# Dostenlinus/Aiyagari-HARK

Hardware: AMD Instinct MI355X
Metric: GE solves/sec (Table II sweep); agent-periods/sec; % HBM roofline (higher is better)
Workload: dtype f64

## Files before the change

aiyagari_hark_amd/_lib.py:

```python
from __future__ import annotations

import atexit
import ctypes
import os
import threading

import torch

HERE = os.path.dirname(os.path.abspath(__file__))
LIB_PATH = os.environ.get("AIYAGARI_LIB") or os.path.join(HERE, "lib", "libaiyagari.so")

AIY_OK = 0
ERRORS = {-1: "AIY_ERR_ARG", -2: "AIY_ERR_HIP", -3: "AIY_ERR_STATE", -4: "AIY_ERR_UNSUPPORTED",
          -5: "AIY_ERR_COMM"}
AIY_MAX_STATES = 64
AIY_SOW_DOUBLES = 8
AIY_OPT_USE_GRAPHS = 1
AIY_OPT_RESIDENT = 2
AIY_OPT_RESIDENT_SHAPE = 3
AIY_OPT_HIST_FUSED = 4
AIY_OPT_RESIDENT_STREAM = 5
AIY_OPT_HIST_RESIDENT = 6
AIY_OPT_HIST_CLUSTER = 7
AIY_OPT_HIST_ACCEL = 8
AIY_OPT_HIST_KRYLOV = 9
AIY_OPT_GE_RESIDENT = 10
AIY_OPT_CU_LIMIT = 11
AIY_OPT_GE_REBALANCE = 12
AIY_OPT_GE_EXTRAP_PERIOD = 13
AIY_OPT_GE_LOGSEC = 14
AIY_OPT_HIST_PULL = 15
AIY_OPT_GE_LOOSE_HIST = 17
AIY_OPT_RESIDENT_SHAPE_STREAM = 18
AIY_OPT_GE_ANDERSON = 23

c_double_p = ctypes.POINTER(ctypes.c_double)
c_int32_p = ctypes.POINTER(ctypes.c_int32)
c_uint8_p = ctypes.POINTER(ctypes.c_uint8)
vp = ctypes.c_void_p


class EgmDims(ctypes.Structure):
    _fields_ = [("n_cal", ctypes.c_int32), ("S", ctypes.c_int32), ("n_M", ctypes.c_int32), ("n_a", ctypes.c_int32)]


class EgmInputs(ctypes.Structure):
    _fields_ = [(n, vp) for n in ("a_grid", "M_grid", "P", "R_next", "W_next", "M_next", "lab", "beta", "crra")]


class Market(ctypes.Structure):
    _fields_ = [("cap_share", ctypes.c_double), ("depr_fac", ctypes.c_double),
                ("prod", ctypes.c_double * 2), ("agg_L", ctypes.c_double * 2)]


class PanelModel(ctypes.Structure):
    _fields_ = [("S", ctypes.c_int32), ("n_M", ctypes.c_int32), ("n_a", ctypes.c_int32), ("n_lab", ctypes.c_int32),
                ("tables", vp), ("M_grid", vp), ("lab_level", vp), ("lab_cdf", vp), ("mrkv_hist", vp),
                ("act_T", ctypes.c_int32), ("unemployed", ctypes.c_int32)]


class PanelBatch(ctypes.Structure):
    _fields_ = [("n_cal", ctypes.c_int32), ("S", ctypes.c_int32), ("n_M", ctypes.c_int32), ("n_a", ctypes.c_int32),
                ("n_lab", ctypes.c_int32), ("tables", vp), ("M_grid", vp), ("lab_level", vp), ("lab_cdf", vp),
                ("mrkv_hist", vp), ("unemployed", ctypes.c_int32)]


class StationaryModel(ctypes.Structure):
    _fields_ = [("n_cal", ctypes.c_int32), ("S", ctypes.c_int32), ("n_a", ctypes.c_int32)] + \
               [(n, vp) for n in ("a_grid", "P", "lab", "beta", "crra", "alpha", "delta", "disc")]


class TransitionModel(ctypes.Structure):
    _fields_ = [("n_cal", ctypes.c_int32), ("S", ctypes.c_int32), ("n_a", ctypes.c_int32), ("T", ctypes.c_int32)] + \
               [(n, vp) for n in ("a_grid", "P", "lab", "beta", "crra", "R", "w", "m_term", "c_term")]


class GeOptions(ctypes.Structure):
    _fields_ = [("method", ctypes.c_int32), ("r_tol", ctypes.c_double), ("egm_tol", ctypes.c_double),
                ("hist_tol", ctypes.c_double), ("max_steps", ctypes.c_int32), ("max_egm_cycles", ctypes.c_int32),
                ("max_hist_iter", ctypes.c_int32), ("warm_hist", ctypes.c_int32), ("warm_egm", ctypes.c_int32),
                ("accel", ctypes.c_int32), ("r_lo", vp), ("r_hi", vp), ("secant_start", ctypes.c_int32),
                ("loose_bracket", ctypes.c_int32), ("egm_extrapolate", ctypes.c_int32), ("status_out", vp)]


SIGNATURES = {
    "aiy_version": (ctypes.c_int32, []),
    "aiy_create": (ctypes.c_int32, [ctypes.c_int32, ctypes.POINTER(vp)]),
    "aiy_destroy": (ctypes.c_int32, [vp]),
    "aiy_last_error": (ctypes.c_char_p, [vp]),
    "aiy_egm_step": (ctypes.c_int32, [vp, ctypes.POINTER(EgmDims), ctypes.POINTER(EgmInputs), vp, vp, vp, vp, vp]),
    "aiy_egm_solve": (ctypes.c_int32, [vp, ctypes.POINTER(EgmDims), ctypes.POINTER(EgmInputs), ctypes.c_double,
                                       ctypes.c_int32, ctypes.c_int32, vp, vp, vp, vp, c_int32_p, c_double_p, vp]),
    "aiy_egm_solve_from": (ctypes.c_int32, [vp, ctypes.POINTER(EgmDims), ctypes.POINTER(EgmInputs), ctypes.c_double,
                                            ctypes.c_int32, ctypes.c_int32, vp, vp, vp, vp, vp, vp, c_int32_p,
                                            c_double_p, vp]),
    "aiy_egm_kernel_time": (ctypes.c_int32, [vp, ctypes.POINTER(EgmDims), ctypes.POINTER(EgmInputs), vp, vp, vp, vp,
                                             ctypes.c_int32, ctypes.POINTER(ctypes.c_float), vp]),
    "aiy_policy_eval": (ctypes.c_int32, [vp, ctypes.c_int32, ctypes.c_int32, ctypes.c_int32, vp, vp, vp, vp, vp, vp,
                                         ctypes.c_int64, vp, vp]),
    "aiy_sim_periods": (ctypes.c_int32, [vp, ctypes.POINTER(PanelModel), ctypes.POINTER(Market), ctypes.c_int64,
                                         ctypes.c_int64, ctypes.c_int64, vp, vp, vp, ctypes.c_int64, vp,
                                         ctypes.c_int64, ctypes.c_uint64, ctypes.c_uint32, ctypes.c_int32,
                                         ctypes.c_int32, vp, vp, vp, vp]),
    "aiy_sim_period_local": (ctypes.c_int32, [vp, ctypes.POINTER(PanelModel), ctypes.c_int64, ctypes.c_int64, vp, vp,
                                              vp, vp, ctypes.c_uint64, ctypes.c_uint32, ctypes.c_int32, vp, vp]),
    "aiy_sim_period_prices": (ctypes.c_int32, [vp, ctypes.POINTER(PanelModel), ctypes.POINTER(Market),
                                               ctypes.c_int64, ctypes.c_int32, vp, vp, vp, vp]),
    "aiy_get_shocks": (ctypes.c_int32, [vp, ctypes.c_int32, vp, ctypes.c_int64, ctypes.c_int64, vp, vp,
                                        ctypes.c_uint64, ctypes.c_uint32, ctypes.c_int32, vp]),
    "aiy_get_states": (ctypes.c_int32, [vp, vp, ctypes.c_int64, ctypes.c_double, ctypes.c_double, vp, vp, vp, vp,
                                        vp]),
    "aiy_get_controls": (ctypes.c_int32, [vp, ctypes.c_int32, ctypes.c_int32, ctypes.c_int32, vp, vp, c_double_p,
                                          ctypes.c_int32, ctypes.c_double, ctypes.c_int64, vp, vp, vp, vp, vp]),
    "aiy_get_poststates": (ctypes.c_int32, [vp, ctypes.c_int64, vp, vp, vp, vp]),
    "aiy_sum": (ctypes.c_int32, [vp, vp, ctypes.c_int64, vp, vp]),
    "aiy_sim_kernel_time": (ctypes.c_int32, [vp, ctypes.POINTER(PanelModel), ctypes.POINTER(Market), ctypes.c_int64,
                                             vp, vp, ctypes.c_uint64, ctypes.c_uint32, vp, ctypes.c_int32,
                                             ctypes.POINTER(ctypes.c_float), vp]),
    "aiy_panel_launch_stats": (ctypes.c_int32, [vp, c_double_p, ctypes.POINTER(ctypes.c_int64),
                                                ctypes.POINTER(ctypes.c_int64), ctypes.c_int32]),
    "aiy_sim_block_max_agents": (ctypes.c_int32, []),
    "aiy_sim_block_periods": (ctypes.c_int32, [vp, ctypes.POINTER(PanelBatch), vp, ctypes.c_int64, vp, vp, vp,
                                               vp, vp, ctypes.c_uint32, ctypes.c_int32, ctypes.c_int32, ctypes.c_int32,
                                               vp, vp, vp, vp]),
    "aiy_set_option": (ctypes.c_int32, [vp, ctypes.c_int32, ctypes.c_int64]),
    "aiy_get_option": (ctypes.c_int32, [vp, ctypes.c_int32, ctypes.POINTER(ctypes.c_int64)]),
    "aiy_index_ints_per_row": (ctypes.c_int32, []),
    "aiy_panel_table_bytes": (ctypes.c_int64, [ctypes.c_int32, ctypes.c_int32, ctypes.c_int32, ctypes.c_int32]),
    "aiy_panel_build": (ctypes.c_int32, [vp, ctypes.c_int32, ctypes.c_int32, ctypes.c_int32, ctypes.c_int32,
                                         ctypes.c_int32, ctypes.c_int32, vp, vp, vp, vp]),
    "aiy_build_index": (ctypes.c_int32, [vp, ctypes.c_int64, ctypes.c_int32, vp, vp, vp]),
    "aiy_comm_unique_id": (ctypes.c_int32, [vp]),
    "aiy_comm_init": (ctypes.c_int32, [vp, vp, ctypes.c_int32, ctypes.c_int32]),
    "aiy_comm_bind": (ctypes.c_int32, [vp, vp]),
    "aiy_comm_destroy": (ctypes.c_int32, [vp]),
    "aiy_allreduce_sum": (ctypes.c_int32, [vp, vp, ctypes.c_int64, vp]),
    "aiy_hist_lottery": (ctypes.c_int32, [vp, ctypes.c_int32, ctypes.c_int32, ctypes.c_int32, vp, vp, vp, vp, vp, vp,
                                          vp, vp, vp]),
    "aiy_hist_solve": (ctypes.c_int32, [vp, ctypes.c_int32, ctypes.c_int32, ctypes.c_int32, vp, vp, vp, vp,
                                        ctypes.c_double, ctypes.c_int32, ctypes.c_int32, vp, vp, c_double_p,
                                        c_int32_p, vp]),
    "aiy_hist_launch_stats": (ctypes.c_int32, [vp, c_double_p, ctypes.POINTER(ctypes.c_int64), ctypes.c_int32]),
    "aiy_ge_resident_plan": (ctypes.c_int32, [vp, ctypes.c_int32, ctypes.c_int32, ctypes.c_int32, c_int32_p]),
    "aiy_ge_last_profile": (ctypes.c_int32, [vp, c_double_p, ctypes.c_int32]),
    "aiy_ge_last_eval_log": (ctypes.c_int32, [vp, c_double_p, ctypes.c_int32]),
    "aiy_ge_last_rounds": (ctypes.c_int32, [vp, ctypes.POINTER(ctypes.c_int32), ctypes.POINTER(ctypes.c_int32)]),
    "aiy_ge_launch_stats": (ctypes.c_int32, [vp, c_double_p, ctypes.POINTER(ctypes.c_int64), c_double_p, c_double_p,
                                             ctypes.c_int32]),
    "aiy_ge_stationary_work_bytes": (ctypes.c_int64, [ctypes.c_int32, ctypes.c_int32, ctypes.c_int32]),
    "aiy_ge_stationary": (ctypes.c_int32, [vp, ctypes.POINTER(StationaryModel), ctypes.POINTER(GeOptions), vp,
                                           c_double_p, c_double_p, c_double_p, c_int32_p, c_int32_p, c_int32_p, vp]),
    "aiy_transition_work_bytes": (ctypes.c_int64, [ctypes.c_int32, ctypes.c_int32, ctypes.c_int32, ctypes.c_int32]),
    "aiy_transition_backward": (ctypes.c_int32, [vp, ctypes.POINTER(TransitionModel), vp, vp, vp, vp, vp, vp]),
    "aiy_transition_forward": (ctypes.c_int32, [vp, ctypes.c_int32, ctypes.c_int32, ctypes.c_int32, ctypes.c_int32,
                                                vp, vp, vp, vp, vp, vp, vp, vp, vp, c_double_p, c_double_p, vp]),
    "aiy_transition_forward_marginals": (ctypes.c_int32, [vp, ctypes.c_int32, ctypes.c_int32, ctypes.c_int32,
                                                          ctypes.c_int32, vp, vp, vp, vp, vp, vp, vp, vp, vp,
                                                          c_double_p, c_double_p, vp, vp]),
    "aiy_jacobian_work_bytes": (ctypes.c_int64, [ctypes.c_int32, ctypes.c_int32, ctypes.c_int32, ctypes.c_int32]),
    "aiy_jacobian_fanout": (ctypes.c_int32, [vp, ctypes.c_int32, ctypes.c_int32, ctypes.c_int32, ctypes.c_int32,
                                             ctypes.c_int32, vp, vp, vp, vp, vp, vp, vp]),
    "aiy_jacobian_diff": (ctypes.c_int32, [vp, ctypes.c_int64, vp, vp, ctypes.c_double, vp]),
    "aiy_jacobian_expectation": (ctypes.c_int32, [vp, ctypes.c_int32, ctypes.c_int32, ctypes.c_int32, ctypes.c_int32,
                                                  vp, vp, vp, vp, vp, vp, vp]),
    "aiy_jacobian_contract": (ctypes.c_int32, [vp, ctypes.c_int32, ctypes.c_int32, ctypes.c_int32, ctypes.c_int32,
                                               vp, vp, vp, vp, vp, vp]),
    "aiy_lottery_mean": (ctypes.c_int32, [vp, ctypes.c_int32, ctypes.c_int32, ctypes.c_int32, ctypes.c_int32, vp, vp, vp,
                                          vp, vp]),
    "aiy_aggregate_lotteries": (ctypes.c_int32, [vp, ctypes.c_int32, ctypes.c_int32, ctypes.c_int32, ctypes.c_int32,
                                                 ctypes.c_int32, vp, vp, vp, vp, vp, vp, vp, vp]),
    "aiy_wealth_stats": (ctypes.c_int32, [vp, vp, vp, ctypes.c_int64, c_double_p, ctypes.c_int32, c_double_p,
                                          c_double_p, vp]),
    "aiy_dist_stats_work_bytes": (ctypes.c_int64, [ctypes.c_int32, ctypes.c_int32]),
    "aiy_dist_marginal": (ctypes.c_int32, [vp, ctypes.c_int32, ctypes.c_int32, ctypes.c_int32, vp, vp, vp]),
    "aiy_dist_stats": (ctypes.c_int32, [vp, ctypes.c_int32, ctypes.c_int32, ctypes.c_int32, vp, vp, c_double_p,
                                        ctypes.c_int32, vp, c_double_p, c_double_p, c_double_p, vp]),
    "aiy_value_work_bytes": (ctypes.c_int64, [ctypes.c_int32, ctypes.c_int32, ctypes.c_int32]),
    "aiy_value_backward": (ctypes.c_int32, [vp, ctypes.c_int32, ctypes.c_int32, ctypes.c_int32, ctypes.c_int32,
                                            vp, vp, vp, vp, vp, vp, vp, vp, vp, vp, vp, vp, vp, vp]),
    "aiy_value_stationary": (ctypes.c_int32, [vp, ctypes.c_int32, ctypes.c_int32, ctypes.c_int32, vp, vp, vp, vp, vp,
                                              vp, vp, vp, vp, c_double_p, ctypes.c_double, ctypes.c_int32,
                                              ctypes.c_int32, vp, vp, c_int32_p, c_double_p, vp]),
    "aiy_value_reduce": (ctypes.c_int32, [vp, ctypes.c_int32, ctypes.c_int32, ctypes.c_int32, vp, vp, c_double_p, vp]),
    "aiy_consumption_equivalent": (ctypes.c_int32, [vp, ctypes.c_int32, ctypes.c_int64, vp, vp, vp, vp, vp, vp]),
}

_lib = None
_lock = threading.Lock()


class AiyagariLibError(RuntimeError):
    pass


def load(path: str | None = None):
    global _lib
    with _lock:
        if _lib is not None:
            return _lib
        p = path or LIB_PATH
        if not os.path.exists(p):
            raise AiyagariLibError(
                f"{p} is missing: build it with `python -m aiyagari_hark_amd.build` "
                "(there is no CPU fallback)")
        lib = ctypes.CDLL(p)
        for name, (res, args) in SIGNATURES.items():
            fn = getattr(lib, name)
            fn.restype = res
            fn.argtypes = args
        _lib = lib
        return lib


def exported_symbols():
    return sorted(SIGNATURES)


class Handle:

    def __init__(self, device: int | None = 0):
        self.lib = load()
        if device is None:
            device = torch.cuda.current_device()
        self.device = device
        h = vp()
        rc = self.lib.aiy_create(int(device), ctypes.byref(h))
        if rc != AIY_OK:
            raise AiyagariLibError(f"aiy_create(device={device}) failed: {ERRORS.get(rc, rc)}")
        self.h = h

    def check(self, rc: int, what: str):
        if rc != AIY_OK:
            msg = self.lib.aiy_last_error(self.h)
            raise AiyagariLibError(f"{what} failed: {ERRORS.get(rc, rc)}: {msg.decode() if msg else ''}")

    def get_option(self, option: int) -> int:
        v = ctypes.c_int64()
        self.check(self.lib.aiy_get_option(self.h, int(option), ctypes.byref(v)), "aiy_get_option")
        return int(v.value)

    def set_options(self, values: dict) -> dict:
        prev = {k: self.get_option(k) for k in values}
        for k, v in values.items():
            self.check(self.lib.aiy_set_option(self.h, int(k), int(v)), "aiy_set_option")
        return prev

    def close(self):
        if getattr(self, "h", None):
            self.lib.aiy_destroy(self.h)
            self.h = None

    def __del__(self):
        try:
            self.close()
        except Exception:
            pass


_handles: dict[int, Handle] = {}


def close_all():
    while _handles:
        _, h = _handles.popitem()
        h.close()


atexit.register(close_all)


def handle(device: int | None = None) -> Handle:
    if device is None:
        device = torch.cuda.current_device()
    h = _handles.get(device)
    if h is None:
        h = Handle(device)
        _handles[device] = h
    return h


def ptr(t) -> int | None:
    if t is None:
        return None
    if not t.is_cuda:
        raise AiyagariLibError("libaiyagari takes device tensors only")
    if not t.is_contiguous():
        raise AiyagariLibError("tensor must be contiguous")
    return t.data_ptr()


def work_space(device, what: str, label: str, **sizes):
    nbytes = int(getattr(handle(device.index).lib, f"aiy_{what}_work_bytes")(*(int(v) for v in sizes.values())))
    if nbytes < 0:
        raise ValueError(f"{label} sizes not supported: ".lstrip() + " ".join(f"{k}={v}" for k, v in sizes.items()))
    return torch.empty(nbytes, dtype=torch.uint8, device=device)


def stream_ptr(stream=None) -> int:
    s = stream if stream is not None else torch.cuda.current_stream()
    return s.cuda_stream
```

aiyagari_hark_amd/csrc/ge_resident.hip:

```cpp
#include "common.h"
#include "egm_common.h"
#include "ge_search.h"
#include "hist_bicg.h"
#include "hist_cluster.h"
#include "internal.h"

#include <algorithm>
#include <cmath>

namespace aiy {

constexpr int kGeTHMax = 1024;
constexpr int kGeWavesMax = kGeTHMax / kWave;
constexpr int kGeMaxTiles = 16;
constexpr int kGeBufs = 5;
constexpr int kGeAaM = 3;
constexpr int kGeAaHist = kGeAaM + 2;
#ifdef AIY_DIAG_NO_FUSEA
constexpr bool kGeFuseA = false;
#else
constexpr bool kGeFuseA = true;
#endif
#ifndef AIY_FUSEA_KC2
#define AIY_FUSEA_KC2 0
#endif
constexpr bool kGeFuseAKc2 = AIY_FUSEA_KC2 != 0;
template <int NW>
constexpr size_t ge_egm_lds() { return (size_t)NW * (8 * kTile + 4 * kWin) * sizeof(double); }

struct GeCalDev {
  double alpha, delta, disc, r_lo, r_hi;
};

struct GeState;
struct GeRun {
  int n_cal, S, n_a, G, nj, cap, n_work;
  const double* a_grid;
  const double* P;
  const double* lab;
  const double* beta;
  const double* crra;
  const GeCalDev* cal;
  int method;
  double r_tol, egm_tol, hist_tol;
  int max_steps, max_cyc, max_hist;
  int warm_hist, warm_egm, secant, loose, extrap;
  int extrap_period;
  int aa_period;
  double* aah;
  int logsec;
  double loose_hist;
  double* qb;
  int* ainv;
  double* tab;
  double* mass;
  double* pmass;
  double* pg;
  int* lo;
  double* wlo;
  double* slab;
  int* span;
  unsigned* ctr;
  unsigned long long* gran;
  const int* cal_ids;
  GeState* saved;
  const int* resume;
  unsigned* done_ctr;
  int stop_at;
  int* out_done;
  unsigned* err;
  double* out_r;
  double* out_K;
  double* out_Ks;
  int* out_steps;
  int* out_cyc;
  int* out_its;
  int* out_status;
  double* out_prof;
  double* out_evlog;
};
constexpr int kGeProf = 8;
constexpr int kGeEvLog = 32;
constexpr int kGeEvRec = 6;

struct GeState {
  GeEval ev;
  GeEvalOpts opt;
  double Ks, dist, lam_prev, fext;
  int status, n, stop, nan_stop, moved, extrap;
  int in_hist;
  int buf[kGeBufs];
  long long cyc_sum, its_sum;
  unsigned long long t_egm, t_lot, t_hist, t_k, t0, t_ev0;
  unsigned nc_prev[2];
  unsigned nbc;
};

template <int TH>
__device__ __forceinline__ bool ge_reduce(unsigned long long* gran, int G, int w, unsigned& ne, const double* vals,
                                          int nv, unsigned kmax, double (*s_part)[kGeWavesMax], double* s_res,
                                          int* s_flag, unsigned* err) {
  asm volatile("s_waitcnt vmcnt(0)" ::: "memory");
  return hc_reduce<TH>(gran, G, w, ne, vals, nv, kmax, s_part, s_res, s_flag, err, [] {});
}

template <int SMAX, int NW, typename Sink, typename Begin, typename End>
__device__ __forceinline__ void ge_rows_pass(int S, int n_a, int j0, int j1, const double* __restrict__ a_grid,
                                             const double* __restrict__ src_m, const double* __restrict__ src_c,
                                             double R, const double* s_Wl, int* s_hint, double* lds_win,
                                             Sink&& sink, Begin&& begin, End&& end) {
  const int tid = threadIdx.x, lane = tid & (kWave - 1);
  const int wv = __builtin_amdgcn_readfirstlane(tid / kWave);
  const int n = n_a, n1 = n_a + 1;
  const int ntile = (j1 - j0 + kTile - 1) / kTile;
  double* X = lds_win + (size_t)wv * 4 * kWin;
  double* Y = X + kWin;
  double* XB = X + 2 * kWin;
  double* YB = X + 3 * kWin;
#pragma unroll 1
  for (int tile = wv; tile < ntile; tile += NW) {
    const int jr = j0 + tile * kTile + lane;
    const int j = jr < j1 ? jr : j1 - 1;
    const double a = a_grid[j];
    int* hint = s_hint + tile * SMAX;
    auto fetch = [&](int r, RowWin& wn) {
      const int rr = r < S ? r : S - 1;
      load_win<true>(src_m + (size_t)rr * n1, src_c + (size_t)rr * n1, n, win_base(hint[rr], n1), lane, wn);
    };
    unsigned redo = 0u;
    auto step_unit = [&](int u, const RowWin& wa, const RowWin& wb) {
      const int ra = 2 * u, rb = 2 * u + 1;
      if (ra >= S) return;
      const bool has_b = rb < S;
      const int rbb = has_b ? rb : ra;
      const bool na = __any(stage_win(wa, n, X, Y, lane));
      const bool nb = __any(stage_win(wb, n, XB, YB, lane));
      __builtin_amdgcn_fence(__ATOMIC_RELEASE, "wavefront");
      __builtin_amdgcn_wave_barrier();
      __builtin_amdgcn_fence(__ATOMIC_ACQUIRE, "wavefront");
      const double qa = R * a + s_Wl[ra];
      const double qb = R * a + s_Wl[rbb];
      int lba, lbb;
      bool oka, okb;
      const double fa = search_win(wa.base, na, n, qa, X, Y, lba, oka);
      const double fb = search_win(wb.base, nb, n, qb, XB, YB, lbb, okb);
      hint[ra] = __builtin_amdgcn_readfirstlane(lba);
      if (has_b) hint[rb] = __builtin_amdgcn_readfirstlane(lbb);
      if (__any(!oka)) redo |= 1u << ra;
      else sink(tile, jr, j, ra, qa, fa);
      if (has_b) {
        if (__any(!okb)) redo |= 1u << rb;
        else sink(tile, jr, j, rb, qb, fb);
      }
    };
    RowWin a0, b0, a1, b1;
    fetch(0, a0);
    fetch(1, b0);
    begin(tile, j);
#pragma unroll 1
    for (int u = 0; 2 * u < S; u += 2) {
      fetch(2 * u + 2, a1);
      fetch(2 * u + 3, b1);
      step_unit(u, a0, b0);
      fetch(2 * u + 4, a0);
      fetch(2 * u + 5, b0);
      step_unit(u + 1, a1, b1);
    }
#pragma unroll 1
    while (redo != 0u) {
      const int s = __builtin_ctz(redo);
      redo &= redo - 1u;
      const double q = R * a + s_Wl[s];
      int lb;
      const double f = interp_row_global_agent(src_m + (size_t)s * n1, src_c + (size_t)s * n1, n, q, lb);
      hint[s] = __builtin_amdgcn_readfirstlane(lb);
      sink(tile, jr, j, s, q, f);
    }
    end(tile, j, a);
  }
}

template <int SMAX, int SC, int PK, int NW>
__device__ __forceinline__ double ge_egm_cycle(int S, int n_a, int j0, int j1, const double* __restrict__ a_grid,
                                               const double* src_m, const double* src_c, double* dst_m,
                                               double* dst_c, bool track, double R, double beta, double gam,
                                               const double* s_Wl, const double* s_Pe, int* s_hint,
                                               double* lds_v, double* lds_win, double* ring) {
  const int tid = threadIdx.x, lane = tid & (kWave - 1);
  const int wv = __builtin_amdgcn_readfirstlane(tid / kWave);
  const int n1 = n_a + 1;
  double* Vw = lds_v + (size_t)wv * SMAX * kTile;
  const int ntile = (j1 - j0 + kTile - 1) / kTile;
  double dmax = 0.0;
  if (src_m == nullptr) {
#pragma unroll 1
    for (int tile = wv; tile < ntile; tile += NW) {
      const int jr = j0 + tile * kTile + lane;
      const int j = jr < j1 ? jr : j1 - 1;
      const double a = a_grid[j];
      for (int sp = 0; sp < S; ++sp) {
        const double c = (R * a + s_Wl[sp]) * 1.0;
        Vw[sp * kTile + lane] = R * marg_u<PK>(c, gam);
      }
      for (int s = 0; s < S; ++s) {
        double sum;
        if constexpr (SC > 0) sum = pairwise_dot<SC>(Vw + lane, s_Pe + s * SC);
        else sum = np_pairwise_sum<SMAX>(S, [&](int t) { return Vw[t * kTile + lane] * uniform_f64(s_Pe[s * S + t]); });
        const double c = inv_marg<PK>(beta * sum, gam);
        store_f64_agent(&dst_m[(size_t)s * n1 + j + 1], a + c);
        store_f64_agent(&dst_c[(size_t)s * n1 + j + 1], c);
        if (ring) store_f64_agent(&ring[(size_t)s * n_a + j], c);
        if (j == 0) {
          store_f64_agent(&dst_m[(size_t)s * n1], kBorrowNode);
          store_f64_agent(&dst_c[(size_t)s * n1], kBorrowNode);
        }
      }
    }
    return 0.0;
  }
  constexpr int NP = SC > 0 ? SC : SMAX;
  double pmv[NP], pcv[NP];
  auto begin = [&](int, int j) {
#pragma unroll
    for (int s = 0; s < NP; ++s) {
      const int rr = s < S ? s : S - 1;
      pmv[s] = load_f64_agent(&src_m[(size_t)rr * n1 + j + 1]);
      pcv[s] = load_f64_agent(&src_c[(size_t)rr * n1 + j + 1]);
    }
  };
  auto end = [&](int, int j, double a) {
#pragma unroll
    for (int s = 0; s < NP; ++s) {
      if (s < S) {
        __builtin_amdgcn_sched_barrier(0);
        double sum;
        if constexpr (SC > 0) sum = pairwise_dot<SC>(Vw + lane, s_Pe + s * SC);
        else sum = np_pairwise_sum<SMAX>(S, [&](int t) { return Vw[t * kTile + lane] * uniform_f64(s_Pe[s * S + t]); });
        const double E = beta * sum;
        const double c = inv_marg<PK>(E, gam);
        const double m = a + c;
        store_f64_agent(&dst_m[(size_t)s * n1 + j + 1], m);
        store_f64_agent(&dst_c[(size_t)s * n1 + j + 1], c);
        if (ring) store_f64_agent(&ring[(size_t)s * n_a + j], c);
        if (track) dmax = nan_max(dmax, nan_max(fabs(m - pmv[s]), fabs(c - pcv[s])));
        if (j == 0) {
          store_f64_agent(&dst_m[(size_t)s * n1], kBorrowNode);
          store_f64_agent(&dst_c[(size_t)s * n1], kBorrowNode);
        }
      }
    }
  };
  ge_rows_pass<SMAX, NW>(S, n_a, j0, j1, a_grid, src_m, src_c, R, s_Wl, s_hint, lds_win,
                     [&](int, int, int, int sp, double, double f) {
                       Vw[sp * kTile + lane] = R * marg_u<PK>(f, gam);
                     },
                     begin, end);
  return dmax;
}

constexpr int kGeSmax = 8;
extern __shared__ double ge_dyn[];
__shared__ double ge_s_part[kHcRed][kGeWavesMax];
__shared__ double ge_s_res[kHcRed];
__shared__ int ge_s_flag;
__shared__ double ge_s_Pe[kGeSmax * kGeSmax];
__shared__ double ge_s_Wl[kGeSmax];
__shared__ int ge_s_hint[kGeMaxTiles * kGeSmax];
__shared__ unsigned ge_s_nc;
__shared__ GeState ge_st;

template <int SMAX, int SC, int PK, int NW>
__device__ __forceinline__ double ge_egm_cycle_fn(int S, int n_a, int j0, int j1, const double* a_grid,
                                               const double* src_m, const double* src_c, double* dst_m,
                                               double* dst_c, bool track, double R, double beta, double gam,
                                               double* dyn, double* ring) {
  return ge_egm_cycle<SMAX, SC, PK, NW>(S, n_a, j0, j1, a_grid, src_m, src_c, dst_m, dst_c, track, R, beta, gam,
                                        ge_s_Wl, ge_s_Pe, ge_s_hint, dyn, dyn + (size_t)NW * SMAX * kTile, ring);
}

template <int SMAX, int NW>
__device__ __forceinline__ void ge_lottery_fn(int S, int n_a, int j0, int j1, const double* a_grid, const double* fm,
                                           const double* fc, double R, bool have_prev, int* LO, double* WL,
                                           bool write_through) {
  ge_rows_pass<SMAX, NW>(S, n_a, j0, j1, a_grid, fm, fc, R, ge_s_Wl, ge_s_hint, ge_dyn + (size_t)NW * SMAX * kTile,
                     [&](int, int jr, int, int s, double q, double c) {
                       if (jr >= j1) return;
                       const double ap = q - c;
                       const size_t o = (size_t)s * n_a + jr;
                       int d = -1;
                       if (have_prev) {
                         const int h = LO[o];
                         if (h >= 0 && h < n_a - 1 && a_grid[h] <= ap && ap < a_grid[h + 1]) d = h;
                       }
                       if (d < 0) {
                         int lo = 0, hi = n_a;
                         while (lo < hi) {
                           const int mid = lo + ((hi - lo) >> 1);
                           if (a_grid[mid] <= ap) lo = mid + 1; else hi = mid;
                         }
                         d = lo - 1;
                       }
                       d = d < 0 ? 0 : (d > n_a - 2 ? n_a - 2 : d);
                       double wl = (a_grid[d + 1] - ap) / (a_grid[d + 1] - a_grid[d]);
                       wl = wl < 0.0 ? 0.0 : (wl > 1.0 ? 1.0 : wl);
                       if (write_through) {
                         __hip_atomic_store(to_global(&LO[o]), d, __ATOMIC_RELAXED, __HIP_MEMORY_SCOPE_AGENT);
                         store_f64_agent(&WL[o], wl);
                       } else {
                         LO[o] = d;
                         WL[o] = wl;
                       }
                     },
                     [](int, int) {}, [](int, int, double) {});
}

struct GeCtx {
  double* tab;
  double* X;
  double* PX;
  int* LO;
  double* WL;
  unsigned* ctr;
  unsigned long long* cw;
  unsigned long long* gran;
  const double* a_grid;
  double* aah;
  unsigned* err;
  double beta, gam;
  size_t tab_sz;
  int j0, j1, w, G, S, n_a, cal, lc;
  __device__ __forceinline__ double* tabm(int b) const { return tab + (size_t)b * 2 * tab_sz; }
  __device__ __forceinline__ double* tabc(int b) const { return tab + (size_t)b * 2 * tab_sz + tab_sz; }
};

__device__ __forceinline__ GeEvalOpts ge_eval_opts(const GeRun& g) {
  return {g.method, g.loose, g.logsec, g.warm_egm, g.warm_hist, g.secant, g.r_tol, g.egm_tol, g.hist_tol, g.loose_hist};
}

__device__ __forceinline__ bool ge_barrier(const GeCtx& cx, unsigned& nb, unsigned* err) {
  asm volatile("s_waitcnt vmcnt(0)" ::: "memory");
  ++nb;
  return hc_barrier(err, cx.ctr, (unsigned)cx.G * nb, &ge_s_flag);
}

__device__ __forceinline__ bool ge_vote(const GeCtx& cx, unsigned* err, unsigned flag, unsigned& dlt) {
  GeState& st = ge_st;
  const int tid = threadIdx.x;
  if (tid == 0) ++st.nbc;
  asm volatile("s_waitcnt vmcnt(0)" ::: "memory");
  __syncthreads();
  const unsigned k = st.nbc, par = k & 1u;
  if (!hc_barrier_count(err, &cx.cw[par], (unsigned)cx.G * ((k + par) / 2), flag, &ge_s_nc, &ge_s_flag))
    return false;
  if (tid == 0) {
    dlt = ge_s_nc - st.nc_prev[par];
    st.nc_prev[par] = ge_s_nc;
  }
  return true;
}

template <int TH>
__device__ __forceinline__ void ge_secant_tables(const GeCtx& cx, int b_cur, int b_prev, int b_init, double theta) {
  const int tid = threadIdx.x, n1 = cx.n_a + 1;
  for (int s = 0; s < cx.S; ++s) {
    for (int k = cx.j0 + tid; k < cx.j1; k += TH) {
      const size_t o = (size_t)s * n1 + k + 1;
      const double cm = load_f64_agent(&cx.tabm(b_cur)[o]), pm = load_f64_agent(&cx.tabm(b_prev)[o]);
      const double cc = load_f64_agent(&cx.tabc(b_cur)[o]), pc = load_f64_agent(&cx.tabc(b_prev)[o]);
      store_f64_agent(&cx.tabm(b_init)[o], theta == 0.0 ? cm : cm + theta * (cm - pm));
      store_f64_agent(&cx.tabc(b_init)[o], theta == 0.0 ? cc : cc + theta * (cc - pc));
    }
    if (cx.j0 == 0 && tid == 0) {
      store_f64_agent(&cx.tabm(b_init)[(size_t)s * n1], kBorrowNode);
      store_f64_agent(&cx.tabc(b_init)[(size_t)s * n1], kBorrowNode);
    }
  }
}

template <int TH>
__device__ __forceinline__ bool ge_extrapolate(const GeCtx& cx, unsigned& nb, unsigned* err, int b_dst, int b_src,
                                               double dclu, int n) {
  GeState& st = ge_st;
  const int tid = threadIdx.x, n1 = cx.n_a + 1;
  if (tid == 0) {
    st.fext = egm_extrap_factor(dclu, st.dist, st.ev.etol, n, st.lam_prev);
    if (st.fext != 0.0) st.moved = 1;
  }
  __syncthreads();
  const double f = st.fext;
  if (f != 0.0) {
    double* cm = cx.tabm(b_dst);
    double* cc = cx.tabc(b_dst);
    const double* pm = cx.tabm(b_src);
    const double* pc = cx.tabc(b_src);
    for (int s = 0; s < cx.S; ++s)
      for (int k = cx.j0 + tid; k < cx.j1; k += TH) {
        const size_t o = (size_t)s * n1 + k + 1;
        const double x = load_f64_agent(&cm[o]), y = load_f64_agent(&cc[o]);
        store_f64_agent(&cm[o], x + f * (x - load_f64_agent(&pm[o])));
        store_f64_agent(&cc[o], y + f * (y - load_f64_agent(&pc[o])));
      }
    if (!ge_barrier(cx, nb, err)) return false;
  }
  return true;
}

__device__ __forceinline__ double* ge_ring(const GeCtx& cx, int c) {
  return cx.aah + (size_t)(c % kGeAaHist) * cx.S * cx.n_a;
}

template <int TH>
__device__ __forceinline__ bool ge_anderson(const GeCtx& cx, unsigned& nb, unsigned& ne, int n, int b_dst) {
  static_assert(kGeAaM == 3 && kGeAaHist == 5, "the mixing is written for m = 3");
  const int tid = threadIdx.x, n1 = cx.n_a + 1;
  const double* W0 = ge_ring(cx, n - 4);
  const double* W1 = ge_ring(cx, n - 3);
  const double* W2 = ge_ring(cx, n - 2);
  const double* W3 = ge_ring(cx, n - 1);
  const double* W4 = ge_ring(cx, n);
  double gp[9];
  for (int q = 0; q < 9; ++q) gp[q] = 0.0;
  for (int s = 0; s < cx.S; ++s)
    for (int k = cx.j0 + tid; k < cx.j1; k += TH) {
      const size_t o = (size_t)s * cx.n_a + k;
      const double w0 = load_f64_agent(W0 + o), w1 = load_f64_agent(W1 + o), w2 = load_f64_agent(W2 + o);
      const double w3 = load_f64_agent(W3 + o), w4 = load_f64_agent(W4 + o);
      aa_gram_add(w0, w1, w2, w3, w4, gp);
    }
  double gs[9], gam[3];
  if (!ge_reduce<TH>(cx.gran, cx.G, cx.w, ne, gp, 6, 0u, ge_s_part, ge_s_res, &ge_s_flag, cx.err)) return false;
  for (int q = 0; q < 6; ++q) gs[q] = ge_s_res[q];
  if (!ge_reduce<TH>(cx.gran, cx.G, cx.w, ne, gp + 6, 3, 0u, ge_s_part, ge_s_res, &ge_s_flag, cx.err)) return false;
  for (int q = 0; q < 3; ++q) gs[6 + q] = ge_s_res[q];
  if (aa_solve(gs, gam)) {
    double* dm = cx.tabm(b_dst);
    double* dc = cx.tabc(b_dst);
    for (int s = 0; s < cx.S; ++s)
      for (int k = cx.j0 + tid; k < cx.j1; k += TH) {
        const size_t o = (size_t)s * cx.n_a + k;
        const double w1 = load_f64_agent(W1 + o), w2 = load_f64_agent(W2 + o);
        const double w3 = load_f64_agent(W3 + o), w4 = load_f64_agent(W4 + o);
        const double cn = aa_mix(gam, w1, w2, w3, w4);
        store_f64_agent(&dm[(size_t)s * n1 + k + 1], cx.a_grid[k] + cn);
        store_f64_agent(&dc[(size_t)s * n1 + k + 1], cn);
      }
    if (tid == 0) ge_st.moved = 1;
    if (!ge_barrier(cx, nb, cx.err)) return false;
  }
  return true;
}

struct GeHhOpt {
  int max_cyc, aa_period, extrap_period;
};

__device__ __forceinline__ bool ge_ring_wanted(int n, int p) {
  const int ph = n % p;
  const int mix = ph == 0 ? n : n + (p - ph);
  return (ph == 0 || ph > p - kGeAaHist) && mix >= kGeAaHist + 1;
}

template <int SMAX, int SC, int PK, int TH>
__device__ __forceinline__ int ge_household_solve(const GeCtx& cx, unsigned& nb, unsigned& ne, const GeHhOpt& g,
                                                  double R, const double* init_m, const double* init_c, double* dyn) {
  constexpr int NW = TH / kWave;
  GeState& st = ge_st;
  const int tid = threadIdx.x;
  int final_buf = -1;
  for (int attempt = 0; attempt < 2; ++attempt) {
    if (!ge_barrier(cx, nb, cx.err)) return -1;
    const bool aa = g.aa_period > 0 && attempt == 0;
    const bool ext = st.extrap != 0 && attempt == 0 && !aa;
    if (tid == 0) {
      st.lam_prev = -1.0;
      st.moved = 0;
      st.nan_stop = 0;
    }
    int n = 1;
    const int last_allowed = g.max_cyc + 1;
    bool converged = false;
    while (true) {
      const int b_dst = st.buf[n & 1], b_src = st.buf[(n - 1) & 1];
      const double* sm = n == 1 ? init_m : cx.tabm(b_src);
      const double* sc = n == 1 ? init_c : cx.tabc(b_src);
      const bool track = n >= 2;
      double* ring = aa && ge_ring_wanted(n, g.aa_period) ? ge_ring(cx, n) : nullptr;
      const double dl = ge_egm_cycle_fn<SMAX, SC, PK, NW>(cx.S, cx.n_a, cx.j0, cx.j1, cx.a_grid, sm, sc, cx.tabm(b_dst),
                                                          cx.tabc(b_dst), track, R, cx.beta, cx.gam, dyn, ring);
      const int xp = g.extrap_period;
      const bool want_value = ext && n >= xp - 1 && ((n % xp) == xp - 1 || (n % xp) == 0);
      double dclu = 0.0;
      bool go;
      if (want_value) {
        double v[1] = {dl};
        if (!ge_reduce<TH>(cx.gran, cx.G, cx.w, ne, v, 1, 1u, ge_s_part, ge_s_res, &ge_s_flag, cx.err)) return -1;
        dclu = ge_s_res[0];
        go = dclu > st.ev.etol;
        if (tid == 0) st.nan_stop = dclu != dclu;
      } else {
        const double dw = wave_nan_max(dl);
        if ((tid & (kWave - 1)) == 0) ge_s_part[0][tid / kWave] = dw;
        __syncthreads();
        unsigned flag = 0u, dlt = 0u;
        if (tid == 0) {
          double d = ge_s_part[0][0];
          for (int q = 1; q < TH / kWave; ++q) d = nan_max(d, ge_s_part[0][q]);
          flag = (d > st.ev.etol ? 1u : 0u) | (d != d ? (1u << 16) : 0u);
        }
        if (!ge_vote(cx, cx.err, flag, dlt)) return -1;
        if (tid == 0) {
          st.stop = (dlt & 0xffffu) == 0u || (dlt >> 16) != 0u;
          st.nan_stop = (dlt >> 16) != 0u;
        }
        __syncthreads();
        go = !st.stop;
      }
      if (track && !go) {
        converged = true;
        break;
      }
      if (n >= last_allowed) break;
      if (want_value && (n % xp) == 0) {
        if (!ge_extrapolate<TH>(cx, nb, cx.err, b_dst, b_src, dclu, n)) return -1;
      } else if (want_value) {
        if (tid == 0) st.dist = dclu;
      }
      if (aa && n >= g.aa_period && n >= kGeAaHist + 1 && (n % g.aa_period) == 0) {
        if (!ge_anderson<TH>(cx, nb, ne, n, b_dst)) return -1;
      }
      ++n;
    }
    if (tid == 0) {
      st.n = n;
      if (!converged) st.status |= 1;
    }
    __syncthreads();
    final_buf = st.buf[n & 1];
    if (!(st.moved && st.nan_stop)) break;
    if (tid == 0) {
      st.extrap = 0;
      st.status &= ~1;
    }
    __syncthreads();
  }
  return final_buf;
}

struct GeHhArgs {
  gptr<double> tab, aah;
  gptr<unsigned> ctr, err;
  gptr<unsigned long long> gran;
  gptr<const double> a_grid, init_m, init_c;
  double beta, gam, R;
  int j0, j1, w, G, S, n_a;
  GeHhOpt opt;
  unsigned dyn_lds;
};
template <int SMAX, int SC, int PK, int TH>
__device__ __noinline__ int ge_household_isolated(GeHhArgs a, unsigned* nb_io, unsigned* ne_io) {
  double* dyn = (double*)(lptr<double>)(size_t)(unsigned)hk_uni((int)a.dyn_lds);
  GeCtx cx;
  cx.tab = (double*)hk_uni(a.tab);
  cx.aah = (double*)hk_uni(a.aah);
  cx.ctr = (unsigned*)hk_uni(a.ctr);
  cx.cw = reinterpret_cast<unsigned long long*>(cx.ctr + 2);
  cx.err = (unsigned*)hk_uni(a.err);
  cx.gran = (unsigned long long*)hk_uni(a.gran);
  cx.a_grid = (const double*)hk_uni(a.a_grid);
  cx.X = cx.PX = cx.WL = nullptr;
  cx.LO = nullptr;
  cx.beta = hk_uni(a.beta); cx.gam = hk_uni(a.gam);
  cx.j0 = hk_uni(a.j0); cx.j1 = hk_uni(a.j1); cx.w = hk_uni(a.w); cx.G = hk_uni(a.G);
  cx.S = SC > 0 ? SC : hk_uni(a.S);
  cx.n_a = hk_uni(a.n_a);
  cx.cal = cx.lc = 0;
  cx.tab_sz = (size_t)cx.S * (cx.n_a + 1);
  const GeHhOpt opt = {hk_uni(a.opt.max_cyc), hk_uni(a.opt.aa_period), hk_uni(a.opt.extrap_period)};
  unsigned nb = *nb_io, ne = *ne_io;
  const int fb = ge_household_solve<SMAX, SC, PK, TH>(cx, nb, ne, opt, hk_uni(a.R), (const double*)hk_uni(a.init_m),
                                                     (const double*)hk_uni(a.init_c), dyn);
  *nb_io = nb;
  *ne_io = ne;
  return fb;
}

template <int TH>
__device__ __forceinline__ void ge_mass_start(const GeCtx& cx, bool fresh, bool warm, bool secant, double theta) {
  const int tid = threadIdx.x;
  if (fresh) {
    const double u0 = 1.0 / ((double)cx.S * cx.n_a);
    for (int s = 0; s < cx.S; ++s)
      for (int k = cx.j0 + tid; k < cx.j1; k += TH) cx.X[(size_t)s * cx.n_a + k] = u0;
  } else if (warm) {
    for (int s = 0; s < cx.S; ++s)
      for (int k = cx.j0 + tid; k < cx.j1; k += TH) {
        const size_t o = (size_t)s * cx.n_a + k;
        const double x = cx.X[o];
        if (secant) cx.X[o] = theta == 0.0 ? x : x + theta * (x - cx.PX[o]);
        cx.PX[o] = x;
      }
  }
}

template <int TH>
__device__ __forceinline__ bool ge_capital(const GeCtx& cx, unsigned& ne, unsigned* err) {
  double part = 0.0;
  for (int k = cx.j0 + (int)threadIdx.x; k < cx.j1; k += TH) {
    double ms = 0.0;
    for (int s = 0; s < cx.S; ++s) ms += cx.X[(size_t)s * cx.n_a + k];
    part += ms * cx.a_grid[k];
  }
  double v[1] = {part};
  return ge_reduce<TH>(cx.gran, cx.G, cx.w, ne, v, 1, 0u, ge_s_part, ge_s_res, &ge_s_flag, err);
}

__device__ __forceinline__ void ge_write_out(const GeCtx& cx, const GeRun& g, const GeCalDev& cd) {
  const GeState& st = ge_st;
  const int cal = cx.cal;
  __hip_atomic_fetch_add(to_global(g.done_ctr), 1u, __ATOMIC_RELAXED, __HIP_MEMORY_SCOPE_AGENT);
  g.out_done[cal] = 1;
  g.out_r[cal] = st.ev.rs.x;
  g.out_K[cal] = ge_prices(st.ev.rs.x, cd.alpha, cd.delta).Kd;
  g.out_Ks[cal] = st.Ks;
  g.out_steps[cal] = st.ev.steps;
  g.out_cyc[cal] = (int)min(st.cyc_sum, 0x7fffffffll);
  g.out_its[cal] = (int)min(st.its_sum, 0x7fffffffll);
  g.out_status[cal] = st.status | (st.ev.rs.done ? 0 : 4);
  double* pf = g.out_prof + (size_t)cal * kGeProf;
  pf[0] = st.t_egm * 0.01;
  pf[1] = st.t_lot * 0.01;
  pf[2] = st.t_hist * 0.01;
  pf[3] = st.t_k * 0.01;
  pf[4] = (__builtin_amdgcn_s_memrealtime() - st.t0) * 0.01;
  pf[5] = (double)st.cyc_sum;
  pf[6] = (double)st.its_sum;
  pf[7] = (double)st.ev.steps;
}

template <int SMAX, int SC, int KC, int TH, bool PULL>
__global__ __launch_bounds__(TH) void ge_cluster_kernel(GeRun g) {
  constexpr int NW = TH / kWave;
  static_assert(SMAX <= kGeSmax, "file-scope LDS sized for kGeSmax states");
  GeState& st = ge_st;

  const int per = gridDim.x >> 3;
  const int u = (blockIdx.x & 7) * per + (blockIdx.x >> 3);
  if (u >= g.n_work) return;
  const int G = g.G, S = g.S, n_a = g.n_a;
  const int tid = threadIdx.x;
  GeCtx cx;
  cx.G = G; cx.S = S; cx.n_a = n_a;
  cx.lc = u / G; cx.w = u - cx.lc * G;
  const int lc = cx.lc, w = cx.w, cal = g.cal_ids[lc];
  cx.cal = cal;
  cx.j0 = w * g.nj; cx.j1 = min(cx.j0 + g.nj, n_a);
  const int j0 = cx.j0, j1 = cx.j1;
  cx.a_grid = g.a_grid + (size_t)cal * n_a;
  cx.beta = g.beta[cal]; cx.gam = g.crra[cal];
  const GeCalDev cd = g.cal[cal];
  cx.tab_sz = (size_t)S * (n_a + 1);
  cx.tab = g.tab + (size_t)cal * kGeBufs * 2 * cx.tab_sz;
  const size_t row0 = (size_t)cal * S * n_a;
  cx.X = g.mass + row0;
  cx.PX = g.pmass + row0;
  cx.LO = g.lo + row0;
  cx.WL = g.wlo + row0;
  cx.ctr = g.ctr + (size_t)lc * kHcCtrStride;
  cx.cw = reinterpret_cast<unsigned long long*>(cx.ctr + 2);
  cx.gran = g.gran + (size_t)lc * 2 * G * kHcRedRec;
  cx.aah = g.aah + (size_t)cal * kGeAaHist * S * n_a;
  cx.err = g.err;
  unsigned nb = 0, ne = 0;
  const int pk = crra_kind(cx.gam);

  for (int q = tid; q < S * S; q += TH) ge_s_Pe[q] = g.P[(size_t)cal * S * S + q];
  for (int q = tid; q < kGeMaxTiles * SMAX; q += TH) ge_s_hint[q] = -1;
  if (tid == 0) {
    if (g.resume[cal]) {
      st = g.saved[cal];
      st.t0 = __builtin_amdgcn_s_memrealtime() - st.t0;
    } else {
      st.ev.init(ge_eval_opts(g), cd.r_lo, cd.r_hi);
      st.Ks = 0.0;
      st.in_hist = 0;
      st.status = 0;
      st.cyc_sum = st.its_sum = 0;
      for (int b = 0; b < kGeBufs; ++b) st.buf[b] = b;
      st.t_egm = st.t_lot = st.t_hist = st.t_k = 0ull;
      st.t0 = __builtin_amdgcn_s_memrealtime();
    }
    st.opt = ge_eval_opts(g);
    st.nc_prev[0] = st.nc_prev[1] = 0u;
    st.nbc = 0u;
  }
  __syncthreads();

  bool stopped = false;
  while ((!st.ev.rs.done && st.ev.steps < g.max_steps) || st.ev.final_ks) {
    if (g.stop_at > 0 && st.ev.steps > 0 && !st.in_hist) {
      unsigned flag = 0u, dlt = 0u;
      if (tid == 0)
        flag = __hip_atomic_load(to_global(g.done_ctr), __ATOMIC_RELAXED, __HIP_MEMORY_SCOPE_AGENT) >=
                       (unsigned)g.stop_at ? 1u : 0u;
      if (!ge_vote(cx, g.err, flag, dlt)) return;
      if (tid == 0) st.stop = dlt != 0u;
      __syncthreads();
      if (st.stop) {
        stopped = true;
        break;
      }
    }
    unsigned long long tp = __builtin_amdgcn_s_memrealtime();
    if (tid == 0 && !st.in_hist) st.t_ev0 = tp;
    if (!st.in_hist) {
      if (tid == 0) {
        st.ev.plan(st.opt, cd.alpha, cd.delta);
        st.extrap = g.extrap;
        st.moved = 0;
      }
      __syncthreads();
      if (tid < S) ge_s_Wl[tid] = st.ev.wage * g.lab[(size_t)cal * S + tid];
      const double R = st.ev.R, theta = st.ev.theta;
      const bool secant = st.ev.secant != 0, warm = st.ev.warm_egm != 0;
      const int b_cur = st.buf[2], b_prev = st.buf[3], b_init = st.buf[4];
      if (secant) ge_secant_tables<TH>(cx, b_cur, b_prev, b_init, theta);
      tp = __builtin_amdgcn_s_memrealtime();
      GeHhArgs ha;
      ha.tab = to_global(cx.tab); ha.aah = to_global(cx.aah); ha.ctr = to_global(cx.ctr); ha.err = to_global(g.err);
      ha.gran = to_global(cx.gran); ha.a_grid = to_global(cx.a_grid);
      ha.init_m = to_global((const double*)(secant ? cx.tabm(b_init) : (warm ? cx.tabm(b_cur) : nullptr)));
      ha.init_c = to_global((const double*)(secant ? cx.tabc(b_init) : (warm ? cx.tabc(b_cur) : nullptr)));
      ha.beta = cx.beta; ha.gam = cx.gam; ha.R = R;
      ha.j0 = j0; ha.j1 = j1; ha.w = w; ha.G = G; ha.S = S; ha.n_a = n_a;
      ha.opt = {g.max_cyc, g.aa_period, g.extrap_period};
      ha.dyn_lds = hk_lds_addr(ge_dyn);
      const int final_buf = pk == 1   ? ge_household_isolated<SMAX, SC, 1, TH>(ha, &nb, &ne)
                            : pk == 3 ? ge_household_isolated<SMAX, SC, 3, TH>(ha, &nb, &ne)
                            : pk == 5 ? ge_household_isolated<SMAX, SC, 5, TH>(ha, &nb, &ne)
                                      : ge_household_isolated<SMAX, SC, 0, TH>(ha, &nb, &ne);
      if (final_buf < 0) return;
      if (tid == 0) {
        const unsigned long long tn = __builtin_amdgcn_s_memrealtime();
        st.t_egm += tn - tp;
        st.cyc_sum += st.n;
        const int fb = final_buf;
        const int other = st.buf[0] == fb ? st.buf[1] : st.buf[0];
        const int old_prev = st.buf[3];
        st.buf[3] = st.buf[2];
        st.buf[2] = fb;
        st.buf[0] = other;
        st.buf[1] = old_prev;
      }
      __syncthreads();
      tp = __builtin_amdgcn_s_memrealtime();
      ge_lottery_fn<SMAX, NW>(S, n_a, j0, j1, cx.a_grid, cx.tabm(st.buf[2]), cx.tabc(st.buf[2]), R, st.ev.steps > 0,
                              cx.LO, cx.WL, PULL);
      ge_mass_start<TH>(cx, st.ev.fresh_mass != 0, warm, secant, theta);
      __syncthreads();
      if (tid == 0) {
        const unsigned long long tn = __builtin_amdgcn_s_memrealtime();
        st.t_lot += tn - tp;
        tp = tn;
      }
    }
    int mv;
    {
      HkArgs hk;
      hk.G = G; hk.S = S; hk.n_a = n_a; hk.cap = g.cap; hk.w = w; hk.j0 = j0; hk.j1 = j1;
      hk.LO = to_global((const int*)cx.LO); hk.WL = to_global((const double*)cx.WL); hk.X = to_global(cx.X);
      hk.Pg = to_global(g.pg + row0); hk.Vg = to_global((double*)nullptr);
      hk.slab_cl = to_global(g.slab + (size_t)lc * G * 2 * g.cap);
      hk.span_cl = to_global(g.span + (size_t)lc * G * SMAX * 4);
      hk.ctr = to_global(cx.ctr); hk.gran = to_global(cx.gran); hk.Pc = to_global(g.P + (size_t)cal * S * S);
      hk.max_iter = g.max_hist; hk.err = to_global(g.err);
      hk.tol = st.ev.htol;
      hk.stop_ctr = to_global((const unsigned*)(g.stop_at > 0 ? g.done_ctr : nullptr));
      hk.stop_at = (unsigned)g.stop_at;
      hk.Qg = to_global(g.qb + row0);
      hk.Ainv = to_global(g.ainv + (size_t)cal * S * (n_a + 1));
      hk.lottery_fresh = true;
      hk.dyn_lds = hk_lds_addr(ge_dyn);
      if constexpr (PULL) mv = hk_solve_inlined<SMAX, KC, TH, true, false, SC>(hk, &nb, &ne);
      else mv = hk_solve_isolated<SMAX, KC, TH, false, (KC == 1 || kGeFuseAKc2) && kGeFuseA, SC>(hk, &nb, &ne);
    }
    if (mv == -1) return;
    if (tid == 0) {
      const unsigned long long tn = __builtin_amdgcn_s_memrealtime();
      st.t_hist += tn - tp;
      tp = tn;
    }
    if (mv <= -2) {
      if (tid == 0) {
        st.its_sum += -mv - 2;
        st.in_hist = 1;
        if (w == 0) __hip_atomic_fetch_add(to_global(g.done_ctr + 1), 1u, __ATOMIC_RELAXED, __HIP_MEMORY_SCOPE_AGENT);
      }
      __syncthreads();
      stopped = true;
      break;
    }
    if (tid == 0) st.in_hist = 0;
    if (!ge_capital<TH>(cx, ne, g.err)) return;
    const bool fin = st.ev.final_ks != 0;
    if (tid == 0) {
      const double Ks = ge_s_res[0];
      if (w == 0 && st.ev.steps < kGeEvLog && !fin) {
        double* ev = g.out_evlog + ((size_t)cal * kGeEvLog + st.ev.steps) * kGeEvRec;
        ev[0] = st.ev.rs.x;
        ev[1] = (Ks - st.ev.Kd) / st.ev.Kd;
        ev[2] = (double)st.n;
        ev[3] = (double)mv;
        ev[4] = (double)st.ev.loose;
        ev[5] = (double)(__builtin_amdgcn_s_memrealtime() - st.t_ev0) * 0.01;
      }
      st.its_sum += mv;
      if (mv >= g.max_hist) st.status |= 2;
    }
    if (fin) {
      if (tid == 0) st.Ks = ge_s_res[0];
      __syncthreads();
      break;
    }
    if (tid == 0) {
      st.ev.accept(ge_s_res[0]);
      st.Ks = ge_s_res[0];
      st.t_k += __builtin_amdgcn_s_memrealtime() - tp;
    }
    __syncthreads();
  }
  if (stopped) {
    if (w == 0 && tid == 0) {
      st.t0 = __builtin_amdgcn_s_memrealtime() - st.t0;
      g.saved[cal] = st;
      g.out_done[cal] = 0;
    }
    return;
  }
  if (w == 0 && tid == 0) ge_write_out(cx, g, cd);
}

struct GePlan {
  int G = 0, nj = 0, kc = 0, smax = 0, sc = 0, cap = 0, blocks = 0, th = 0;
  size_t lds = 0;
  const void* fn = nullptr;
};

template <int SMAX, int SC, int KC, int TH>
static const void* ge_fn(bool pull) {
  return pull ? reinterpret_cast<const void*>(ge_cluster_kernel<SMAX, SC, KC, TH, true>)
              : reinterpret_cast<const void*>(ge_cluster_kernel<SMAX, SC, KC, TH, false>);
}

static bool ge_make_plan(aiy_handle* h, int n_cal, int S, int n_a, GePlan& p) {
  if (S < 1 || S > kGeSmax || n_a < 2 || n_cal < 1) return false;
  int cus = 0;
  if (hipDeviceGetAttribute(&cus, hipDeviceAttributeMultiprocessorCount, h->device) != hipSuccess || cus < 1) return false;
  if (h->cu_limit > 0) cus = std::min(cus, h->cu_limit);
  const int g_cap = h->hist_cluster_cap > 0 ? h->hist_cluster_cap : 32;
  if (!hc_cluster_split(n_a, (n_a + 2 * 512 - 1) / (2 * 512), g_cap, cus, n_cal, &p.G, &p.nj)) return false;
  if (p.G > kHcMaxG) return false;
  if (p.nj > kGeMaxTiles * kTile) return false;
  if ((long long)p.G * n_cal > cus) return false;
  p.th = 512;
  const int th = p.th;
  p.kc = p.nj <= th ? 1 : 2;
  p.smax = S == 7 ? 7 : 8;
  p.sc = S == 7 ? 7 : 0;
  const bool pull = h->hist_pull != 0;
  if (p.sc == 7) p.fn = p.kc == 1 ? ge_fn<7, 7, 1, 512>(pull) : ge_fn<7, 7, 2, 512>(pull);
  else p.fn = p.kc == 1 ? ge_fn<8, 0, 1, 512>(pull) : ge_fn<8, 0, 2, 512>(pull);
  HcLds lds;
  if (!hc_lds_budget(h->device, p.fn, lds)) return false;
  p.lds = lds.dyn;
  const size_t vbytes = (size_t)p.kc * p.smax * th * sizeof(double);
  const size_t egm_lds = ge_egm_lds<8>();
  if (p.lds < egm_lds || p.lds <= vbytes + 4096) return false;
  p.cap = (int)((p.lds - vbytes) / sizeof(double));
  p.blocks = (p.G * n_cal + 7) / 8 * 8;
  return true;
}

struct GeScratch {
  double *tab, *mass, *pmass, *pg, *qb, *wlo, *slab, *outd, *prof, *evlog, *aah;
  int *ainv, *lo, *span, *ids, *resume, *done, *outi;
  unsigned *ctr, *err;
  unsigned long long* gran;
  GeState* saved;
  GeCalDev* cal;
  size_t bytes;
};
static GeScratch ge_scratch(Carve c, int n_cal, int S, int n_a, int cus, int cap_max) {
  GeScratch L;
  const size_t pts = (size_t)n_cal * S * n_a;
  L.tab = c.take<double>((size_t)n_cal * kGeBufs * 2 * S * (n_a + 1));
  L.mass = c.take<double>(pts); L.pmass = c.take<double>(pts); L.pg = c.take<double>(pts); L.qb = c.take<double>(pts);
  L.ainv = c.take<int>((size_t)n_cal * S * (n_a + 1));
  L.lo = c.take<int>(pts); L.wlo = c.take<double>(pts);
  L.slab = c.take<double>((size_t)cus * 2 * cap_max);
  L.span = c.take<int>((size_t)cus * 8 * 4);
  L.ctr = c.take<unsigned>((size_t)n_cal * kHcCtrStride);
  L.gran = c.take<unsigned long long>((size_t)cus * 2 * kHcRedRec);
  L.ids = c.take<int>(n_cal);
  L.saved = c.take<GeState>(n_cal);
  L.resume = c.take<int>(n_cal);
  L.done = c.take<int>(n_cal);
  L.err = c.take<unsigned>(256 / sizeof(unsigned));
  L.cal = c.take<GeCalDev>(n_cal);
  L.outd = c.take<double>((size_t)n_cal * 3);
  L.outi = c.take<int>((size_t)n_cal * 4);
  L.prof = c.take<double>((size_t)n_cal * kGeProf);
  L.evlog = c.take<double>((size_t)n_cal * kGeEvLog * kGeEvRec);
  L.aah = c.take<double>((size_t)n_cal * kGeAaHist * S * n_a);
  L.bytes = c.bytes();
  return L;
}

int32_t ge_stationary_resident(aiy_handle* h, const aiy_stationary_model* M, const aiy_ge_options* o, double* r_out,
                               double* K_out, double* Ks_out, int32_t* steps_out, int32_t* cyc_out,
                               int32_t* its_out, int32_t* status_out, hipStream_t st) {
  if (!h->ge_resident || o->accel >= 0) return 0;
  const int n_cal = M->n_cal, S = M->S, n_a = M->n_a;
  GePlan p0;
  if (!ge_make_plan(h, n_cal, S, n_a, p0)) return 0;
  int cus = 0;
  if (hipDeviceGetAttribute(&cus, hipDeviceAttributeMultiprocessorCount, h->device) != hipSuccess) return 0;
  if (h->cu_limit > 0) cus = std::min(cus, h->cu_limit);
  const int cap_max = (int)(kHcLdsTotal / sizeof(double));
  const int32_t rsv = h->ge.reserve(h, ge_scratch(Carve(), n_cal, S, n_a, cus, cap_max).bytes);
  if (rsv) return rsv;
  const GeScratch L = ge_scratch(Carve(h->ge.get()), n_cal, S, n_a, cus, cap_max);
  std::vector<GeCalDev> cals(n_cal);
  for (int c = 0; c < n_cal; ++c) {
    cals[c].alpha = M->alpha[c];
    cals[c].delta = M->delta[c];
    cals[c].disc = M->disc[c];
    cals[c].r_lo = o->r_lo ? o->r_lo[c] : GeEval::default_lo(M->delta[c]);
    cals[c].r_hi = o->r_hi ? o->r_hi[c] : GeEval::default_hi(M->disc[c]);
  }
  GeRun g;
  g.n_cal = n_cal; g.S = S; g.n_a = n_a;
  g.a_grid = M->a_grid; g.P = M->P; g.lab = M->lab; g.beta = M->beta; g.crra = M->crra;
  g.cal = L.cal;
  g.method = o->method; g.r_tol = o->r_tol; g.egm_tol = o->egm_tol; g.hist_tol = o->hist_tol;
  g.max_steps = o->max_steps;
  g.max_cyc = o->max_egm_cycles > 0 ? o->max_egm_cycles : 5000;
  g.max_hist = o->max_hist_iter > 0 ? o->max_hist_iter : 200000;
  g.warm_hist = o->warm_hist != 0; g.warm_egm = o->warm_egm != 0;
  g.secant = o->secant_start != 0; g.loose = o->loose_bracket != 0; g.extrap = o->egm_extrapolate != 0;
  g.extrap_period = h->ge_extrap_period;
  g.aa_period = o->egm_extrapolate != 0 ? h->ge_anderson : 0;
  g.aah = L.aah;
  g.logsec = h->ge_logsec;
  g.tab = L.tab; g.mass = L.mass; g.pmass = L.pmass; g.pg = L.pg; g.qb = L.qb; g.ainv = L.ainv;
  g.loose_hist = std::pow(10.0, -(double)h->ge_loose_hist);
  g.lo = L.lo; g.wlo = L.wlo; g.slab = L.slab; g.span = L.span; g.ctr = L.ctr; g.gran = L.gran;
  int *d_ids = L.ids, *d_resume = L.resume, *outi = L.outi;
  g.cal_ids = d_ids; g.saved = L.saved; g.resume = d_resume; g.out_done = L.done;
  g.err = L.err;
  g.done_ctr = g.err + 1;
  double* outd = L.outd;
  g.out_r = outd; g.out_K = outd + n_cal; g.out_Ks = outd + 2 * n_cal;
  g.out_steps = outi; g.out_cyc = outi + n_cal; g.out_its = outi + 2 * n_cal; g.out_status = outi + 3 * n_cal;
  g.out_prof = L.prof; g.out_evlog = L.evlog;
  AIY_HIP(h, hipMemsetAsync(g.out_evlog, 0, (size_t)n_cal * kGeEvLog * kGeEvRec * sizeof(double), st));
  AIY_HIP(h, hipMemcpyAsync(L.cal, cals.data(), sizeof(GeCalDev) * n_cal, hipMemcpyHostToDevice, st));
  AIY_HIP(h, hipMemsetAsync(d_resume, 0, (size_t)n_cal * sizeof(int), st));
  AIY_HIP(h, hipMemsetAsync(g.out_done, 0, (size_t)n_cal * sizeof(int), st));
  AIY_HIP(h, h->ge_timer.ensure());
  std::vector<int> active(n_cal), done(n_cal, 0), resume(n_cal, 0);
  for (int c = 0; c < n_cal; ++c) active[c] = c;
  h->ge_rounds = 0;
  h->ge_mid_stops = 0;
  while (!active.empty()) {
    const int n = (int)active.size();
    GePlan p;
    if (!ge_make_plan(h, n, S, n_a, p)) return fail(h, AIY_ERR_STATE, "device-resident GE: no plan for %d calibrations", n);
    const Admit adm = admit_launch(p.fn, p.th, p.lds, true);
    if (adm != Admit::fits) {
      if (h->ge_rounds == 0) return 0;
      return fail(h, AIY_ERR_STATE, adm == Admit::attr_error ? "device-resident GE: dynamic LDS attribute"
                                                             : "device-resident GE: occupancy query");
    }
    g.G = p.G; g.nj = p.nj; g.cap = p.cap; g.n_work = n * p.G;
    g.stop_at = (h->ge_rebalance > 0 && n > 4) ? std::max(1, (n * h->ge_rebalance + 99) / 100) : 0;
    std::vector<int> res_h(n_cal);
    for (int c = 0; c < n_cal; ++c) res_h[c] = resume[c];
    AIY_HIP(h, hipMemcpyAsync(d_ids, active.data(), sizeof(int) * n, hipMemcpyHostToDevice, st));
    AIY_HIP(h, hipMemcpyAsync(d_resume, res_h.data(), sizeof(int) * n_cal, hipMemcpyHostToDevice, st));
    AIY_HIP(h, hipMemsetAsync(g.ctr, 0, (size_t)n * kHcCtrStride * sizeof(unsigned), st));
    AIY_HIP(h, hipMemsetAsync(g.gran, 0, (size_t)n * 2 * p.G * kHcRedRec * sizeof(unsigned long long), st));
    AIY_HIP(h, hipMemsetAsync(g.err, 0, 256, st));
    void* args[] = {&g};
    AIY_HIP(h, h->ge_timer.begin(st));
    AIY_HIP(h, hipLaunchKernel(p.fn, dim3(p.blocks), dim3(p.th), args, p.lds, st));
    AIY_HIP(h, h->ge_timer.end(st));
    unsigned errw[3] = {0, 0, 0};
    AIY_HIP(h, hipMemcpyAsync(errw, g.err, sizeof(errw), hipMemcpyDeviceToHost, st));
    AIY_HIP(h, hipMemcpyAsync(done.data(), g.out_done, sizeof(int) * n_cal, hipMemcpyDeviceToHost, st));
    AIY_HIP(h, hipStreamSynchronize(st));
    h->ge_timer.collect();
    ++h->ge_rounds;
    h->ge_mid_stops += errw[2];
    const unsigned err = errw[0];
    if (err == 1u)
      return fail(h, AIY_ERR_STATE, "device-resident GE: cluster barrier timed out (workgroups not co-resident?)");
    if (err) return fail(h, AIY_ERR_STATE, "device-resident GE: histogram shape does not fit (error %u)", err);
    std::vector<int> next;
    for (int c : active) {
      if (!done[c]) {
        next.push_back(c);
        resume[c] = 1;
      }
    }
    if ((int)next.size() == n && g.stop_at > 0)
      return fail(h, AIY_ERR_STATE, "device-resident GE: a rebalancing launch finished no calibration");
    active.swap(next);
  }
  std::vector<double> hd(3 * (size_t)n_cal);
  std::vector<int> hi(4 * (size_t)n_cal);
  AIY_HIP(h, hipMemcpyAsync(hd.data(), outd, sizeof(double) * 3 * n_cal, hipMemcpyDeviceToHost, st));
  AIY_HIP(h, hipMemcpyAsync(hi.data(), outi, sizeof(int) * 4 * n_cal, hipMemcpyDeviceToHost, st));
  h->ge_prof.assign((size_t)n_cal * kGeProf, 0.0);
  h->ge_evlog.assign((size_t)n_cal * kGeEvLog * kGeEvRec, 0.0);
  AIY_HIP(h, hipMemcpyAsync(h->ge_evlog.data(), g.out_evlog, sizeof(double) * kGeEvLog * kGeEvRec * n_cal,
                            hipMemcpyDeviceToHost, st));
  AIY_HIP(h, hipMemcpyAsync(h->ge_prof.data(), g.out_prof, sizeof(double) * kGeProf * n_cal, hipMemcpyDeviceToHost,
                            st));
  AIY_HIP(h, hipStreamSynchronize(st));
  long long cyc = 0, its = 0;
  int steps = 0;
  for (int c = 0; c < n_cal; ++c) {
    r_out[c] = hd[c];
    K_out[c] = hd[n_cal + c];
    if (Ks_out) Ks_out[c] = hd[2 * n_cal + c];
    steps = std::max(steps, hi[c]);
    cyc += hi[n_cal + c];
    its += hi[2 * n_cal + c];
    if (status_out) status_out[c] = hi[3 * n_cal + c];
    h->ge_points += (double)hi[2 * n_cal + c] * S * n_a;
    h->ge_egm_cycles += hi[n_cal + c];
  }
  if (steps_out) *steps_out = steps;
  if (cyc_out) *cyc_out = (int32_t)std::min<long long>(cyc, 0x7fffffff);
  if (its_out) *its_out = (int32_t)std::min<long long>(its, 0x7fffffff);
  return 1;
}

}

using namespace aiy;

extern "C" int32_t aiy_ge_resident_plan(aiy_handle* h, int32_t n_cal, int32_t S, int32_t n_a, int32_t* out4) {
  if (!h || !out4) return AIY_ERR_ARG;
  GePlan p;
  if (!h->ge_resident || !ge_make_plan(h, n_cal, S, n_a, p)) {
    out4[0] = out4[1] = out4[2] = out4[3] = 0;
    return 0;
  }
  out4[0] = p.G;
  out4[1] = p.nj;
  out4[2] = p.kc;
  out4[3] = p.blocks;
  return 1;
}

extern "C" int32_t aiy_ge_last_rounds(aiy_handle* h, int32_t* launches, int32_t* mid_solve_stops) {
  if (!h) return AIY_ERR_ARG;
  if (launches) *launches = h->ge_rounds;
  if (mid_solve_stops) *mid_solve_stops = h->ge_mid_stops;
  return AIY_OK;
}

extern "C" int32_t aiy_ge_launch_stats(aiy_handle* h, double* ms_sum, int64_t* launches, double* point_matvecs,
                                       double* egm_cycles, int32_t reset) {
  if (!h) return AIY_ERR_ARG;
  h->ge_timer.read(ms_sum, launches, reset != 0);
  if (point_matvecs) *point_matvecs = h->ge_points;
  if (egm_cycles) *egm_cycles = h->ge_egm_cycles;
  if (reset) {
    h->ge_points = 0.0;
    h->ge_egm_cycles = 0.0;
  }
  return AIY_OK;
}

extern "C" int32_t aiy_ge_last_eval_log(aiy_handle* h, double* out, int32_t n_cal) {
  if (!h || !out || n_cal < 0) return AIY_ERR_ARG;
  const int have = (int)(h->ge_evlog.size() / (kGeEvLog * kGeEvRec));
  const int n = std::min(have, (int)n_cal);
  std::copy(h->ge_evlog.begin(), h->ge_evlog.begin() + (size_t)n * kGeEvLog * kGeEvRec, out);
  return n;
}

extern "C" int32_t aiy_ge_last_profile(aiy_handle* h, double* out, int32_t n_cal) {
  if (!h || !out || n_cal < 0) return AIY_ERR_ARG;
  const int have = (int)(h->ge_prof.size() / kGeProf);
  const int n = std::min(have, (int)n_cal);
  std::copy(h->ge_prof.begin(), h->ge_prof.begin() + (size_t)n * kGeProf, out);
  return n;
}
```

aiyagari_hark_amd/csrc/hist_bicg.h:

```cpp
#pragma once

#include "common.h"
#include "hist_cluster.h"

namespace aiy {

constexpr int kHkStall = 256;
constexpr double kHkStopSentinel = 1e300;
constexpr int kHkHeavy = 31;
#ifndef AIY_HK_WAVE_CN
#define AIY_HK_WAVE_CN 6
#endif
constexpr int kHkWaveCn = AIY_HK_WAVE_CN;
static_assert(kHcCand <= 32, "covering-span index and count packed in 5 + 6 bits");
__device__ __forceinline__ unsigned short hk_cinfo(int cf, int cn, int hi) {
  return (unsigned short)(cf | (cn << 5) | (hi << 11));
}
__device__ __forceinline__ int hk_cf(int ci) { return ci & 31; }
__device__ __forceinline__ int hk_cn(int ci) { return (ci >> 5) & 63; }
__device__ __forceinline__ int hk_hi(int ci) { return ci >> 11; }

__device__ __forceinline__ double hk_uni(double x) {
  const unsigned long long u = (unsigned long long)__double_as_longlong(x);
  const unsigned lo = (unsigned)__builtin_amdgcn_readfirstlane((int)(unsigned)u);
  const unsigned hi = (unsigned)__builtin_amdgcn_readfirstlane((int)(unsigned)(u >> 32));
  return __longlong_as_double((long long)(((unsigned long long)hi << 32) | lo));
}

__device__ __forceinline__ double hk_rhat(unsigned q) {
  unsigned h = q * 0x9E3779B1u + 0x7F4A7C15u;
  h ^= h >> 16;
  h *= 0x85EBCA6Bu;
  h ^= h >> 13;
  h *= 0xC2B2AE35u;
  h ^= h >> 16;
  return (double)(int)h * (1.0 / 2147483648.0);
}

#ifdef AIY_DIAG_PHASES
#define HK_PH(k)                                                        \
  do {                                                                  \
    if (tid == 0 && blockIdx.x >= AIY_DIAG_PHASES && blockIdx.x < AIY_DIAG_PHASES + 10) { \
      const unsigned long long tn = __builtin_amdgcn_s_memrealtime();   \
      if ((k) >= 0) ph[(k)] += tn - tq;                                 \
      tq = tn;                                                          \
    }                                                                   \
  } while (0)
#else
#define HK_PH(k) \
  do {           \
  } while (0)
#endif

template <int SMAX, int KC, int TH>
struct HkShared {
  double* Tacc;
  int* s_base;
  int (*s_pub)[2];
  int* s_tot;
  HcCand (*s_cand)[kHcCand];
  int* s_ncand;
  unsigned short* s_cinfo;
  double* s_P;
  double (*s_part)[TH / kWave];
  double* s_res;
  int* s_flag;
  int* s_stop;
  int* s_ex;
  int* s_nheavy;
  int* s_wcnt;
  int (*s_heavy)[4];
  double* s_hval;
  int* s_rok;
};

struct HkArgs {
  int G, S, n_a, cap, w, j0, j1;
  gptr<const int> LO;
  gptr<const double> WL;
  gptr<double> X;
  gptr<double> Pg;
  gptr<double> Vg;
  gptr<double> slab_cl;
  gptr<int> span_cl;
  gptr<unsigned> ctr;
  gptr<unsigned long long> gran;
  gptr<const double> Pc;
  double tol;
  int max_iter;
  gptr<unsigned> err;
  gptr<const unsigned> stop_ctr;
  unsigned stop_at;
  gptr<double> Qg;
  gptr<int> Ainv;
  bool lottery_fresh;
  unsigned dyn_lds;
};

template <class T>
using lptr = __attribute__((address_space(3))) T*;
__device__ __forceinline__ unsigned hk_lds_addr(double* p) {
  unsigned a = (unsigned)(size_t)(lptr<double>)p;
  asm volatile("" : "+s"(a));
  return a;
}

template <int SMAX, int KC, int TH, bool PULL = false, bool FUSEA = false, int SC = 0>
__device__ __forceinline__ int hk_solve(const HkArgs& r, const HkShared<SMAX, KC, TH>& L, unsigned& nb,
                                        unsigned& ne) {
  constexpr bool kVlds = SMAX <= 8;
#ifdef AIY_DIAG_PHASES
  unsigned long long ph[6] = {0, 0, 0, 0, 0, 0}, tq = 0;
#endif
  double* Tacc = L.Tacc;
  int* s_base = L.s_base;
  int (*s_pub)[2] = L.s_pub;
  HcCand (*s_cand)[kHcCand] = L.s_cand;
  int* s_ncand = L.s_ncand;
  unsigned short* s_cinfo = L.s_cinfo;
  double* s_P = L.s_P;
  double (*s_part)[TH / kWave] = L.s_part;
  double* s_res = L.s_res;
  int& s_flag = *L.s_flag;
  int& s_stop = *L.s_stop;
  int& s_tot = *L.s_tot;

  const int tid = threadIdx.x;
  const int lane = tid & (kWave - 1), wid = tid / kWave;
  static_assert(SC >= 0 && SC <= SMAX, "compile-time state count within SMAX");
  const int G = r.G, S = SC > 0 ? SC : r.S, n_a = r.n_a, cap = r.cap;
  const int w = r.w;
  const int j0 = r.j0;
  const int j1 = r.j1;
  unsigned* ctr = (unsigned*)r.ctr;
  unsigned long long* gran = (unsigned long long*)r.gran;
  const int* LO = (const int*)r.LO;
  const double* WL = (const double*)r.WL;
  double* X = (double*)r.X;
  double* slab_cl = (double*)r.slab_cl;
  const double* __restrict__ Pc = (const double*)r.Pc;
  int* span_cl = (int*)r.span_cl;
  unsigned* err = (unsigned*)r.err;

  for (int q = tid; q < SMAX * SMAX; q += TH) {
    const int s = q / SMAX, sp = q - s * SMAX;
    s_P[q] = (s < S && sp < S) ? Pc[s * S + sp] : 0.0;
  }
  auto barrier = [&]() -> bool {
    ++nb;
    return hc_barrier(err, ctr, (unsigned)G * nb, &s_flag);
  };
  const int n_own = j1 - j0, aspan = n_own + 2;
  int* s_A = reinterpret_cast<int*>(Tacc);
  int* s_ex = L.s_ex;
  int* Ainv = (int*)r.Ainv;
  double* Qg = (double*)r.Qg;
  if constexpr (PULL) {
    const int n1 = n_a + 1;
    unsigned bad = 0u;
    if (r.lottery_fresh) {
      asm volatile("s_waitcnt vmcnt(0)" ::: "memory");
      if (!barrier()) return -1;
    }
    for (int q = tid; q < S * n_own; q += TH) {
      const int s = q / n_own, j = j0 + (q - s * n_own);
      const int l = hc_lo_at(LO, n_a, r.lottery_fresh, s, j);
      const int lp = j > 0 ? hc_lo_at(LO, n_a, r.lottery_fresh, s, j - 1) : -1;
      const bool ok = l >= 0 && l <= n_a - 2 && lp >= -1 && lp <= l;
      if (!ok) {
        bad = 2u;
        continue;
      }
      for (int d = lp + 1; d <= l; ++d)
        __hip_atomic_store(to_global(&Ainv[(size_t)s * n1 + d]), j, __ATOMIC_RELAXED, __HIP_MEMORY_SCOPE_AGENT);
      if (j == n_a - 1)
        for (int d = l + 1; d <= n_a; ++d)
          __hip_atomic_store(to_global(&Ainv[(size_t)s * n1 + d]), n_a, __ATOMIC_RELAXED, __HIP_MEMORY_SCOPE_AGENT);
    }
    if (S * aspan * (int)sizeof(int) > cap * (int)sizeof(double)) bad = 2u;
    if (bad) __hip_atomic_store(to_global(err), bad, __ATOMIC_RELAXED, __HIP_MEMORY_SCOPE_AGENT);
    hc_exported(LO, n_a, r.lottery_fresh, S, j0, j1, s_ex);
    asm volatile("s_waitcnt vmcnt(0)" ::: "memory");
    if (!barrier()) return -1;
    if (hc_failed(err, &s_stop)) return -1;
    for (int q = tid; q < S * aspan; q += TH) {
      const int s = q / aspan, d = j0 - 1 + (q - s * aspan);
      s_A[q] = d < 0 ? 0 : __hip_atomic_load(to_global(&Ainv[(size_t)s * n1 + d]), __ATOMIC_RELAXED,
                                              __HIP_MEMORY_SCOPE_AGENT);
    }
    __syncthreads();
  }
  if (!PULL && tid == 0) {
    int tot = 0;
    unsigned bad = 0;
    for (int s = 0; s < S; ++s) {
      const int f = LO[(size_t)s * n_a + j0];
      const int l = LO[(size_t)s * n_a + j1 - 1] - f + 2;
      if (l < 2 || f < 0 || f + l > n_a) bad = 2u;
      const int ll = l > 0 ? l : 0;
      s_base[s] = tot - f;
      s_pub[2 * s][0] = tot;
      s_pub[2 * s][1] = tot + max(0, min(ll, j0 - f));
      s_pub[2 * s + 1][0] = tot + min(ll, max(0, j1 - f));
      s_pub[2 * s + 1][1] = tot + ll;
      int* sp = &span_cl[((size_t)w * SMAX + s) * 4];
      __hip_atomic_store(to_global(&sp[0]), f, __ATOMIC_RELAXED, __HIP_MEMORY_SCOPE_AGENT);
      __hip_atomic_store(to_global(&sp[1]), ll, __ATOMIC_RELAXED, __HIP_MEMORY_SCOPE_AGENT);
      __hip_atomic_store(to_global(&sp[2]), tot - f, __ATOMIC_RELAXED, __HIP_MEMORY_SCOPE_AGENT);
      tot += ll;
    }
    s_tot = tot;
    *L.s_nheavy = 0;
    if (tot > cap) bad = 2u;
    if (bad) __hip_atomic_store(to_global(err), bad, __ATOMIC_RELAXED, __HIP_MEMORY_SCOPE_AGENT);
    asm volatile("s_waitcnt vmcnt(0)" ::: "memory");
  }
  if (!PULL) {
  if (!barrier()) return -1;
  if (hc_failed(err, &s_stop)) return -1;
  if (tid < S) {
    const int s = tid;
    int n = 0, bad = 0;
    for (int w2 = 0; w2 < G; ++w2) {
      const int* sp = &span_cl[((size_t)w2 * SMAX + s) * 4];
      const int f = __hip_atomic_load(to_global(&sp[0]), __ATOMIC_RELAXED, __HIP_MEMORY_SCOPE_AGENT);
      const int l = __hip_atomic_load(to_global(&sp[1]), __ATOMIC_RELAXED, __HIP_MEMORY_SCOPE_AGENT);
      if (f < j1 && f + l > j0) {
        const int base = __hip_atomic_load(to_global(&sp[2]), __ATOMIC_RELAXED, __HIP_MEMORY_SCOPE_AGENT);
        if (n < kHcCand) s_cand[s][n] = HcCand{w2, f, l, base};
        else bad = 1;
        ++n;
      }
    }
    s_ncand[s] = n < kHcCand ? n : kHcCand;
    if (bad) {
      __hip_atomic_store(to_global(err), 3u, __ATOMIC_RELAXED, __HIP_MEMORY_SCOPE_AGENT);
      asm volatile("s_waitcnt vmcnt(0)" ::: "memory");
    }
  }
  const int total = s_tot;
  for (int q = tid; q < total; q += TH) Tacc[q] = 0.0;
  if (!barrier()) return -1;
  if (hc_failed(err, &s_stop)) return -1;
  }
#pragma unroll
  for (int k = 0; k < KC; ++k) {
    if (PULL) break;
    const int d = j0 + tid + k * TH;
#pragma unroll
    for (int s = 0; s < SMAX; ++s) {
      int cf = 0, cn = 0;
      if (s < S && d < j1) {
        const int nc = s_ncand[s];
        for (int c = 0; c < nc; ++c) {
          const HcCand cd = s_cand[s][c];
          if (d >= cd.first && d < cd.first + cd.len) {
            if (cn == 0) cf = c;
            ++cn;
          }
        }
      }
      const bool heavy = cn > kHkWaveCn;
      const unsigned long long bm = __ballot(heavy);
      if (lane == 0) L.s_wcnt[wid] = __popcll(bm);
      __syncthreads();
      int base = *L.s_nheavy;
      for (int q = 0; q < wid; ++q) base += L.s_wcnt[q];
      int tot = 0;
      for (int q = 0; q < TH / kWave; ++q) tot += L.s_wcnt[q];
      const int e = base + __popcll(bm & ((1ull << lane) - 1ull));
      int hi = kHkHeavy;
      if (heavy && e < kHkHeavy) {
        hi = e;
        L.s_heavy[e][0] = k;
        L.s_heavy[e][1] = s;
        L.s_heavy[e][2] = tid;
        L.s_heavy[e][3] = cf | (cn << 8);
      }
      __syncthreads();
      if (tid == 0) *L.s_nheavy = base + tot;
      s_cinfo[(k * SMAX + s) * TH + tid] = hk_cinfo(cf, cn, hi);
    }
  }
  constexpr bool kLoReg = SMAX <= 8 && KC == 1 && TH <= 512;
  int dreg[KC][kLoReg ? SMAX : 1];
  double wreg[KC][kLoReg ? SMAX : 1];
  if constexpr (kLoReg) {
#pragma unroll
    for (int k = 0; k < KC; ++k) {
      const int j = j0 + tid + k * TH;
#pragma unroll
      for (int s = 0; s < SMAX; ++s) {
        const bool ok = s < S && j < j1;
        dreg[k][s] = ok ? LO[(size_t)s * n_a + j] : -1;
        wreg[k][s] = ok ? WL[(size_t)s * n_a + j] : 0.0;
      }
    }
  }
  const int v_base = lane < S ? s_base[lane] : 0;
  const int v_plo = lane < 2 * S ? s_pub[lane][0] : 0;
  const int v_phi = lane < 2 * S ? s_pub[lane][1] : 0;
  const int jbase = j0 + tid;
  auto col = [&]() {
    int c = jbase;
    asm volatile("" : "+v"(c));
    return c;
  };

  auto push = [&](const double (&q)[KC][SMAX]) {
    constexpr int PR = SMAX <= 8 ? SMAX : 4;
    const int jc = col();
#pragma unroll
    for (int s0 = 0; s0 < SMAX; s0 += PR) {
      if (s0 < S) {
        int dd[KC][PR];
        double ww[KC][PR];
#pragma unroll
        for (int k = 0; k < KC; ++k) {
          const int j = jc + k * TH;
#pragma unroll
          for (int u = 0; u < PR; ++u) {
            const int s = s0 + u;
            if constexpr (kLoReg) {
              dd[k][u] = s < SMAX ? dreg[k][s < SMAX ? s : 0] : -1;
              ww[k][u] = s < SMAX ? wreg[k][s < SMAX ? s : 0] : 0.0;
            } else {
              const bool ok = s < S && j < j1;
              const int q = min(s, S - 1) * n_a + min(j, n_a - 1);
              const int dv = LO[q];
              const double wv = WL[q];
              dd[k][u] = ok ? dv : -1;
              ww[k][u] = ok ? wv : 0.0;
            }
          }
        }
#pragma unroll
        for (int k = 0; k < KC; ++k) {
          const bool act = j0 + tid + k * TH < j1;
#pragma unroll
          for (int u = 0; u < PR; ++u) {
            const int s = s0 + u;
            if (s < S) {
              const int d = dd[k][u];
              const double vlo = ww[k][u] * q[k][s];
              const double vhi = (1.0 - ww[k][u]) * q[k][s];
              const int ilo = __builtin_amdgcn_readlane(v_base, s) + d, ihi = ilo + 1;
              const int d0 = __builtin_amdgcn_readfirstlane(d);
              if (__all(act && d == d0)) {
                const double tl = wave_sum_lane63(vlo), th = wave_sum_lane63(vhi);
                if (lane == kWave - 1) {
                  atomicAdd(&Tacc[ilo], tl);
                  if (th != 0.0) atomicAdd(&Tacc[ihi], th);
                }
              } else if (act) {
                if (vlo != 0.0) atomicAdd(&Tacc[ilo], vlo);
                if (vhi != 0.0) atomicAdd(&Tacc[ihi], vhi);
              }
            }
          }
        }
      }
    }
    __syncthreads();
  };
  auto publish = [&](int par) {
    double* slab = slab_cl + ((size_t)w * 2 + par) * cap;
    for (int rr = 0; rr < 2 * S; ++rr) {
      const int lo = __builtin_amdgcn_readlane(v_plo, rr), hi = __builtin_amdgcn_readlane(v_phi, rr);
      for (int q = lo + tid; q < hi; q += TH) {
        store_f64_agent(&slab[q], Tacc[q]);
        Tacc[q] = 0.0;
      }
    }
    asm volatile("s_waitcnt vmcnt(0)" ::: "memory");
  };
  auto gather_mix = [&](int par, double (&out)[KC][SMAX]) {
    constexpr int GR = 4;
    double T[KC][SMAX];
#pragma unroll
    for (int k = 0; k < KC; ++k)
#pragma unroll
      for (int s = 0; s < SMAX; ++s) T[k][s] = 0.0;
    bool more = false;
#pragma unroll
    for (int s0 = 0; s0 < SMAX; s0 += GR) {
      if (s0 < S) {
        double v0[KC][GR], v1[KC][GR];
        int oq[KC][GR];
#pragma unroll
        for (int k = 0; k < KC; ++k) {
          const int d = j0 + tid + k * TH;
#pragma unroll
          for (int q = 0; q < GR; ++q) {
            const int s = s0 + q;
            v0[k][q] = 0.0;
            v1[k][q] = 0.0;
            oq[k][q] = -1;
            if (s < S) {
              const int ci = s_cinfo[(k * SMAX + s) * TH + tid], cf = hk_cf(ci), cn = hk_cn(ci);
              if (cn >= 1) {
                const HcCand c = s_cand[s][cf];
                if (c.w != w) v0[k][q] = load_f64_agent(&slab_cl[((size_t)c.w * 2 + par) * cap + c.base + d]);
                else oq[k][q] = c.base + d;
              }
              if (cn >= 2) {
                const HcCand c = s_cand[s][cf + 1];
                if (c.w != w) v1[k][q] = load_f64_agent(&slab_cl[((size_t)c.w * 2 + par) * cap + c.base + d]);
                else oq[k][q] = c.base + d;
              }
              more = more || (cn > 2 && hk_hi(ci) == kHkHeavy);
            }
          }
        }
#pragma unroll
        for (int k = 0; k < KC; ++k)
#pragma unroll
          for (int q = 0; q < GR; ++q)
            if (oq[k][q] >= 0) {
              T[k][s0 + q] = Tacc[oq[k][q]];
              Tacc[oq[k][q]] = 0.0;
            }
#pragma unroll
        for (int k = 0; k < KC; ++k)
#pragma unroll
          for (int q = 0; q < GR; ++q) T[k][s0 + q] = (v0[k][q] + v1[k][q]) + T[k][s0 + q];
      }
    }
    const int nh = min(*L.s_nheavy, kHkHeavy);
    if (nh > 0) {
      constexpr int NW = TH / kWave, EPW = (kHkHeavy + NW - 1) / NW;
      double hx[EPW];
#pragma unroll
      for (int i = 0; i < EPW; ++i) {
        const int e = wid + i * NW;
        hx[i] = 0.0;
        if (e < nh) {
          const int ek = L.s_heavy[e][0], es = L.s_heavy[e][1], et = L.s_heavy[e][2], ec = L.s_heavy[e][3];
          const int c = 2 + lane;
          if (c < (ec >> 8)) hx[i] = hc_take(s_cand[es][(ec & 255) + c], w, j0 + et + ek * TH, par, cap, slab_cl, Tacc);
        }
      }
#pragma unroll
      for (int i = 0; i < EPW; ++i) {
        const int e = wid + i * NW;
        if (e < nh) {
          const double sum = wave_sum_lane63(hx[i]);
          if (lane == kWave - 1) L.s_hval[e] = sum;
        }
      }
      __syncthreads();
#pragma unroll
      for (int k = 0; k < KC; ++k)
#pragma unroll
        for (int s = 0; s < SMAX; ++s)
          if (s < S) {
            const int ci = s_cinfo[(k * SMAX + s) * TH + tid];
            if (hk_hi(ci) < kHkHeavy) T[k][s] += L.s_hval[hk_hi(ci)];
          }
    }
    if (__any(more)) {
#pragma unroll
      for (int k = 0; k < KC; ++k) {
        const int d = j0 + tid + k * TH;
        double e2[SMAX], e3[SMAX];
#pragma unroll
        for (int s = 0; s < SMAX; ++s) {
          e2[s] = 0.0;
          e3[s] = 0.0;
          if (s < S) {
            const int ci = s_cinfo[(k * SMAX + s) * TH + tid], cf = hk_cf(ci), cn = hk_cn(ci);
            if (cn > 2 && hk_hi(ci) == kHkHeavy) {
              e2[s] = hc_take(s_cand[s][cf + 2], w, d, par, cap, slab_cl, Tacc);
              if (cn > 3) e3[s] = hc_take(s_cand[s][cf + 3], w, d, par, cap, slab_cl, Tacc);
            }
          }
        }
#pragma unroll
        for (int s = 0; s < SMAX; ++s) T[k][s] += e2[s] + e3[s];
#pragma unroll
        for (int s = 0; s < SMAX; ++s) {
          if (s < S) {
            const int ci = s_cinfo[(k * SMAX + s) * TH + tid], cf = hk_cf(ci), cn = hk_cn(ci);
            if (hk_hi(ci) < kHkHeavy) continue;
            for (int c0 = 4; c0 < cn; c0 += 4) {
              double x[4];
#pragma unroll
              for (int u = 0; u < 4; ++u) {
                const int c = c0 + u;
                x[u] = 0.0;
                if (c < cn) x[u] = hc_take(s_cand[s][cf + c], w, d, par, cap, slab_cl, Tacc);
              }
              T[k][s] += ((x[0] + x[1]) + x[2]) + x[3];
            }
          }
        }
      }
    }
#pragma unroll
    for (int sp = 0; sp < SMAX; ++sp) {
      double pc[SMAX];
      asm volatile("" ::: "memory");
#pragma unroll
      for (int s = 0; s < SMAX; ++s) pc[s] = s_P[s * SMAX + sp];
#pragma unroll
      for (int k = 0; k < KC; ++k) {
        double acc = 0.0;
#pragma unroll
        for (int s = 0; s < SMAX; ++s) acc += pc[s] * T[k][s];
        out[k][sp] = acc;
      }
    }
  };
  auto stage_q = [&](const double (&q)[KC][SMAX]) {
    const int jc = col();
#pragma unroll
    for (int k = 0; k < KC; ++k) {
      const int j = jc + k * TH;
#pragma unroll
      for (int s = 0; s < SMAX; ++s) {
        if (s < S && j < j1) {
          double* p = Qg + (size_t)s * n_a + j;
          if (j < s_ex[2 * s] || j >= s_ex[2 * s + 1]) store_f64_agent(p, q[k][s]);
          else *p = q[k][s];
        }
      }
    }
    asm volatile("s_waitcnt vmcnt(0)" ::: "memory");
  };
  auto w_at = [&](int s, int j) -> double {
    const double* p = WL + (size_t)s * n_a + j;
    return r.lottery_fresh ? load_f64_agent(p) : *p;
  };
  auto q_at = [&](int s, int j) -> double { return load_f64_agent(Qg + (size_t)s * n_a + j); };
  auto pull_mix = [&](double (&out)[KC][SMAX]) {
    const int jc = col();
#pragma unroll
    for (int k = 0; k < KC; ++k) {
      asm volatile("" ::: "memory");
      const int d = jc + k * TH;
      const bool valid = d < j1;
      double T[SMAX];
#pragma unroll
      for (int s = 0; s < SMAX; ++s) T[s] = 0.0;
      constexpr int GRP = SMAX <= 8 ? (KC == 1 ? (SMAX + 1) / 2 : 2) : 4;
#pragma unroll
      for (int s0 = 0; s0 < SMAX; s0 += GRP) {
        if (s0 >= S) break;
        asm volatile("" ::: "memory");
        int a0[GRP], a1[GRP], a2[GRP];
        double wv[GRP][4], qv[GRP][4];
#pragma unroll
        for (int u = 0; u < GRP; ++u) {
          const int sc = min(s0 + u, S - 1);
          const int* As = s_A + sc * aspan - (j0 - 1);
          a0[u] = valid ? min(max(As[d - 1], 0), n_a) : 0;
          a1[u] = valid ? min(max(As[d], a0[u]), n_a) : 0;
          a2[u] = valid ? min(max(As[d + 1], a1[u]), n_a) : 0;
          const int i0 = min(a1[u], n_a - 1), i1 = min(a1[u] + 1, n_a - 1);
          const int i2 = min(a0[u], n_a - 1), i3 = min(a0[u] + 1, n_a - 1);
          wv[u][0] = w_at(sc, i0); qv[u][0] = q_at(sc, i0);
          wv[u][1] = w_at(sc, i1); qv[u][1] = q_at(sc, i1);
          wv[u][2] = w_at(sc, i2); qv[u][2] = q_at(sc, i2);
          wv[u][3] = w_at(sc, i3); qv[u][3] = q_at(sc, i3);
        }
#pragma unroll
        for (int u = 0; u < GRP; ++u) {
          const int sr = s0 + u;
          if (sr < S) {
            const int n1c = a2[u] - a1[u], n0c = a1[u] - a0[u];
            const bool heavy = valid && (n1c + n0c) > kWave;
            double acc = 0.0;
            if (valid && !heavy) {
              if (n1c > 0) acc += wv[u][0] * qv[u][0];
              if (n1c > 1) acc += wv[u][1] * qv[u][1];
              for (int j = a1[u] + 2; j < a2[u]; ++j) acc += w_at(sr, j) * q_at(sr, j);
              if (n0c > 0) acc += (1.0 - wv[u][2]) * qv[u][2];
              if (n0c > 1) acc += (1.0 - wv[u][3]) * qv[u][3];
              for (int j = a0[u] + 2; j < a1[u]; ++j) acc += (1.0 - w_at(sr, j)) * q_at(sr, j);
            }
            unsigned long long hm = __ballot(heavy);
            while (hm) {
              const int h = __builtin_ctzll(hm);
              hm &= hm - 1ull;
              const int b0 = __builtin_amdgcn_readlane(a0[u], h), b1 = __builtin_amdgcn_readlane(a1[u], h),
                        b2 = __builtin_amdgcn_readlane(a2[u], h);
              double pa = 0.0, pb = 0.0;
              for (int j = b1 + lane; j < b2; j += kWave) pa += w_at(sr, j) * q_at(sr, j);
              for (int j = b0 + lane; j < b1; j += kWave) pb += (1.0 - w_at(sr, j)) * q_at(sr, j);
              const double ta = wave_sum_lane63(pa), tb = wave_sum_lane63(pb);
              const double tot = __shfl(ta, kWave - 1, kWave) + __shfl(tb, kWave - 1, kWave);
              if (lane == h) acc = tot;
            }
            T[sr] = acc;
          }
        }
      }
#pragma unroll
      for (int sp = 0; sp < SMAX; ++sp) {
        double pc[SMAX];
        asm volatile("" ::: "memory");
#pragma unroll
        for (int s = 0; s < SMAX; ++s) pc[s] = s_P[s * SMAX + sp];
        double acc = 0.0;
#pragma unroll
        for (int s = 0; s < SMAX; ++s) acc += pc[s] * T[s];
        out[k][sp] = acc;
      }
    }
  };
  auto matvec = [&](const double (&q)[KC][SMAX], double (&out)[KC][SMAX]) -> bool {
    if constexpr (PULL) {
      HK_PH(5);
      stage_q(q);
      HK_PH(1);
      if (!barrier()) return false;
      HK_PH(2);
      pull_mix(out);
      HK_PH(3);
      return true;
    }
    HK_PH(5);
    push(q);
    HK_PH(0);
    const int par = (int)((nb + 1) & 1);
    publish(par);
    HK_PH(1);
    if (!barrier()) return false;
    HK_PH(2);
    gather_mix(par, out);
    HK_PH(3);
    return true;
  };
  auto reduce = [&](double (&vals)[kHcRed], int nv, unsigned kmax, auto&& prefetch) -> bool {
    HK_PH(5);
    hc_wave_parts(vals, nv, kmax, s_part);
    __syncthreads();
    ++ne;
    const unsigned long long tag = hc_red_tag(ne);
    unsigned long long* slot = hc_red_slot(gran, G, ne);
    hc_store_granules<TH>(slot, w, tag, nv, kmax, s_part);
    prefetch();
    if (wid == 0) hc_sweep(slot, G, tag, nv, kmax, s_res, &s_flag, err);
    __syncthreads();
    HK_PH(4);
    return s_flag != 0;
  };
  auto matvec_rp = [&](auto&& do_push, double (&out)[KC][SMAX], const double* vals, int nv, unsigned kmax) -> bool {
    HK_PH(5);
    hc_wave_parts(vals, nv, kmax, s_part);
    do_push();
    HK_PH(0);
    ++ne;
    const unsigned long long tag = hc_red_tag(ne);
    unsigned long long* slot = hc_red_slot(gran, G, ne);
    hc_store_granules<TH>(slot, w, tag, nv, kmax, s_part);
    const int par = (int)((nb + 1) & 1);
    publish(par);
    HK_PH(1);
    if (!barrier()) return false;
    HK_PH(2);
    if (wid == TH / kWave - 1) hc_sweep(slot, G, tag, nv, kmax, s_res, L.s_rok, err);
    gather_mix(par, out);
    __syncthreads();
    HK_PH(3);
    return *L.s_rok != 0;
  };
  auto matvec_r = [&](const double (&q)[KC][SMAX], double (&out)[KC][SMAX], const double* vals, int nv,
                      unsigned kmax) -> bool { return matvec_rp([&] { push(q); }, out, vals, nv, kmax); };
  double rv[KC][SMAX], pv[KC][SMAX], tv[KC][SMAX];
  double* Vl = kVlds ? Tacc + cap : (double*)r.Vg;
  double* Pg = (double*)r.Pg;
  auto vidx = [&](int k, int s) { return (k * SMAX + s) * TH + tid; };
  double part[kHcRed];
  const double tol = r.tol;
  int mv = 0;
  bool restart = true, first = true;
  double rho = 0.0, total0 = 0.0;
  auto own = [&](int jc, int k, int s) { return s < S && jc + k * TH < j1; };
  auto col_act = [&](int jc, bool (&act)[KC]) {
#pragma unroll
    for (int k = 0; k < KC; ++k) act[k] = jc + k * TH < j1;
  };
  bool act[KC];
  unsigned seed = 0;
  auto rh_at = [&](int jc, int k, int s) { return hk_rhat((unsigned)(s * n_a + jc + k * TH) + seed * 0x5BD1E995u); };
  double best = __builtin_inf();
  int mv_best = 0;
  auto gidx = [&](int jc, int k, int s) { return (size_t)s * n_a + jc + k * TH; };
  double* Ug = (double*)r.Qg;
  double pu = 0.0;
  auto make_u = [&]() {
    if constexpr (FUSEA) {
      const int jc = col();
      double acc = 0.0;
#pragma unroll
      for (int k = 0; k < KC; ++k)
#pragma unroll
        for (int s = 0; s < SMAX; ++s) {
          if (own(jc, k, s)) {
            int d;
            double wl;
            if constexpr (kLoReg) {
              d = dreg[k][s];
              wl = wreg[k][s];
            } else {
              d = LO[gidx(jc, k, s)];
              wl = WL[gidx(jc, k, s)];
            }
            double tr = 0.0;
            for (int sp = 0; sp < S; ++sp) {
              const unsigned q = (unsigned)(sp * n_a + d) + seed * 0x5BD1E995u;
              tr += s_P[s * SMAX + sp] * (wl * hk_rhat(q) + (1.0 - wl) * hk_rhat(q + 1u));
            }
            const double u = rh_at(jc, k, s) - tr;
            Ug[gidx(jc, k, s)] = u;
            acc += u * pv[k][s];
          }
        }
      pu = acc;
    }
  };
#ifndef AIY_FUSEA_KC2
#define AIY_FUSEA_KC2 0
#endif
  constexpr bool kUqPre = KC == 1 || AIY_FUSEA_KC2 == 1;
  HK_PH(-1);
  while (true) {
    if (restart) {
      int jc = col();
#pragma unroll
      for (int k = 0; k < KC; ++k)
#pragma unroll
        for (int s = 0; s < SMAX; ++s) {
          const double xv = X[min(s, S - 1) * n_a + min(jc + k * TH, n_a - 1)];
          pv[k][s] = own(jc, k, s) ? xv : 0.0;
        }
      if (!matvec(pv, tv)) return -1;
      ++mv;
      jc = col();
      double rr = 0.0, rm = 0.0, xs = 0.0;
#pragma unroll
      for (int k = 0; k < KC; ++k)
#pragma unroll
        for (int s = 0; s < SMAX; ++s) {
          rv[k][s] = tv[k][s] - pv[k][s];
          if (own(jc, k, s)) {
            rr += rh_at(jc, k, s) * rv[k][s];
            rm = nan_max(rm, fabs(rv[k][s]));
            xs += pv[k][s];
          }
        }
      part[0] = rr;
      part[1] = rm;
      part[2] = xs;
      if (!reduce(part, 3, 2u, [] {})) return -1;
      rho = s_res[0];
      if (mv == 1) total0 = s_res[2];
      if (s_res[1] < tol || mv >= r.max_iter) {
        const double scale = total0 / s_res[2];
#pragma unroll
        for (int k = 0; k < KC; ++k)
#pragma unroll
          for (int s = 0; s < SMAX; ++s)
            if (own(jc, k, s)) X[gidx(jc, k, s)] = mv == 1 ? tv[k][s] : tv[k][s] * scale;
        break;
      }
#pragma unroll
      for (int k = 0; k < KC; ++k)
#pragma unroll
        for (int s = 0; s < SMAX; ++s) pv[k][s] = rv[k][s];
      make_u();
      restart = false;
      first = true;
    }
#pragma unroll
    for (int k = 0; k < KC; ++k)
#pragma unroll
      for (int s = 0; s < SMAX; ++s) Vl[vidx(k, s)] = rv[k][s];
    if (r.stop_ctr != nullptr && tid == 0 && ((mv >> 1) & 7) == 0)
      s_stop = __hip_atomic_load((const unsigned*)r.stop_ctr, __ATOMIC_RELAXED, __HIP_MEMORY_SCOPE_AGENT) >= r.stop_at;
    double xq[KC][SMAX];
    int jc;
    if constexpr (FUSEA) {
      jc = col();
      col_act(jc, act);
      double rm = 0.0;
#pragma unroll
      for (int k = 0; k < KC; ++k) {
        if (act[k]) {
#pragma unroll
          for (int s = 0; s < SMAX; ++s)
            if (s < S) rm = nan_max(rm, fabs(Vl[vidx(k, s)]));
        }
        if constexpr (KC == 1) {
#pragma unroll
          for (int s = 0; s < SMAX; ++s) xq[k][s] = X[min(s, S - 1) * n_a + min(jc + k * TH, n_a - 1)];
        }
      }
      part[0] = pu;
      part[1] = (r.stop_ctr != nullptr && tid == 0 && s_stop) ? kHkStopSentinel : rm;
      if (!matvec_r(pv, tv, part, 2, 2u)) return -1;
      ++mv;
      jc = col();
#pragma unroll
      for (int k = 0; k < KC; ++k)
#pragma unroll
        for (int s = 0; s < SMAX; ++s) {
          const double v = pv[k][s] - tv[k][s];
          rv[k][s] = Vl[vidx(k, s)];
          Vl[vidx(k, s)] = v;
          if constexpr (KC > 1) xq[k][s] = X[min(s, S - 1) * n_a + min(jc + k * TH, n_a - 1)];
        }
    } else {
      if (!matvec(pv, tv)) return -1;
      ++mv;
      jc = col();
      col_act(jc, act);
      double rvv = 0.0, rm = 0.0;
#pragma unroll
      for (int k = 0; k < KC; ++k) {
#pragma unroll
        for (int s = 0; s < SMAX; ++s) {
          tv[k][s] = pv[k][s] - tv[k][s];
          rv[k][s] = Vl[vidx(k, s)];
          Vl[vidx(k, s)] = tv[k][s];
        }
        if (act[k]) {
#pragma unroll
          for (int s = 0; s < SMAX; ++s)
            if (s < S) {
              rvv += rh_at(jc, k, s) * tv[k][s];
              rm = nan_max(rm, fabs(rv[k][s]));
            }
        }
      }
      part[0] = rvv;
      part[1] = (r.stop_ctr != nullptr && tid == 0 && s_stop) ? kHkStopSentinel : rm;
      if (!reduce(part, 2, 2u, [&] {
            const int jq = col();
#pragma unroll
            for (int k = 0; k < KC; ++k)
#pragma unroll
              for (int s = 0; s < SMAX; ++s) xq[k][s] = X[min(s, S - 1) * n_a + min(jq + k * TH, n_a - 1)];
          }))
        return -1;
    }
    if (s_res[1] >= kHkStopSentinel) return -(2 + mv);
    if ((!first && s_res[1] < tol) || mv >= r.max_iter) {
      restart = true;
      continue;
    }
    if (first || s_res[1] < 0.9 * best) {
      best = first ? __builtin_inf() : s_res[1];
      mv_best = mv;
    } else if (mv - mv_best > kHkStall) {
      ++seed;
      best = __builtin_inf();
      restart = true;
      continue;
    }
    first = false;
    const double alpha = rho / s_res[0];
    if (!(fabs(alpha) < 1e300)) {
      restart = true;
      continue;
    }
    jc = col();
    col_act(jc, act);
#pragma unroll
    for (int k = 0; k < KC; ++k) {
      if (act[k]) {
#pragma unroll
        for (int s = 0; s < SMAX; ++s)
          if (s < S) {
            const int g = s * n_a + jc + k * TH;
            X[g] = xq[k][s] + alpha * pv[k][s];
            Pg[g] = pv[k][s];
          }
      }
#pragma unroll
      for (int s = 0; s < SMAX; ++s) rv[k][s] -= alpha * Vl[vidx(k, s)];
    }
    if (!matvec(rv, tv)) return -1;
    ++mv;
    jc = col();
    col_act(jc, act);
    double ts = 0.0, tt = 0.0, rs = 0.0, rt = 0.0, sm = 0.0;
#pragma unroll
    for (int k = 0; k < KC; ++k) {
#pragma unroll
      for (int s = 0; s < SMAX; ++s) tv[k][s] = rv[k][s] - tv[k][s];
      if (act[k]) {
#pragma unroll
        for (int s = 0; s < SMAX; ++s)
          if (s < S) {
            const double h = rh_at(jc, k, s);
            ts += tv[k][s] * rv[k][s];
            tt += tv[k][s] * tv[k][s];
            rs += h * rv[k][s];
            rt += h * tv[k][s];
            sm = nan_max(sm, fabs(rv[k][s]));
          }
      }
    }
    part[0] = ts;
    part[1] = tt;
    part[2] = rs;
    part[3] = rt;
    part[4] = sm;
    double pq[KC][SMAX];
    double uq[FUSEA && kUqPre ? KC : 1][SMAX];
    if (!reduce(part, 5, 16u, [&] {
          const int jq = col();
#pragma unroll
          for (int k = 0; k < KC; ++k)
#pragma unroll
            for (int s = 0; s < SMAX; ++s) {
              const int g = min(s, S - 1) * n_a + min(jq + k * TH, n_a - 1);
              xq[k][s] = X[g];
              pq[k][s] = Pg[g];
              if constexpr (FUSEA && kUqPre) uq[k][s] = Ug[g];
            }
        }))
      return -1;
    double omega = (s_res[4] < tol) ? 0.0 : s_res[0] / s_res[1];
    if (!(fabs(omega) < 1e300)) omega = 0.0;
    if (omega == 0.0) {
      restart = true;
      continue;
    }
    const double rho2 = s_res[2] - omega * s_res[3];
    const double beta = (rho2 / rho) * (alpha / omega);
    rho = rho2;
    jc = col();
    col_act(jc, act);
    double pun = 0.0;
#pragma unroll
    for (int k = 0; k < KC; ++k) {
      if (act[k]) {
#pragma unroll
        for (int s = 0; s < SMAX; ++s)
          if (s < S) X[s * n_a + jc + k * TH] = xq[k][s] + omega * rv[k][s];
      }
#pragma unroll
      for (int s = 0; s < SMAX; ++s) {
        const double pold = (act[k] && s < S) ? pq[k][s] : 0.0;
        rv[k][s] = rv[k][s] - omega * tv[k][s];
        pv[k][s] = rv[k][s] + beta * (pold - omega * Vl[vidx(k, s)]);
      }
      if constexpr (FUSEA && kUqPre) {
        if (act[k]) {
#pragma unroll
          for (int s = 0; s < SMAX; ++s)
            if (s < S) pun += uq[k][s] * pv[k][s];
        }
      }
    }
    if constexpr (FUSEA && !kUqPre) {
      double ul[KC][SMAX];
#pragma unroll
      for (int k = 0; k < KC; ++k)
#pragma unroll
        for (int s = 0; s < SMAX; ++s) ul[k][s] = Ug[min(s, S - 1) * n_a + min(jc + k * TH, n_a - 1)];
#pragma unroll
      for (int k = 0; k < KC; ++k)
#pragma unroll
        for (int s = 0; s < SMAX; ++s)
          if (own(jc, k, s)) pun += ul[k][s] * pv[k][s];
    }
    pu = pun;
    if (!(fabs(beta) < 1e300) || rho == 0.0) restart = true;
  }
#ifdef AIY_DIAG_PHASES
  if (tid == 0 && blockIdx.x >= AIY_DIAG_PHASES && blockIdx.x < AIY_DIAG_PHASES + 10 && mv > 0)
    printf("[bicg phases] block %d G=%d nj=%d matvecs=%d us/matvec: push %.2f publish %.2f barrier %.2f gather+mix "
           "%.2f reduce %.2f vector %.2f\n",
           (int)blockIdx.x, G, j1 - j0, mv, ph[0] * 0.01 / mv, ph[1] * 0.01 / mv, ph[2] * 0.01 / mv, ph[3] * 0.01 / mv,
           ph[4] * 0.01 / mv, ph[5] * 0.01 / mv);
#endif
  return mv;
}

__device__ __forceinline__ int hk_uni(int x) { return __builtin_amdgcn_readfirstlane(x); }
template <class T>
__device__ __forceinline__ gptr<T> hk_uni(gptr<T> p) {
  const unsigned long long u = (unsigned long long)p;
  const unsigned lo = (unsigned)__builtin_amdgcn_readfirstlane((int)(unsigned)u);
  const unsigned hi = (unsigned)__builtin_amdgcn_readfirstlane((int)(unsigned)(u >> 32));
  return (gptr<T>)(((unsigned long long)hi << 32) | lo);
}
__device__ __forceinline__ HkArgs hk_uniform_args(const HkArgs& a) {
  HkArgs u;
  u.G = hk_uni(a.G); u.S = hk_uni(a.S); u.n_a = hk_uni(a.n_a); u.cap = hk_uni(a.cap);
  u.w = hk_uni(a.w); u.j0 = hk_uni(a.j0); u.j1 = hk_uni(a.j1);
  u.LO = hk_uni(a.LO); u.WL = hk_uni(a.WL); u.X = hk_uni(a.X); u.Pg = hk_uni(a.Pg); u.Vg = hk_uni(a.Vg);
  u.slab_cl = hk_uni(a.slab_cl); u.span_cl = hk_uni(a.span_cl); u.ctr = hk_uni(a.ctr); u.gran = hk_uni(a.gran);
  u.Pc = hk_uni(a.Pc);
  u.tol = hk_uni(a.tol);
  u.max_iter = hk_uni(a.max_iter);
  u.err = hk_uni(a.err);
  u.stop_ctr = hk_uni(a.stop_ctr);
  u.stop_at = (unsigned)hk_uni((int)a.stop_at);
  u.Qg = hk_uni(a.Qg); u.Ainv = hk_uni(a.Ainv);
  u.lottery_fresh = hk_uni((int)a.lottery_fresh) != 0;
  u.dyn_lds = (unsigned)hk_uni((int)a.dyn_lds);
  return u;
}

template <int SMAX, int KC, int TH, bool PULL = false, bool FUSEA = false, int SC = 0>
__device__ __noinline__ int hk_solve_isolated(HkArgs a, unsigned* nb_io, unsigned* ne_io);
template <int SMAX, int KC, int TH, bool PULL = false, bool FUSEA = false, int SC = 0>
__device__ __forceinline__ int hk_solve_inlined(HkArgs a, unsigned* nb_io, unsigned* ne_io) {
  extern __shared__ double hk_dyn_in[];
  __shared__ int s_base[SMAX];
  __shared__ int s_pub[2 * SMAX][2];
  __shared__ int s_tot;
  __shared__ HcCand s_cand[SMAX][kHcCand];
  __shared__ int s_ncand[SMAX];
  __shared__ unsigned short s_cinfo[PULL ? 1 : KC * SMAX * TH];
  __shared__ double s_P[SMAX * SMAX];
  __shared__ double s_part[kHcRed][TH / kWave];
  __shared__ double s_res[kHcRed];
  __shared__ int s_flag, s_stop;
  __shared__ int s_ex[2 * SMAX];
  __shared__ int s_nheavy, s_heavy[kHkHeavy][4], s_rok, s_wcnt[TH / kWave];
  __shared__ double s_hval[kHkHeavy];
  HkShared<SMAX, KC, TH> L{hk_dyn_in, s_base, s_pub, &s_tot, s_cand, s_ncand, s_cinfo, s_P, s_part, s_res,
                                 &s_flag, &s_stop, s_ex, &s_nheavy, s_wcnt, s_heavy, s_hval, &s_rok};
  unsigned nb = *nb_io, ne = *ne_io;
  const int mv = hk_solve<SMAX, KC, TH, PULL, FUSEA, SC>(a, L, nb, ne);
  *nb_io = nb;
  *ne_io = ne;
  return mv;
}
template <int SMAX, int KC, int TH, bool PULL, bool FUSEA, int SC>
__device__ __noinline__ int hk_solve_isolated(HkArgs a, unsigned* nb_io, unsigned* ne_io) {
  double* hk_dyn = (double*)(lptr<double>)(size_t)(unsigned)__builtin_amdgcn_readfirstlane((int)a.dyn_lds);
  __shared__ int s_base[SMAX];
  __shared__ int s_pub[2 * SMAX][2];
  __shared__ int s_tot;
  __shared__ HcCand s_cand[SMAX][kHcCand];
  __shared__ int s_ncand[SMAX];
  __shared__ unsigned short s_cinfo[KC * SMAX * TH];
  __shared__ double s_P[SMAX * SMAX];
  __shared__ double s_part[kHcRed][TH / kWave];
  __shared__ double s_res[kHcRed];
  __shared__ int s_flag, s_stop;
  __shared__ int s_ex[2 * SMAX];
  __shared__ int s_nheavy, s_heavy[kHkHeavy][4], s_rok, s_wcnt[TH / kWave];
  __shared__ double s_hval[kHkHeavy];
  HkShared<SMAX, KC, TH> L{hk_dyn, s_base, s_pub, &s_tot, s_cand, s_ncand, s_cinfo, s_P, s_part, s_res,
                                 &s_flag, &s_stop, s_ex, &s_nheavy, s_wcnt, s_heavy, s_hval, &s_rok};
  unsigned nb = *nb_io, ne = *ne_io;
  const int mv = hk_solve<SMAX, KC, TH, PULL, FUSEA, SC>(hk_uniform_args(a), L, nb, ne);
  *nb_io = nb;
  *ne_io = ne;
  return mv;
}

}
```

aiyagari_hark_amd/csrc/internal.h:

```cpp
#pragma once

#include <hip/hip_runtime.h>
#include <rccl/rccl.h>

#include <cstdarg>
#include <cstdio>
#include <cstring>
#include <string>
#include <vector>

#include "../../include/aiyagari.h"
#include "carve.h"
#include "owned.h"

struct aiy_handle {
  int device = 0;
  std::string err;
  aiy::DeviceBuffer egm_dev; aiy::PinnedBuffer egm_pin;
  aiy::DeviceBuffer egm_hint;
  unsigned long long egm_hint_sig = ~0ull;
  aiy::DeviceBuffer egm_aa;
  aiy::DeviceBuffer partials, ticket;
  hipStream_t cap_stream = nullptr;
  bool use_graphs = true;
  aiy::DeviceBuffer hist_dev; aiy::PinnedBuffer hist_pin;
  bool hist_fused = false;
  bool hist_resident = true;
  int hist_cluster_cap = 0;
  int hist_accel = 0;
  int hist_krylov = 0;
  int res_shape_stream = 1;
  int hist_pull = 0;
  int ge_loose_hist = 8;
  const double* egm_tolv = nullptr;
  const double* egm_tolh = nullptr;
  const double* hist_tolv = nullptr;
  int egm_extrap = 0;
  aiy::DeviceBuffer hc, hcd;
  aiy::LaunchTimer hc_timer;
  bool ge_resident = false;
  int cu_limit = 0;
  int ge_rebalance = 55;
  int ge_rounds = 0;
  int ge_mid_stops = 0;
  int ge_extrap_period = 32;
  int ge_anderson = 12;
  int ge_logsec = 2;
  aiy::DeviceBuffer ge;
  aiy::LaunchTimer ge_timer;
  double ge_points = 0.0, ge_egm_cycles = 0.0;
  std::vector<double> ge_prof;
  std::vector<double> ge_evlog;
  aiy::DeviceBuffer stats;
  aiy::DeviceBuffer welf;
  aiy::DeviceBuffer res_sync;
  bool use_resident = true;
  int res_shape = 0;
  aiy::LaunchTimer res_timer;
  long long res_periods = 0;
  unsigned res_epoch = 0;
  const void* res_occ_fn = nullptr;
  size_t res_occ_lds = 0;
  aiy::DeviceBuffer blk_dev; aiy::PinnedBuffer blk_pin;
  bool res_stream = false;
  ncclComm_t comm = nullptr;
  bool comm_owned = false;
  int nranks = 1, rank = 0;
  hipStream_t last_stream = nullptr;
  bool has_last_stream = false;
  aiy::Event hand_ev;
};

int32_t aiy_egm_solve_impl(aiy_handle* h, const aiy_egm_dims* dims, const aiy_egm_inputs* in, double tol,
                           int32_t max_cycles, int32_t chunk, const double* m_init, const double* c_init,
                           double* work_m, double* work_c, double* m_out, double* c_out, int32_t* cycles_out,
                           double* dist_out, aiy_stream stream);

namespace aiy {

int32_t launch_build_index(aiy_handle* h, const double* x, long long n_rows, int n1, int* H, hipStream_t st);
int32_t hist_solve_resident(aiy_handle* h, int n_cal, int S, int n_a, const int* lo, const double* wlo,
                            const double* P, double tol, int max_iter, double* mass, int* d_iters, hipStream_t st);
int32_t hist_resident_plan(aiy_handle* h, int n_cal, int S, int n_a, int* out4);
int32_t ge_stationary_resident(aiy_handle* h, const aiy_stationary_model* M, const aiy_ge_options* o, double* r_out,
                               double* K_out, double* Ks_out, int32_t* steps_out, int32_t* cyc_out,
                               int32_t* its_out, int32_t* status_out, hipStream_t st);

inline int32_t fail(aiy_handle* h, int32_t code, const char* fmt, ...) {
  char buf[512];
  va_list ap;
  va_start(ap, fmt);
  vsnprintf(buf, sizeof(buf), fmt, ap);
  va_end(ap);
  if (h) h->err = buf;
  return code;
}

#define AIY_HIP(h, expr)                                                                 \
  do {                                                                                   \
    hipError_t _e = (expr);                                                              \
    if (_e != hipSuccess)                                                                \
      return aiy::fail((h), AIY_ERR_HIP, "%s failed: %s (%s:%d)", #expr,                \
                       hipGetErrorString(_e), __FILE__, __LINE__);                        \
  } while (0)

#define AIY_CHECK_LAUNCH(h) AIY_HIP(h, hipGetLastError())

inline hipStream_t as_stream(aiy_stream s) { return reinterpret_cast<hipStream_t>(s); }

inline int32_t use_stream(aiy_handle* h, hipStream_t st) {
  if (h->has_last_stream && h->last_stream != st) {
    AIY_HIP(h, h->hand_ev.ensure(hipEventDisableTiming));
    if (hipEventRecord(h->hand_ev.get(), h->last_stream) == hipSuccess) {
      AIY_HIP(h, hipStreamWaitEvent(st, h->hand_ev.get(), 0));
    } else {
      (void)hipGetLastError();
    }
  }
  h->last_stream = st;
  h->has_last_stream = true;
  return AIY_OK;
}
#define AIY_USE_STREAM(h, st)                        \
  do {                                               \
    int32_t _r = aiy::use_stream((h), (st));         \
    if (_r) return _r;                               \
  } while (0)

enum class Admit { fits, not_fits, attr_error, query_error };
inline Admit admit_launch(const void* fn, int threads, size_t lds, bool set_attr, hipError_t* err = nullptr) {
  hipError_t e = hipSuccess;
  Admit a = Admit::fits;
  int per_cu = 0;
  if (set_attr && (e = hipFuncSetAttribute(fn, hipFuncAttributeMaxDynamicSharedMemorySize, (int)lds)) != hipSuccess)
    a = Admit::attr_error;
  else if ((e = hipOccupancyMaxActiveBlocksPerMultiprocessor(&per_cu, fn, threads, lds)) != hipSuccess)
    a = Admit::query_error;
  else if (per_cu < 1)
    a = Admit::not_fits;
  if (e != hipSuccess) (void)hipGetLastError();
  if (err) *err = e;
  return a;
}

template <class Launch>
int32_t time_launches(aiy_handle* h, hipStream_t st, int n, Launch launch, float* ms) {
  std::vector<hipEvent_t> ev(2 * (size_t)n, nullptr);
  int32_t rc = AIY_OK;
  for (auto& e : ev)
    if (hipEventCreate(&e) != hipSuccess) { rc = fail(h, AIY_ERR_HIP, "hipEventCreate failed"); break; }
  for (int k = 0; rc == AIY_OK && k < n; ++k) {
    if (hipEventRecord(ev[2 * k], st) != hipSuccess) rc = fail(h, AIY_ERR_HIP, "hipEventRecord failed");
    launch();
    if (hipGetLastError() != hipSuccess) rc = fail(h, AIY_ERR_HIP, "kernel launch failed");
    if (hipEventRecord(ev[2 * k + 1], st) != hipSuccess) rc = fail(h, AIY_ERR_HIP, "hipEventRecord failed");
  }
  if (rc == AIY_OK && hipStreamSynchronize(st) != hipSuccess) rc = fail(h, AIY_ERR_HIP, "hipStreamSynchronize failed");
  float tot = 0.f;
  for (int k = 0; rc == AIY_OK && k < n; ++k) {
    float t = 0.f;
    if (hipEventElapsedTime(&t, ev[2 * k], ev[2 * k + 1]) != hipSuccess) rc = fail(h, AIY_ERR_HIP, "hipEventElapsedTime failed");
    tot += t;
  }
  for (auto& e : ev)
    if (e) (void)hipEventDestroy(e);
  if (rc == AIY_OK) *ms = tot;
  return rc;
}

}
```

aiyagari_hark_amd/csrc/panel.hip:

```cpp
#include "common.h"
#include "internal.h"
#include "panel_common.h"

#include <algorithm>

namespace aiy {

constexpr int kSimBlock = 256;
constexpr int kSimMaxBlocks = 8192;
constexpr int kTicketGroups = 16;
constexpr int kTicketStride = 32;
constexpr int kGraphPeriods = 64;

struct PanelRun {
  long long n, offset, n_total;
  double* a;
  uint8_t* lab;
  const double* u;
  long long u_ld;
  int u_t0;
  const uint8_t* emp;
  long long emp_ld;
  unsigned long long seed;
  unsigned ge_iter;
// ... 111 lines not shown
  __shared__ int is_last;
#pragma unroll
  for (int o = 32; o > 0; o >>= 1) local += __shfl_down(local, o, kWave);
  if ((threadIdx.x & (kWave - 1)) == 0) red[threadIdx.x / kWave] = local;
  __syncthreads();
  if (threadIdx.x == 0) {
    const double s = (red[0] + red[1]) + (red[2] + red[3]);
    store_f64_agent(&r.partials[blockIdx.x], s);
    asm volatile("s_waitcnt vmcnt(0)" ::: "memory");
    const int nb = (int)gridDim.x;
    const int ng = nb < kTicketGroups ? nb : kTicketGroups;
    const int g = blockIdx.x % kTicketGroups;
    const int gsize = (nb - g + kTicketGroups - 1) / kTicketGroups;
    const unsigned prev = __hip_atomic_fetch_add(to_global(&r.ticket[g * kTicketStride]), 1u, __ATOMIC_RELAXED,
                                                 __HIP_MEMORY_SCOPE_AGENT);
    is_last = 0;
    if (prev == (unsigned)gsize - 1) {
      const unsigned top = __hip_atomic_fetch_add(to_global(&r.ticket[kTicketGroups * kTicketStride]), 1u, __ATOMIC_RELAXED,
                                                  __HIP_MEMORY_SCOPE_AGENT);
      is_last = (top == (unsigned)ng - 1) ? 1 : 0;
    }
  }
  __syncthreads();
  if (!is_last) return;
  double acc = 0.0;
  for (int b = threadIdx.x; b < (int)gridDim.x; b += blockDim.x) acc += load_f64_agent(&r.partials[b]);
#pragma unroll
  for (int o = 32; o > 0; o >>= 1) acc += __shfl_down(acc, o, kWave);
  __syncthreads();
  if ((threadIdx.x & (kWave - 1)) == 0) red[threadIdx.x / kWave] = acc;
  __syncthreads();
  if (threadIdx.x == 0) {
    const double total = (red[0] + red[1]) + (red[2] + red[3]);
    for (int g = 0; g <= kTicketGroups; ++g)
      __hip_atomic_store(to_global(&r.ticket[g * kTicketStride]), 0u, __ATOMIC_RELAXED, __HIP_MEMORY_SCOPE_AGENT);
    if (r.finish) mill(mk, P.mrkv_hist, r.n_total, total, r.sow, r.hist_A, r.hist_M);
    else store_f64_agent(&r.sow[6], total);
  }
}

__global__ void period_price_kernel(aiy_market mk, const int* __restrict__ mrkv_hist, long long n_total, double* sow,
                                    double* hist_A, double* hist_M) {
  if (threadIdx.x != 0) return;
  mill(mk, mrkv_hist, n_total, load_f64_agent(&sow[6]), sow, hist_A, hist_M);
}

__global__ void zero_sum_kernel(double* sow) {
  if (threadIdx.x == 0) store_f64_agent(&sow[6], 0.0);
}

__global__ void set_period_kernel(double* sow, int t) {
  if (threadIdx.x == 0) store_f64_agent(&sow[7], (double)t);
}

static int sim_blocks(long long n) {
  long long nb = (n + (long long)kSimBlock * kAgents - 1) / ((long long)kSimBlock * kAgents);
  return (int)std::max(1LL, std::min<long long>(nb, kSimMaxBlocks));
}

static int32_t ensure_panel_scratch(aiy_handle* h) {
  if (h->cap_stream) return AIY_OK;
  const size_t tk = sizeof(unsigned) * (kTicketGroups + 1) * kTicketStride;
  int32_t rc = h->partials.reserve(h, sizeof(double) * kSimMaxBlocks);
  if (rc == AIY_OK) rc = h->ticket.reserve(h, tk);
  if (rc) return rc;
  AIY_HIP(h, hipMemset(h->ticket.get(), 0, tk));
  AIY_HIP(h, hipStreamCreateWithFlags(&h->cap_stream, hipStreamNonBlocking));
  return AIY_OK;
}

static int32_t enqueue_period(aiy_handle* h, const PanelDev& P, const PanelRun& r, const aiy_market& mk, int nb,
                              hipStream_t st) {
  if (r.n > 0) {
    hipLaunchKernelGGL(sim_period_kernel, dim3(nb), dim3(kSimBlock), 0, st, P, r, mk);
  } else {
    hipLaunchKernelGGL(zero_sum_kernel, dim3(1), dim3(64), 0, st, r.sow);
  }
  if (!r.finish) {
    ncclResult_t e = ncclAllReduce(r.sow + 6, r.sow + 6, 1, ncclDouble, ncclSum, h->comm, st);
    if (e != ncclSuccess) return fail(h, AIY_ERR_COMM, "ncclAllReduce: %s", ncclGetErrorString(e));
    hipLaunchKernelGGL(period_price_kernel, dim3(1), dim3(64), 0, st, mk, P.mrkv_hist, r.n_total, r.sow, r.hist_A,
                       r.hist_M);
  }
  return AIY_OK;
}

}

using namespace aiy;

extern "C" int32_t aiy_sim_periods(aiy_handle* h, const aiy_panel_model* model, const aiy_market* mkt,
                                   int64_t n_local, int64_t agent_offset, int64_t n_total, double* a, uint8_t* lab,
                                   const double* u, int64_t u_ld, const uint8_t* emp, int64_t emp_ld, uint64_t seed,
                                   uint32_t ge_iter, int32_t t0, int32_t n_periods, double* sow, double* hist_A,
                                   double* hist_M, aiy_stream stream) {
  if (!h) return AIY_ERR_ARG;
  if (!model || !mkt || !sow) return fail(h, AIY_ERR_ARG, "null model/market/sow");
  PanelDev P;
  int32_t rc = panel_dev(h, model, P);
  if (rc) return rc;
  if (n_local < 0 || n_total < 1 || agent_offset < 0) return fail(h, AIY_ERR_ARG, "bad agent counts");
  if (n_local > 0 && (!a || !lab)) return fail(h, AIY_ERR_ARG, "null agent arrays");
  if (u && u_ld < n_local) return fail(h, AIY_ERR_ARG, "u_ld < n_local");
  if (emp && emp_ld < n_local) return fail(h, AIY_ERR_ARG, "emp_ld < n_local");
  if (emp && !P.unemployed) return fail(h, AIY_ERR_ARG, "employment states need tables with the unemployed cells");
  if (t0 < 0 || n_periods < 0 || t0 + (int64_t)n_periods > P.act_T)
    return fail(h, AIY_ERR_ARG, "bad period range [%d, %lld) for act_T=%d", t0, (long long)t0 + n_periods, P.act_T);
  if (ge_iter >= (1u << 12)) return fail(h, AIY_ERR_ARG, "ge_iter too large for the Philox counter");
  if (!h->comm && n_local != n_total) return fail(h, AIY_ERR_ARG, "n_local != n_total without a communicator");
  if (n_periods == 0) return AIY_OK;
  AIY_HIP(h, hipSetDevice(h->device));
  rc = ensure_panel_scratch(h);
  if (rc) return rc;
  hipStream_t st = as_stream(stream);
  rc = use_stream(h, st);
  if (rc) return rc;
  const int nb = sim_blocks(n_local);
  PanelRun r;
  r.n = n_local; r.offset = agent_offset; r.n_total = n_total; r.a = a; r.lab = lab; r.u = u; r.u_ld = u_ld;
  r.u_t0 = t0; r.emp = emp; r.emp_ld = emp_ld; r.seed = seed; r.ge_iter = ge_iter; r.sow = sow;
  r.partials = h->partials.as<double>(); r.ticket = h->ticket.as<unsigned>();
  r.hist_A = hist_A; r.hist_M = hist_M; r.finish = h->comm ? 0 : 1;
  const aiy_market mk = *mkt;

  const bool res_ok = h->use_resident && !emp && n_local >= kResMinAgents && resident_supported(P) &&
                      resident_aligned(a, lab);
  if (h->comm && res_ok && (agent_offset & 1) == 0) {
    hipLaunchKernelGGL(set_period_kernel, dim3(1), dim3(64), 0, st, sow, (int)t0);
    for (int p = 0; p < n_periods; ++p) {
      const int fl = kResSharded | (p == 0 ? kResDraw0 : kResPrices | kResKeepTmo) |
                     (p + 1 < n_periods ? kResDrawNext : 0);
      rc = launch_resident(h, P, mk, n_local, a, lab, u ? u + (size_t)p * u_ld : nullptr, u_ld, seed, ge_iter, t0 + p,
                           1, sow, hist_A, hist_M, st, agent_offset, fl, n_total);
      if (rc) return rc;
      const ncclResult_t e = ncclAllReduce(sow + 6, sow + 6, 1, ncclDouble, ncclSum, h->comm, st);
      if (e != ncclSuccess) return fail(h, AIY_ERR_COMM, "ncclAllReduce: %s", ncclGetErrorString(e));
    }
    hipLaunchKernelGGL(period_price_kernel, dim3(1), dim3(64), 0, st, mk, P.mrkv_hist, (long long)n_total, sow,
                       hist_A, hist_M);
    AIY_CHECK_LAUNCH(h);
    return resident_status(h, st, false);
  }
  if (!h->comm && res_ok) {
    hipLaunchKernelGGL(set_period_kernel, dim3(1), dim3(64), 0, st, sow, (int)t0);
    rc = launch_resident(h, P, mk, n_local, a, lab, u, u_ld, seed, ge_iter, t0, n_periods, sow, hist_A, hist_M, st);
    if (rc) return rc;
    AIY_CHECK_LAUNCH(h);
    return resident_status(h, st);
  }
  hipLaunchKernelGGL(set_period_kernel, dim3(1), dim3(64), 0, st, sow, (int)t0);
  int done = 0;
  if (h->use_graphs && !h->comm && n_periods >= 2 * kGraphPeriods) {
    hipGraph_t g = nullptr;
    hipGraphExec_t ge = nullptr;
    AIY_HIP(h, hipStreamBeginCapture(h->cap_stream, hipStreamCaptureModeThreadLocal));
    for (int p = 0; p < kGraphPeriods; ++p) {
      rc = enqueue_period(h, P, r, mk, nb, h->cap_stream);
      if (rc) {
        hipGraph_t junk;
        (void)hipStreamEndCapture(h->cap_stream, &junk);
        return rc;
      }
    }
    AIY_HIP(h, hipStreamEndCapture(h->cap_stream, &g));
    AIY_HIP(h, hipGraphInstantiate(&ge, g, nullptr, nullptr, 0));
    const int reps = n_periods / kGraphPeriods;
    for (int k = 0; k < reps; ++k) AIY_HIP(h, hipGraphLaunch(ge, st));
    done = reps * kGraphPeriods;
    AIY_HIP(h, hipStreamSynchronize(st));
    (void)hipGraphExecDestroy(ge);
    (void)hipGraphDestroy(g);
  }
  for (int p = done; p < n_periods; ++p) {
    rc = enqueue_period(h, P, r, mk, nb, st);
    if (rc) return rc;
  }
  AIY_CHECK_LAUNCH(h);
  return AIY_OK;
}

extern "C" int32_t aiy_sim_period_local(aiy_handle* h, const aiy_panel_model* model, int64_t n_local,
                                        int64_t agent_offset, double* a, uint8_t* lab, const double* u,
                                        const uint8_t* emp, uint64_t seed, uint32_t ge_iter, int32_t t, double* sow,
                                        aiy_stream stream) {
  if (!h) return AIY_ERR_ARG;
  if (!sow) return fail(h, AIY_ERR_ARG, "null sow");
  PanelDev P;
  int32_t rc = panel_dev(h, model, P);
  if (rc) return rc;
  if (n_local < 0 || agent_offset < 0) return fail(h, AIY_ERR_ARG, "bad agent counts");
  if (n_local > 0 && (!a || !lab)) return fail(h, AIY_ERR_ARG, "null agent arrays");
  if (t < 0 || t >= P.act_T) return fail(h, AIY_ERR_ARG, "period t=%d outside [0, act_T=%d)", t, P.act_T);
  if (ge_iter >= (1u << 12)) return fail(h, AIY_ERR_ARG, "ge_iter too large for the Philox counter");
  if (emp && !P.unemployed) return fail(h, AIY_ERR_ARG, "employment states need tables with the unemployed cells");
  AIY_HIP(h, hipSetDevice(h->device));
  rc = ensure_panel_scratch(h);
  if (rc) return rc;
  hipStream_t st = as_stream(stream);
  rc = use_stream(h, st);
  if (rc) return rc;
  PanelRun r;
  r.n = n_local; r.offset = agent_offset; r.n_total = n_local; r.a = a; r.lab = lab; r.u = u; r.u_ld = n_local;
  r.u_t0 = t; r.emp = emp; r.emp_ld = n_local; r.seed = seed; r.ge_iter = ge_iter; r.sow = sow; r.partials = h->partials.as<double>(); r.ticket = h->ticket.as<unsigned>();
  r.hist_A = nullptr; r.hist_M = nullptr; r.finish = 0;
  hipLaunchKernelGGL(set_period_kernel, dim3(1), dim3(64), 0, st, sow, (int)t);
  if (h->use_resident && !emp && n_local >= kResMinAgents && resident_supported(P) && resident_aligned(a, lab) &&
      (agent_offset & 1) == 0) {
    const aiy_market unused{};
    rc = launch_resident(h, P, unused, n_local, a, lab, u, n_local, seed, ge_iter, t, 1, sow, nullptr, nullptr, st,
                         agent_offset, kResSharded | kResDraw0);
    if (rc) return rc;
    AIY_CHECK_LAUNCH(h);
    return resident_status(h, st, false);
  }
  if (n_local > 0) {
    const aiy_market unused{};
    hipLaunchKernelGGL(sim_period_kernel, dim3(sim_blocks(n_local)), dim3(kSimBlock), 0, st, P, r, unused);
  } else {
    hipLaunchKernelGGL(zero_sum_kernel, dim3(1), dim3(64), 0, st, sow);
  }
  AIY_CHECK_LAUNCH(h);
  return AIY_OK;
}

extern "C" int32_t aiy_sim_period_prices(aiy_handle* h, const aiy_panel_model* model, const aiy_market* mkt,
                                         int64_t n_total, int32_t t, double* sow, double* hist_A, double* hist_M,
                                         aiy_stream stream) {
  if (!h) return AIY_ERR_ARG;
  if (!mkt || !sow) return fail(h, AIY_ERR_ARG, "null market/sow");
  PanelDev P;
  int32_t rc = panel_dev(h, model, P);
  if (rc) return rc;
  if (n_total < 1) return fail(h, AIY_ERR_ARG, "n_total < 1");
  if (t < 0 || t >= P.act_T) return fail(h, AIY_ERR_ARG, "period t=%d outside [0, act_T=%d)", t, P.act_T);
  AIY_HIP(h, hipSetDevice(h->device));
  hipStream_t st = as_stream(stream);
  rc = use_stream(h, st);
  if (rc) return rc;
  hipLaunchKernelGGL(period_price_kernel, dim3(1), dim3(64), 0, st, *mkt, P.mrkv_hist, (long long)n_total, sow, hist_A,
                     hist_M);
  AIY_CHECK_LAUNCH(h);
  return AIY_OK;
}

extern "C" int32_t aiy_sim_kernel_time(aiy_handle* h, const aiy_panel_model* model, const aiy_market* mkt,
                                       int64_t n_local, double* a, uint8_t* lab, uint64_t seed, uint32_t ge_iter,
                                       double* sow, int32_t n_launch, float* ms_out, aiy_stream stream) {
  if (!h) return AIY_ERR_ARG;
  if (!model || !mkt || !sow || !a || !lab || !ms_out || n_local < 1 || n_launch < 1)
    return fail(h, AIY_ERR_ARG, "bad arguments");
  PanelDev P;
  int32_t rc = panel_dev(h, model, P);
  if (rc) return rc;
  if (n_launch > P.act_T) return fail(h, AIY_ERR_ARG, "n_launch=%d > act_T=%d", n_launch, P.act_T);
  AIY_HIP(h, hipSetDevice(h->device));
  rc = ensure_panel_scratch(h);
  if (rc) return rc;
  hipStream_t st = as_stream(stream);
  rc = use_stream(h, st);
  if (rc) return rc;
  PanelRun r;
  r.n = n_local; r.offset = 0; r.n_total = n_local; r.a = a; r.lab = lab; r.u = nullptr; r.u_ld = 0; r.u_t0 = 0;
  r.emp = nullptr; r.emp_ld = 0; r.seed = seed; r.ge_iter = ge_iter; r.sow = sow; r.partials = h->partials.as<double>(); r.ticket = h->ticket.as<unsigned>();
  r.hist_A = nullptr; r.hist_M = nullptr; r.finish = 1;
  const int nb = sim_blocks(n_local);
  hipLaunchKernelGGL(set_period_kernel, dim3(1), dim3(64), 0, st, sow, 0);
  AIY_CHECK_LAUNCH(h);
  if (h->use_resident && n_local >= kResMinAgents && resident_supported(P) &&
      resident_aligned(a, lab)) {
    rc = time_launches(h, st, 1,
                       [&] {
                         (void)launch_resident(h, P, *mkt, n_local, a, lab, nullptr, 0, seed, ge_iter, 0, n_launch, sow,
                                               nullptr, nullptr, st);
                       },
                       ms_out);
    if (rc) return rc;
    return resident_status(h, st);
  }
  return time_launches(h, st, n_launch,
                       [&] { hipLaunchKernelGGL(sim_period_kernel, dim3(nb), dim3(kSimBlock), 0, st, P, r, *mkt); },
                       ms_out);
}

extern "C" int32_t aiy_set_option(aiy_handle* h, int32_t option, int64_t value) {
  if (!h) return AIY_ERR_ARG;
  switch (option) {
    case AIY_OPT_USE_GRAPHS: h->use_graphs = value != 0; return AIY_OK;
    case AIY_OPT_RESIDENT:
      h->use_resident = value != 0;
      return AIY_OK;
    case AIY_OPT_RESIDENT_SHAPE:
      if (value < 0 || value > 2) return fail(h, AIY_ERR_ARG, "AIY_OPT_RESIDENT_SHAPE must be 0, 1 or 2");
      h->res_shape = (int)value;
      return AIY_OK;
    case AIY_OPT_HIST_FUSED: h->hist_fused = value != 0; return AIY_OK;
    case AIY_OPT_RESIDENT_STREAM: h->res_stream = value != 0; return AIY_OK;
    case AIY_OPT_HIST_RESIDENT: h->hist_resident = value != 0; return AIY_OK;
    case AIY_OPT_HIST_ACCEL:
      if (value < 0 || value > (1 << 20)) return fail(h, AIY_ERR_ARG, "AIY_OPT_HIST_ACCEL must be >= 0");
      h->hist_accel = (int)value;
      return AIY_OK;
    case AIY_OPT_HIST_KRYLOV: h->hist_krylov = value != 0; return AIY_OK;
    case AIY_OPT_HIST_PULL: h->hist_pull = value != 0; return AIY_OK;
    case AIY_OPT_RESIDENT_SHAPE_STREAM:
      if (value < -1 || value > 2) return fail(h, AIY_ERR_ARG, "AIY_OPT_RESIDENT_SHAPE_STREAM must be -1, 0, 1 or 2");
      h->res_shape_stream = (int)value;
      return AIY_OK;
    case AIY_OPT_GE_LOOSE_HIST:
      if (value < 6 || value > 14) return fail(h, AIY_ERR_ARG, "AIY_OPT_GE_LOOSE_HIST must be in [6, 14]");
      h->ge_loose_hist = (int)value;
      return AIY_OK;
    case AIY_OPT_GE_RESIDENT: h->ge_resident = value != 0; return AIY_OK;
    case AIY_OPT_GE_LOGSEC:
      if (value < 0 || value > 2) return fail(h, AIY_ERR_ARG, "AIY_OPT_GE_LOGSEC must be 0, 1 or 2");
      h->ge_logsec = (int)value;
      return AIY_OK;
    case AIY_OPT_GE_EXTRAP_PERIOD:
      if (value < 4 || value > 1024) return fail(h, AIY_ERR_ARG, "AIY_OPT_GE_EXTRAP_PERIOD must be in [4, 1024]");
      h->ge_extrap_period = (int)value;
      return AIY_OK;
    case AIY_OPT_GE_ANDERSON:
      if (value != 0 && (value < 5 || value > 1024))
        return fail(h, AIY_ERR_ARG, "AIY_OPT_GE_ANDERSON must be 0 or in [5, 1024]");
      h->ge_anderson = (int)value;
      return AIY_OK;
    case AIY_OPT_GE_REBALANCE:
      if (value < 0 || value > 100) return fail(h, AIY_ERR_ARG, "AIY_OPT_GE_REBALANCE must be in [0, 100]");
      h->ge_rebalance = (int)value;
      return AIY_OK;
    case AIY_OPT_CU_LIMIT:
      if (value < 0 || value > 65536) return fail(h, AIY_ERR_ARG, "AIY_OPT_CU_LIMIT must be in [0, 65536]");
      h->cu_limit = (int)value;
      return AIY_OK;
    case AIY_OPT_HIST_CLUSTER:
      if (value < 0 || value > 128) return fail(h, AIY_ERR_ARG, "AIY_OPT_HIST_CLUSTER must be in [0, 128]");
      h->hist_cluster_cap = (int)value;
      return AIY_OK;
    default: return fail(h, AIY_ERR_ARG, "unknown option %d", option);
  }
}

extern "C" int32_t aiy_get_option(aiy_handle* h, int32_t option, int64_t* value) {
  if (!h || !value) return AIY_ERR_ARG;
  switch (option) {
    case AIY_OPT_USE_GRAPHS: *value = h->use_graphs; return AIY_OK;
    case AIY_OPT_RESIDENT: *value = h->use_resident; return AIY_OK;
    case AIY_OPT_RESIDENT_SHAPE: *value = h->res_shape; return AIY_OK;
    case AIY_OPT_HIST_FUSED: *value = h->hist_fused; return AIY_OK;
    case AIY_OPT_RESIDENT_STREAM: *value = h->res_stream; return AIY_OK;
    case AIY_OPT_HIST_RESIDENT: *value = h->hist_resident; return AIY_OK;
    case AIY_OPT_HIST_ACCEL: *value = h->hist_accel; return AIY_OK;
    case AIY_OPT_HIST_KRYLOV: *value = h->hist_krylov; return AIY_OK;
    case AIY_OPT_HIST_PULL: *value = h->hist_pull; return AIY_OK;
    case AIY_OPT_RESIDENT_SHAPE_STREAM: *value = h->res_shape_stream; return AIY_OK;
    case AIY_OPT_GE_LOOSE_HIST: *value = h->ge_loose_hist; return AIY_OK;
    case AIY_OPT_GE_RESIDENT: *value = h->ge_resident; return AIY_OK;
    case AIY_OPT_GE_LOGSEC: *value = h->ge_logsec; return AIY_OK;
    case AIY_OPT_GE_EXTRAP_PERIOD: *value = h->ge_extrap_period; return AIY_OK;
    case AIY_OPT_GE_ANDERSON: *value = h->ge_anderson; return AIY_OK;
    case AIY_OPT_GE_REBALANCE: *value = h->ge_rebalance; return AIY_OK;
    case AIY_OPT_CU_LIMIT: *value = h->cu_limit; return AIY_OK;
    case AIY_OPT_HIST_CLUSTER: *value = h->hist_cluster_cap; return AIY_OK;
    default: return fail(h, AIY_ERR_ARG, "unknown option %d", option);
  }
}
```

aiyagari_hark_amd/stationary.py:

```python
from __future__ import annotations

import atexit
import ctypes
import math
from dataclasses import dataclass, field

import numpy as np
import torch

from . import _lib
from . import setup_math as sm
from .egm import EgmBatch, egm_solve

F64 = torch.float64

TABLE2_RHO = (0.0, 0.3, 0.6, 0.9)
TABLE2_SIGMA = (0.2, 0.4)
TABLE2_CRRA = (1.0, 3.0, 5.0)


@dataclass
class Calibration:
    LaborAR: float = 0.6
    LaborSD: float = 0.2
    CRRA: float = 1.0
    DiscFac: float = 0.96
    CapShare: float = 0.36
    DeprFac: float = 0.08
    LaborStatesNo: int = 7
    income: str = "tauchen"

    def income_process(self):
        if self.income == "tauchen":
            y, P = sm.labor_tauchen(self.LaborStatesNo, self.LaborAR, self.LaborSD)
        elif self.income == "rouwenhorst":
            y, P = sm.rouwenhorst(self.LaborStatesNo, self.LaborAR, self.LaborSD)
        else:
            raise ValueError(self.income)
        return sm.labor_levels(y), P


def table2_calibrations(**kw):
    return [Calibration(LaborAR=r, LaborSD=s, CRRA=c, **kw)
            for s in TABLE2_SIGMA for r in TABLE2_RHO for c in TABLE2_CRRA]


def _resolve_device(device):
    dev = torch.device(device if device is not None else "cuda")
    if dev.type != "cuda":
        raise ValueError(f"stationary solves run on a GPU, not {dev}")
    if dev.index is None:
        dev = torch.device("cuda", torch.cuda.current_device())
    return dev


def firm_prices(r, alpha, delta):
    r, alpha, delta = np.broadcast_arrays(np.asarray(r, dtype=np.float64), np.asarray(alpha, dtype=np.float64),
                                          np.asarray(delta, dtype=np.float64))
    KtoL = np.empty(r.shape)
    w = np.empty(r.shape)
    for i in np.ndindex(r.shape):
        a = float(alpha[i])
        k = math.pow(a / (float(r[i]) + float(delta[i])), 1.0 / (1.0 - a))
        KtoL[i] = k
        w[i] = (1.0 - a) * math.pow(k, a)
    if KtoL.ndim == 0:
        return float(w), float(KtoL)
    return w, KtoL


@dataclass
class StationaryResult:
    r: np.ndarray
    K: np.ndarray
    K_supply: np.ndarray
    KtoY: np.ndarray
    saving_rate: np.ndarray
    bisection_steps: int
    egm_cycles: list = field(default_factory=list)
    hist_iters: list = field(default_factory=list)
    status: np.ndarray | None = None


class StationaryBatch:

    def __init__(self, cals, aGrid, device=None):
        self.cals = list(cals)
        self.device = _resolve_device(device)
        n_cal = len(self.cals)
        levels, Ps = zip(*(c.income_process() for c in self.cals))
        S = len(levels[0])
        if any(len(l) != S for l in levels):
            raise ValueError("all calibrations of a batch need the same number of income states")
        self.S = S
        self.n_a = int(np.asarray(aGrid).shape[-1])
        self.aGrid = np.broadcast_to(np.asarray(aGrid, dtype=np.float64), (n_cal, self.n_a)).copy()
        self.levels = np.stack(levels)
        self.P = np.stack(Ps)
        dev = self.device
        self.d_a = torch.as_tensor(self.aGrid).to(dev)
        self.d_P = torch.as_tensor(self.P).to(dev)
        self.d_lab = torch.as_tensor(self.levels).to(dev)
        self.d_beta = torch.as_tensor([c.DiscFac for c in self.cals], dtype=F64).to(dev)
        self.d_crra = torch.as_tensor([c.CRRA for c in self.cals], dtype=F64).to(dev)
        self.alpha = np.array([c.CapShare for c in self.cals])
        self.delta = np.array([c.DeprFac for c in self.cals])
        shp = (n_cal, S, self.n_a)
        self.lo = torch.empty(shp, dtype=torch.int32, device=dev)
        self.wlo = torch.empty(shp, dtype=F64, device=dev)
        self.mass = torch.empty(shp, dtype=F64, device=dev)
        self.work = torch.empty((2,) + shp, dtype=F64, device=dev)

    def capital_supply(self, r, egm_tol=1e-8, hist_tol=1e-12, max_hist=200000, warm=False, warm_egm=False,
                       accel=0):
        n_cal, S = len(self.cals), self.S
        r = np.asarray(r, dtype=np.float64)
        w, _ = firm_prices(r, self.alpha, self.delta)
        R = 1.0 + r
        dev = self.device
        Rn = torch.as_tensor(np.repeat(R[:, None, None], S, axis=2)).to(dev)
        Wn = torch.as_tensor(np.repeat(w[:, None, None], S, axis=2)).to(dev)
        batch = EgmBatch(self.d_a, torch.zeros((n_cal, 1), dtype=F64, device=dev), self.d_P, Rn, Wn,
                         torch.zeros_like(Rn), self.d_lab, self.d_beta, self.d_crra)
        init = self.last_tables if (warm_egm and getattr(self, "last_tables", None) is not None) else None
        m, c, cycles, _ = egm_solve(batch, tol=egm_tol, init=init)
        h = _lib.handle(dev.index)
        dR = torch.as_tensor(R).to(dev)
        dw = torch.as_tensor(w).to(dev)
        sp = _lib.stream_ptr()
        h.check(h.lib.aiy_hist_lottery(h.h, n_cal, S, self.n_a, _lib.ptr(m), _lib.ptr(c), _lib.ptr(self.d_a),
                                       _lib.ptr(dR), _lib.ptr(dw), _lib.ptr(self.d_lab), _lib.ptr(self.lo),
                                       _lib.ptr(self.wlo), sp), "aiy_hist_lottery")
        if not (warm and getattr(self, "_mass_valid", False)):
            self.mass.fill_(1.0 / (S * self.n_a))
        K = (ctypes.c_double * n_cal)()
        iters = (ctypes.c_int32 * n_cal)()
        h.check(h.lib.aiy_set_option(h.h, _lib.AIY_OPT_HIST_ACCEL, max(int(accel), 0)), "aiy_set_option")
        h.check(h.lib.aiy_set_option(h.h, _lib.AIY_OPT_HIST_KRYLOV, int(accel < 0)), "aiy_set_option")
        try:
            h.check(h.lib.aiy_hist_solve(h.h, n_cal, S, self.n_a, _lib.ptr(self.lo), _lib.ptr(self.wlo),
                                         _lib.ptr(self.d_P), _lib.ptr(self.d_a), float(hist_tol), int(max_hist), 64,
                                         _lib.ptr(self.mass), _lib.ptr(self.work), K, iters, sp), "aiy_hist_solve")
        finally:
            h.check(h.lib.aiy_set_option(h.h, _lib.AIY_OPT_HIST_ACCEL, 0), "aiy_set_option")
            h.check(h.lib.aiy_set_option(h.h, _lib.AIY_OPT_HIST_KRYLOV, 0), "aiy_set_option")
        self.last_tables = (m, c)
        self._mass_valid = True
        return np.array(K[:]), np.array(cycles), np.array(iters[:])


class _Brent:

    def __init__(self, lo, hi, xtol):
        self.lo, self.hi, self.flo, self.fhi, self.xtol = lo, hi, None, None, xtol
        self.brent = False
        self.done = False
        self.x = 0.5 * (lo + hi)

    def propose(self):
        return self.x

    def update(self, f):
        if self.done:
            return
        if not self.brent:
            if f > 0:
                self.hi, self.fhi = self.x, f
            else:
                self.lo, self.flo = self.x, f
            if self.hi - self.lo <= self.xtol:
                self.done, self.x = True, 0.5 * (self.lo + self.hi)
                return
            if self.flo is None or self.fhi is None:
                self.x = 0.5 * (self.lo + self.hi)
                return
            self.brent = True
            self.xpre, self.fpre, self.xcur, self.fcur = self.lo, self.flo, self.hi, self.fhi
            self.xblk = self.fblk = self.spre = self.scur = 0.0
            self._step()
            return
        self.xpre, self.fpre = self.xprev_eval, self.fprev_eval
        self.fcur = f
        self._step()

    def _step(self):
        xpre, fpre, xcur, fcur = self.xpre, self.fpre, self.xcur, self.fcur
        xblk, fblk, spre, scur = self.xblk, self.fblk, self.spre, self.scur
        if fpre * fcur < 0:
            xblk, fblk = xpre, fpre
            spre = scur = xcur - xpre
        if abs(fblk) < abs(fcur):
            xpre, xcur, xblk = xcur, xblk, xcur
            fpre, fcur, fblk = fcur, fblk, fcur
        delta = 0.5 * (self.xtol + 4 * np.finfo(float).eps * abs(xcur))
        sbis = 0.5 * (xblk - xcur)
        if fcur == 0 or abs(sbis) < delta:
            self.done, self.x = True, xcur
            return
        if abs(spre) > delta and abs(fcur) < abs(fpre):
            if xpre == xblk:
                stry = -fcur * (xcur - xpre) / (fcur - fpre)
            else:
                dpre = (fpre - fcur) / (xpre - xcur)
                dblk = (fblk - fcur) / (xblk - xcur)
                stry = -fcur * (fblk * dblk - fpre * dpre) / (dblk * dpre * (fblk - fpre))
            if 2 * abs(stry) < min(abs(spre), 3 * abs(sbis) - delta):
                spre, scur = scur, stry
            else:
                spre = scur = sbis
        else:
            spre = scur = sbis
        self.xprev_eval, self.fprev_eval = xcur, fcur
        xcur = xcur + (scur if abs(scur) > delta else (delta if sbis > 0 else -delta))
        self.xpre, self.fpre, self.xcur, self.fcur = xpre, fpre, xcur, fcur
        self.xblk, self.fblk, self.spre, self.scur = xblk, fblk, spre, scur
        self.x = xcur


def resident_plan(device, n_cal, S, n_a, cu_share=1.0):
    dev = _resolve_device(device)
    h = _lib.handle(dev.index)
    prev = h.set_options({_lib.AIY_OPT_GE_RESIDENT: 1, _lib.AIY_OPT_CU_LIMIT: _cu_limit(dev, cu_share)})
    out = (ctypes.c_int32 * 4)()
    try:
        ok = h.lib.aiy_ge_resident_plan(h.h, int(n_cal), int(S), int(n_a), out)
    finally:
        h.set_options(prev)
    return tuple(out) if ok == 1 else None


def _cu_limit(dev, cu_share):
    return 0 if float(cu_share) >= 1.0 else _device_cus(dev, cu_share)


def ge_stationary_native(b, method, r_tol, egm_tol, hist_tol, max_steps, warm_hist, warm_egm, accel, r_lo=None,
                         r_hi=None, secant=False, loose=False, extrapolate=False, handle=None, stream=None,
                         resident=False, cu_share=1.0):
    n = len(b.cals)
    h = handle if handle is not None else _lib.handle(b.device.index)
    work = torch.empty(int(h.lib.aiy_ge_stationary_work_bytes(n, b.S, b.n_a)), dtype=torch.uint8, device=b.device)
    host = lambda x: (ctypes.c_double * n)(*[float(v) for v in x])
    alpha, delta = host(b.alpha), host(b.delta)
    disc = host([c.DiscFac for c in b.cals])
    model = _lib.StationaryModel(n, b.S, b.n_a, _lib.ptr(b.d_a), _lib.ptr(b.d_P), _lib.ptr(b.d_lab),
                                 _lib.ptr(b.d_beta), _lib.ptr(b.d_crra), ctypes.addressof(alpha),
                                 ctypes.addressof(delta), ctypes.addressof(disc))
    lo = host(np.broadcast_to(np.asarray(r_lo, float), (n,))) if r_lo is not None else None
    hi = host(np.broadcast_to(np.asarray(r_hi, float), (n,))) if r_hi is not None else None
    opt = _lib.GeOptions({"bisect": 0, "brent": 1}[method], float(r_tol), float(egm_tol), float(hist_tol),
                         int(max_steps), 5000, 200000, int(bool(warm_hist)), int(bool(warm_egm)), int(accel),
                         ctypes.addressof(lo) if lo is not None else None,
                         ctypes.addressof(hi) if hi is not None else None, int(bool(secant)), int(bool(loose)),
                         int(bool(extrapolate)), None)
    status = (ctypes.c_int32 * n)()
    opt.status_out = ctypes.addressof(status)
    r, K, Ks = (ctypes.c_double * n)(), (ctypes.c_double * n)(), (ctypes.c_double * n)()
    steps, cyc, its = ctypes.c_int32(), ctypes.c_int32(), ctypes.c_int32()
    prev = h.set_options({_lib.AIY_OPT_GE_RESIDENT: int(bool(resident)),
                          _lib.AIY_OPT_CU_LIMIT: _cu_limit(b.device, cu_share)})
    try:
        h.check(h.lib.aiy_ge_stationary(h.h, ctypes.byref(model), ctypes.byref(opt), _lib.ptr(work), r, K, Ks,
                                        ctypes.byref(steps), ctypes.byref(cyc), ctypes.byref(its),
                                        _lib.stream_ptr(stream)),
                "aiy_ge_stationary")
    finally:
        h.set_options(prev)
    return (np.array(r[:]), np.array(K[:]), np.array(Ks[:]), int(steps.value), int(cyc.value), int(its.value),
            np.array(status[:], dtype=np.int32))


_GROUP_CTX = {}
_GROUP_CARRY_OPTIONS = (_lib.AIY_OPT_GE_LOGSEC, _lib.AIY_OPT_GE_REBALANCE, _lib.AIY_OPT_GE_EXTRAP_PERIOD,
                        _lib.AIY_OPT_HIST_PULL, _lib.AIY_OPT_GE_LOOSE_HIST, _lib.AIY_OPT_GE_ANDERSON)


def _close_groups():
    while _GROUP_CTX:
        _, (h, _) = _GROUP_CTX.popitem()
        h.close()


atexit.register(_close_groups)


def _device_cus(dev, cu_share=1.0):
    cus = torch.cuda.get_device_properties(dev).multi_processor_count
    return max(1, int(cus * float(cu_share)))


def _solve_groups(cals, aGrid, dev, groups, method, r_tol, egm_tol, hist_tol, max_steps, warm_hist, warm_egm, accel,
                  r_lo, r_hi, secant, loose, extrapolate, cu_share=1.0):
    from concurrent.futures import ThreadPoolExecutor
    n = len(cals)
    idx = [list(range(g, n, groups)) for g in range(groups)]
    idx = [i for i in idx if i]
    cus = _device_cus(dev, cu_share)
    cap = max(1, min(32, cus // n))
    cur = torch.cuda.current_stream(dev)
    shared = _lib.handle(dev.index)
    carry = {o: shared.get_option(o) for o in _GROUP_CARRY_OPTIONS}
    jobs = []
    for gi, ii in enumerate(idx):
        key = (dev.index, gi)
        if key not in _GROUP_CTX:
            _GROUP_CTX[key] = (_lib.Handle(dev.index), torch.cuda.Stream(dev))
        h, st = _GROUP_CTX[key]
        h.set_options({**carry, _lib.AIY_OPT_HIST_CLUSTER: cap})
        b = StationaryBatch([cals[i] for i in ii], aGrid, device=dev)
        sub = lambda x: None if x is None else np.broadcast_to(np.asarray(x, float), (n,))[ii]
        st.wait_stream(cur)
        jobs.append((ii, b, h, st, sub(r_lo), sub(r_hi)))

    def run(job):
        ii, b, h, st, lo, hi = job
        with torch.cuda.stream(st):
            return ge_stationary_native(b, method, r_tol, egm_tol, hist_tol, max_steps, warm_hist, warm_egm, accel,
                                        lo, hi, secant=secant, loose=loose, extrapolate=extrapolate, handle=h,
                                        stream=st)
    with ThreadPoolExecutor(max_workers=len(jobs)) as ex:
        outs = list(ex.map(run, jobs))
    for _, _, _, st, _, _ in jobs:
        cur.wait_stream(st)
    r, K, Ks = np.zeros(n), np.zeros(n), np.zeros(n)
    status = np.zeros(n, dtype=np.int32)
    steps = cyc = its = 0
    for (ii, b, *_), (rg, Kg, Ksg, sg, cg, ig, stg) in zip(jobs, outs):
        r[ii], K[ii], Ks[ii], status[ii] = rg, Kg, Ksg, stg
        steps, cyc, its = max(steps, sg), cyc + cg, its + ig
    alpha = np.array([c.CapShare for c in cals])
    delta = np.array([c.DeprFac for c in cals])
    KtoY = K ** (1.0 - alpha)
    return StationaryResult(r=r, K=K, K_supply=Ks, KtoY=KtoY, saving_rate=delta * KtoY, bisection_steps=steps,
                            egm_cycles=[np.array([cyc])], hist_iters=[np.array([its])], status=status)


def solve_table2(cals=None, n_a=10000, aMin=0.001, aMax=50.0, aNestFac=2, r_tol=1e-7, egm_tol=1e-8,
                 hist_tol=1e-12, device=None, r_lo=None, r_hi=None, max_steps=60, log=None, warm_hist=True,
                 method="bisect", warm_egm=None, accel=None, engine="native", secant=None, loose=None,
                 extrapolate=None, groups=None, cu_share=1.0, resident=None):
    cals = table2_calibrations() if cals is None else list(cals)
    device = _resolve_device(device)
    aGrid = sm.make_grid_exp_mult(aMin, aMax, n_a, aNestFac)
    if warm_egm is None:
        warm_egm = method == "brent"
    if accel is None:
        accel = -1 if method == "brent" else 0
    if secant is None:
        secant = method == "brent"
    if loose is None:
        loose = method == "brent"
    if extrapolate is None:
        extrapolate = method == "brent"
    if resident is None:
        resident = (engine == "native" and log is None and accel < 0 and
                    resident_plan(device, len(cals), cals[0].LaborStatesNo, n_a, cu_share) is not None)
    resident = bool(resident) and engine == "native" and log is None
    if resident:
        groups = 1
    if groups is None:
        groups = 3 if (method == "brent" and engine == "native" and log is None and len(cals) >= 3) else 1
    if groups > 1:
        S0 = cals[0].LaborStatesNo
        g_min = -(-n_a // (512 * (2 if S0 <= 8 else 1)))
        if g_min * len(cals) > _device_cus(device, cu_share):
            groups = 1
    if engine == "native" and log is None and groups > 1 and len(cals) > 1:
        return _solve_groups(cals, aGrid, device, int(groups), method, r_tol, egm_tol,
                             hist_tol, max_steps, warm_hist, warm_egm, accel, r_lo, r_hi,
                             secant and warm_hist and warm_egm, loose, extrapolate, cu_share)
    b = StationaryBatch(cals, aGrid, device=device)
    n = len(cals)
    lo = np.full(n, -0.5 * b.delta) if r_lo is None else np.broadcast_to(np.asarray(r_lo, float), (n,)).copy()
    hi = (1.0 / np.array([c.DiscFac for c in cals]) - 1.0 - 1e-9) if r_hi is None else \
        np.broadcast_to(np.asarray(r_hi, float), (n,)).copy()
    steps = 0
    cyc_log, it_log = [], []
    Ks = np.zeros(n)
    if engine == "native" and log is None:
        r, K, Ks, steps, cyc_sum, it_sum, status = ge_stationary_native(b, method, r_tol, egm_tol, hist_tol, max_steps,
                                                                warm_hist, warm_egm, accel, r_lo if r_lo is not None
                                                                else None, r_hi if r_hi is not None else None,
                                                                secant=secant and warm_hist and warm_egm,
                                                                loose=loose, extrapolate=extrapolate,
                                                                resident=resident, cu_share=cu_share)
        KtoY = K ** (1.0 - b.alpha)
        return StationaryResult(r=r, K=K, K_supply=Ks, KtoY=KtoY, saving_rate=b.delta * KtoY, bisection_steps=steps,
                                egm_cycles=[np.array([cyc_sum])], hist_iters=[np.array([it_sum])], status=status)
    if method == "brent":
        search = [_Brent(lo[k], hi[k], r_tol) for k in range(n)]
        while not all(sr.done for sr in search) and steps < max_steps:
            x = np.array([sr.propose() for sr in search])
            Ks, cycles, iters = b.capital_supply(x, egm_tol=egm_tol, hist_tol=hist_tol, warm=warm_hist and steps > 0,
                                                 warm_egm=warm_egm and steps > 0, accel=accel)
            _, Kd = firm_prices(x, b.alpha, b.delta)
            for k, sr in enumerate(search):
                sr.update(float(Ks[k] - Kd[k]))
            steps += 1
            cyc_log.append(cycles)
            it_log.append(iters)
            if log is not None:
                log.append(dict(step=steps, r=x.copy(), Ks=Ks.copy(), Kd=Kd.copy()))
        r = np.array([sr.propose() for sr in search])
    elif method == "bisect":
        while np.any(hi - lo > r_tol) and steps < max_steps:
            mid = 0.5 * (lo + hi)
            Ks, cycles, iters = b.capital_supply(mid, egm_tol=egm_tol, hist_tol=hist_tol,
                                                 warm=warm_hist and steps > 0, warm_egm=warm_egm and steps > 0,
                                                 accel=accel)
            _, Kd = firm_prices(mid, b.alpha, b.delta)
            up = Ks > Kd
            hi = np.where(up, mid, hi)
            lo = np.where(up, lo, mid)
            steps += 1
            cyc_log.append(cycles)
            it_log.append(iters)
            if log is not None:
                log.append(dict(step=steps, r=mid.copy(), Ks=Ks.copy(), Kd=Kd.copy()))
        r = 0.5 * (lo + hi)
    else:
        raise ValueError(f"method {method!r}")
    _, K = firm_prices(r, b.alpha, b.delta)
    KtoY = K ** (1.0 - b.alpha)
    return StationaryResult(r=r, K=K, K_supply=Ks, KtoY=KtoY, saving_rate=b.delta * KtoY, bisection_steps=steps,
                            egm_cycles=cyc_log, hist_iters=it_log)
```

include/aiyagari.h:

```cpp
#ifndef AIYAGARI_H
#define AIYAGARI_H

#include <stdint.h>

#ifdef __cplusplus
extern "C" {
#endif

#define AIY_OK 0
#define AIY_ERR_ARG (-1)
#define AIY_ERR_HIP (-2)
#define AIY_ERR_STATE (-3)
#define AIY_ERR_UNSUPPORTED (-4)
#define AIY_ERR_COMM (-5)

#define AIY_MAX_STATES 64

typedef struct aiy_handle aiy_handle;
typedef void* aiy_stream;

typedef struct {
  int32_t n_cal;
  int32_t S;
  int32_t n_M;
  int32_t n_a;
} aiy_egm_dims;

typedef struct {
  const double* a_grid;
  const double* M_grid;
  const double* P;
  const double* R_next;
  const double* W_next;
  const double* M_next;
  const double* lab;
  const double* beta;
  const double* crra;
} aiy_egm_inputs;

int32_t aiy_version(void);

int32_t aiy_create(int32_t device, aiy_handle** out);
int32_t aiy_destroy(aiy_handle* h);
const char* aiy_last_error(const aiy_handle* h);

int32_t aiy_egm_step(aiy_handle* h, const aiy_egm_dims* dims, const aiy_egm_inputs* in,
                     const double* m_next, const double* c_next, double* m_out, double* c_out,
                     aiy_stream stream);

int32_t aiy_egm_solve(aiy_handle* h, const aiy_egm_dims* dims, const aiy_egm_inputs* in, double tol,
                      int32_t max_cycles, int32_t chunk, double* work_m, double* work_c,
                      double* m_out, double* c_out, int32_t* cycles_out, double* dist_out,
                      aiy_stream stream);

int32_t aiy_egm_solve_from(aiy_handle* h, const aiy_egm_dims* dims, const aiy_egm_inputs* in, double tol,
                           int32_t max_cycles, int32_t chunk, const double* m_init, const double* c_init,
                           double* work_m, double* work_c, double* m_out, double* c_out, int32_t* cycles_out,
                           double* dist_out, aiy_stream stream);

int32_t aiy_egm_kernel_time(aiy_handle* h, const aiy_egm_dims* dims, const aiy_egm_inputs* in,
                            const double* m_next, const double* c_next, double* m_out, double* c_out,
                            int32_t n_launch, float* ms_out, aiy_stream stream);

int32_t aiy_policy_eval(aiy_handle* h, int32_t S, int32_t n_M, int32_t n_a, const double* m_tab,
                        const double* c_tab, const double* M_grid, const int32_t* state,
                        const double* m, const double* M, int64_t n, double* c_out, aiy_stream stream);

int32_t aiy_index_ints_per_row(void);
int32_t aiy_build_index(aiy_handle* h, int64_t n_rows, int32_t n1, const double* x, int32_t* index,
                        aiy_stream stream);


typedef struct {
  double cap_share;
  double depr_fac;
  double prod[2];
  double agg_L[2];
} aiy_market;

typedef struct {
  int32_t S, n_M, n_a, n_lab;
  const void* tables;
  const double* M_grid;
  const double* lab_level;
  const double* lab_cdf;
  const int32_t* mrkv_hist;
  int32_t act_T;
  int32_t unemployed;
} aiy_panel_model;

int64_t aiy_panel_table_bytes(int32_t n_lab, int32_t n_M, int32_t n_a, int32_t unemployed);
int32_t aiy_panel_build(aiy_handle* h, int32_t n_cal, int32_t S, int32_t n_M, int32_t n_a, int32_t n_lab,
                        int32_t unemployed, const double* m_pol, const double* c_pol, void* tables,
                        aiy_stream stream);

#define AIY_SOW_DOUBLES 8

int32_t aiy_sim_periods(aiy_handle* h, const aiy_panel_model* model, const aiy_market* mkt,
                        int64_t n_local, int64_t agent_offset, int64_t n_total, double* a,
                        uint8_t* lab, const double* u, int64_t u_ld, const uint8_t* emp, int64_t emp_ld,
                        uint64_t seed, uint32_t ge_iter, int32_t t0, int32_t n_periods, double* sow,
                        double* hist_A, double* hist_M, aiy_stream stream);

int32_t aiy_sim_period_local(aiy_handle* h, const aiy_panel_model* model, int64_t n_local,
                             int64_t agent_offset, double* a, uint8_t* lab, const double* u,
                             const uint8_t* emp, uint64_t seed, uint32_t ge_iter, int32_t t, double* sow,
                             aiy_stream stream);
int32_t aiy_sim_period_prices(aiy_handle* h, const aiy_panel_model* model, const aiy_market* mkt,
                              int64_t n_total, int32_t t, double* sow, double* hist_A, double* hist_M,
                              aiy_stream stream);

int32_t aiy_get_shocks(aiy_handle* h, int32_t n_lab, const double* lab_cdf, int64_t n, int64_t agent_offset,
                       uint8_t* lab, const double* u, uint64_t seed, uint32_t ge_iter, int32_t t,
                       aiy_stream stream);
int32_t aiy_get_states(aiy_handle* h, const double* lab_level, int64_t n, double Rnow, double Wnow,
                       const double* a_prev, const uint8_t* lab, const uint8_t* emp, double* m_out,
                       aiy_stream stream);
int32_t aiy_get_controls(aiy_handle* h, int32_t S, int32_t n_M, int32_t n_a, const double* m_tab,
                         const double* c_tab, const double* M_grid_host, int32_t Mrkv, double Mnow, int64_t n,
                         const double* m, const uint8_t* lab, const uint8_t* emp, double* c_out,
                         aiy_stream stream);
int32_t aiy_get_poststates(aiy_handle* h, int64_t n, const double* m, const double* c, double* a_out,
                           aiy_stream stream);
int32_t aiy_sum(aiy_handle* h, const double* x, int64_t n, double* out, aiy_stream stream);

int32_t aiy_sim_kernel_time(aiy_handle* h, const aiy_panel_model* model, const aiy_market* mkt,
                            int64_t n_local, double* a, uint8_t* lab, uint64_t seed, uint32_t ge_iter,
                            double* sow, int32_t n_launch, float* ms_out, aiy_stream stream);

int32_t aiy_panel_launch_stats(aiy_handle* h, double* ms_sum, int64_t* launches, int64_t* periods,
                               int32_t reset);

typedef struct {
  int32_t n_cal, S, n_M, n_a, n_lab;
  const void* tables;
  const double* M_grid;
  const double* lab_level;
  const double* lab_cdf;
  const int32_t* mrkv_hist;
  int32_t unemployed;
} aiy_panel_batch;

int32_t aiy_sim_block_max_agents(void);

int32_t aiy_sim_block_periods(aiy_handle* h, const aiy_panel_batch* model, const aiy_market* markets,
                              int64_t n_agents, double* a, uint8_t* lab, const double* u,
                              const uint8_t* emp, const uint64_t* seeds, uint32_t ge_iter, int32_t t0, int32_t n_periods,
                              int32_t act_T, double* sow, double* hist_A, double* hist_M,
                              aiy_stream stream);

#define AIY_OPT_USE_GRAPHS 1
#define AIY_OPT_RESIDENT 2
#define AIY_OPT_HIST_FUSED 4
#define AIY_OPT_RESIDENT_SHAPE 3
#define AIY_OPT_RESIDENT_STREAM 5
#define AIY_OPT_HIST_RESIDENT 6
#define AIY_OPT_HIST_CLUSTER 7
#define AIY_OPT_HIST_ACCEL 8
#define AIY_OPT_HIST_KRYLOV 9
#define AIY_OPT_GE_RESIDENT 10
#define AIY_OPT_CU_LIMIT 11
#define AIY_OPT_GE_REBALANCE 12
#define AIY_OPT_GE_EXTRAP_PERIOD 13
#define AIY_OPT_GE_ANDERSON 23
#define AIY_OPT_GE_LOGSEC 14
#define AIY_OPT_HIST_PULL 15
#define AIY_OPT_GE_LOOSE_HIST 17
#define AIY_OPT_RESIDENT_SHAPE_STREAM 18
int32_t aiy_set_option(aiy_handle* h, int32_t option, int64_t value);
int32_t aiy_get_option(aiy_handle* h, int32_t option, int64_t* value);

int32_t aiy_comm_unique_id(void* out128);
int32_t aiy_comm_init(aiy_handle* h, const void* unique_id128, int32_t nranks, int32_t rank);
int32_t aiy_comm_bind(aiy_handle* h, void* comm);
int32_t aiy_comm_destroy(aiy_handle* h);
int32_t aiy_allreduce_sum(aiy_handle* h, double* buf, int64_t n, aiy_stream stream);


int32_t aiy_hist_lottery(aiy_handle* h, int32_t n_cal, int32_t S, int32_t n_a, const double* m_tab,
                         const double* c_tab, const double* a_grid, const double* R, const double* w,
                         const double* lab, int32_t* lo, double* wlo, aiy_stream stream);

int32_t aiy_hist_solve(aiy_handle* h, int32_t n_cal, int32_t S, int32_t n_a, const int32_t* lo,
                       const double* wlo, const double* P, const double* a_grid, double tol,
                       int32_t max_iter, int32_t chunk, double* mass, double* work, double* K_out,
                       int32_t* iters_out, aiy_stream stream);


typedef struct {
  int32_t n_cal, S, n_a;
  const double* a_grid;
  const double* P;
  const double* lab;
  const double* beta;
  const double* crra;
  const double* alpha;
  const double* delta;
  const double* disc;
} aiy_stationary_model;

typedef struct {
  int32_t method;
  double r_tol;
  double egm_tol;
  double hist_tol;
  int32_t max_steps, max_egm_cycles, max_hist_iter;
  int32_t warm_hist;
  int32_t warm_egm;
  int32_t accel;
  const double* r_lo;
  const double* r_hi;
  int32_t secant_start;
  int32_t loose_bracket;
  int32_t egm_extrapolate;
  int32_t* status_out;
} aiy_ge_options;

int64_t aiy_ge_stationary_work_bytes(int32_t n_cal, int32_t S, int32_t n_a);

int32_t aiy_ge_stationary(aiy_handle* h, const aiy_stationary_model* model, const aiy_ge_options* opt,
                          void* work, double* r_out, double* K_out, double* Ks_out, int32_t* steps_out,
                          int32_t* egm_cycles_out, int32_t* hist_iters_out, aiy_stream stream);

int32_t aiy_ge_resident_plan(aiy_handle* h, int32_t n_cal, int32_t S, int32_t n_a, int32_t* out4);

int32_t aiy_ge_launch_stats(aiy_handle* h, double* ms_sum, int64_t* launches, double* point_matvecs,
                            double* egm_cycles, int32_t reset);

int32_t aiy_ge_last_profile(aiy_handle* h, double* out, int32_t n_cal);
int32_t aiy_ge_last_eval_log(aiy_handle* h, double* out, int32_t n_cal);

int32_t aiy_ge_last_rounds(aiy_handle* h, int32_t* launches, int32_t* mid_solve_stops);

int32_t aiy_hist_launch_stats(aiy_handle* h, double* ms_sum, int64_t* launches, int32_t reset);


typedef struct {
  int32_t n_cal, S, n_a, T;
  const double* a_grid;
  const double* P;
  const double* lab;
  const double* beta;
  const double* crra;
  const double* R;
  const double* w;
  const double* m_term;
  const double* c_term;
} aiy_transition_model;

int64_t aiy_transition_work_bytes(int32_t n_cal, int32_t S, int32_t n_a, int32_t T);

int32_t aiy_transition_backward(aiy_handle* h, const aiy_transition_model* model, void* work, int32_t* lo,
                                double* wlo, double* m0_out, double* c0_out, aiy_stream stream);

int32_t aiy_transition_forward(aiy_handle* h, int32_t n_cal, int32_t S, int32_t n_a, int32_t T,
                               const int32_t* lo, const double* wlo, const double* P, const double* a_grid,
                               const double* R, const double* w, const double* lab, void* work, double* mass,
                               double* Ks_out, double* C_out, aiy_stream stream);

int32_t aiy_transition_forward_marginals(aiy_handle* h, int32_t n_cal, int32_t S, int32_t n_a, int32_t T,
                                         const int32_t* lo, const double* wlo, const double* P,
                                         const double* a_grid, const double* R, const double* w, const double* lab,
                                         void* work, double* mass, double* Ks_out, double* C_out, double* marg_out,
                                         aiy_stream stream);



int64_t aiy_jacobian_work_bytes(int32_t n_cal, int32_t S, int32_t n_a, int32_t T);

int32_t aiy_jacobian_fanout(aiy_handle* h, int32_t n_cal, int32_t S, int32_t n_a, int32_t T, int32_t n_t,
                            const int32_t* lo, const double* wlo, const double* P, const double* mass,
                            void* work, double* out, aiy_stream stream);

int32_t aiy_jacobian_diff(aiy_handle* h, int64_t n, double* shocked, const double* ghost, double step,
                          aiy_stream stream);

int32_t aiy_jacobian_expectation(aiy_handle* h, int32_t n_cal, int32_t S, int32_t n_a, int32_t T,
                                 const int32_t* lo, const double* wlo, const double* P, const double* a_grid,
                                 void* work, double* E_out, aiy_stream stream);

int32_t aiy_jacobian_contract(aiy_handle* h, int32_t n_cal, int32_t S, int32_t n_a, int32_t T, const double* E,
                              const double* dD_R, const double* dD_w, void* work, double* F_out,
                              aiy_stream stream);


int32_t aiy_lottery_mean(aiy_handle* h, int32_t n_cal, int32_t S, int32_t n_a, int32_t n_t, const int32_t* lo,
                         const double* wlo, const double* a_grid, double* out, aiy_stream stream);

int32_t aiy_aggregate_lotteries(aiy_handle* h, int32_t n_cal, int32_t S, int32_t n_a, int32_t T, int32_t n_p,
                                const double* a_star, const double* dA_R, const double* dA_w, const double* X,
                                const double* a_grid, int32_t* lo_out, double* wlo_out, aiy_stream stream);


int32_t aiy_wealth_stats(aiy_handle* h, const double* data, const double* weights, int64_t n,
                         const double* pctiles, int32_t n_p, double* lorenz_out, double* pctl_out,
                         aiy_stream stream);



int64_t aiy_dist_stats_work_bytes(int32_t n_dist, int32_t n_a);

int32_t aiy_dist_marginal(aiy_handle* h, int32_t n_dist, int32_t S, int32_t n_a, const double* mass, double* g,
                          aiy_stream stream);

int32_t aiy_dist_stats(aiy_handle* h, int32_t n_dist, int32_t n_grid, int32_t n_a, const double* g,
                       const double* a_grid, const double* pctiles, int32_t n_p, void* work, double* lorenz_out,
                       double* pctl_out, double* summary_out, aiy_stream stream);



int64_t aiy_value_work_bytes(int32_t n_cal, int32_t S, int32_t n_a);

int32_t aiy_value_backward(aiy_handle* h, int32_t n_cal, int32_t S, int32_t n_a, int32_t T, const int32_t* lo,
                           const double* wlo, const double* P, const double* a_grid, const double* R,
                           const double* w, const double* lab, const double* beta, const double* crra,
                           const double* V_term, void* work, double* V0_out, double* V_path_out,
                           aiy_stream stream);

int32_t aiy_value_stationary(aiy_handle* h, int32_t n_cal, int32_t S, int32_t n_a, const int32_t* lo,
                             const double* wlo, const double* P, const double* a_grid, const double* R,
                             const double* w, const double* lab, const double* beta, const double* crra,
                             const double* beta_host, double tol, int32_t max_iter, int32_t chunk, double* V,
                             void* work, int32_t* iters_out, double* dist_out, aiy_stream stream);

int32_t aiy_value_reduce(aiy_handle* h, int32_t n_cal, int32_t S, int32_t n_a, const double* mass,
                         const double* V, double* W_out, aiy_stream stream);

int32_t aiy_consumption_equivalent(aiy_handle* h, int32_t n_cal, int64_t per, const double* V_new,
                                   const double* V_base, const double* beta, const double* crra, double* g_out,
                                   aiy_stream stream);

#ifdef __cplusplus
}
#endif

#endif
```

Baseline: 633.3.

## Exploit IID income shocks to collapse EGM expectations and histogram solve

At runtime the kernel checks whether every row of the transition matrix P is identical (IID shocks). If so, the EGM backward step computes the expectation and consumption once and reuses it for all income states, and the BiCGStab stationary-distribution solve switches to a reduced form. That form keeps a single asset-marginal vector per column instead of S state vectors and recovers the state split from the stationary probabilities. This cuts the per-matvec mixing work and register and memory footprint, at the cost of a large new specialised solver path, a shared LDS struct refactor, and an extra per-calibration flag copy back to the host.

```diff
diff --git a/aiyagari_hark_amd/_lib.py b/aiyagari_hark_amd/_lib.py
--- a/aiyagari_hark_amd/_lib.py
+++ b/aiyagari_hark_amd/_lib.py
@@ -33,6 +33,7 @@
 AIY_OPT_GE_LOOSE_HIST = 17
 AIY_OPT_RESIDENT_SHAPE_STREAM = 18
 AIY_OPT_GE_ANDERSON = 23
+AIY_OPT_HIST_IID = 24
 
 c_double_p = ctypes.POINTER(ctypes.c_double)
 c_int32_p = ctypes.POINTER(ctypes.c_int32)
@@ -145,6 +146,7 @@
     "aiy_ge_last_profile": (ctypes.c_int32, [vp, c_double_p, ctypes.c_int32]),
     "aiy_ge_last_eval_log": (ctypes.c_int32, [vp, c_double_p, ctypes.c_int32]),
     "aiy_ge_last_rounds": (ctypes.c_int32, [vp, ctypes.POINTER(ctypes.c_int32), ctypes.POINTER(ctypes.c_int32)]),
+    "aiy_ge_last_iid_cells": (ctypes.c_int32, [vp, ctypes.POINTER(ctypes.c_int32)]),
     "aiy_ge_launch_stats": (ctypes.c_int32, [vp, c_double_p, ctypes.POINTER(ctypes.c_int64), c_double_p, c_double_p,
                                              ctypes.c_int32]),
     "aiy_ge_stationary_work_bytes": (ctypes.c_int64, [ctypes.c_int32, ctypes.c_int32, ctypes.c_int32]),
diff --git a/aiyagari_hark_amd/csrc/ge_resident.hip b/aiyagari_hark_amd/csrc/ge_resident.hip
--- a/aiyagari_hark_amd/csrc/ge_resident.hip
+++ b/aiyagari_hark_amd/csrc/ge_resident.hip
@@ -25,6 +25,10 @@
 #define AIY_FUSEA_KC2 0
 #endif
 constexpr bool kGeFuseAKc2 = AIY_FUSEA_KC2 != 0;
+#ifndef AIY_IID_FUSEA_KC2
+#define AIY_IID_FUSEA_KC2 0
+#endif
+constexpr bool kGeIidFuseAKc2 = AIY_IID_FUSEA_KC2 != 0;
 template <int NW>
 constexpr size_t ge_egm_lds() { return (size_t)NW * (8 * kTile + 4 * kWin) * sizeof(double); }
 
@@ -46,6 +50,8 @@
   int max_steps, max_cyc, max_hist;
   int warm_hist, warm_egm, secant, loose, extrap;
   int extrap_period;
+  int iid_on;
+  int* out_iid;
   int aa_period;
   double* aah;
   int logsec;
@@ -185,7 +191,7 @@
                                                const double* src_m, const double* src_c, double* dst_m,
                                                double* dst_c, bool track, double R, double beta, double gam,
                                                const double* s_Wl, const double* s_Pe, int* s_hint,
-                                               double* lds_v, double* lds_win, double* ring) {
+                                               double* lds_v, double* lds_win, double* ring, bool iid) {
   const int tid = threadIdx.x, lane = tid & (kWave - 1);
   const int wv = __builtin_amdgcn_readfirstlane(tid / kWave);
   const int n1 = n_a + 1;
@@ -202,11 +208,14 @@
         const double c = (R * a + s_Wl[sp]) * 1.0;
         Vw[sp * kTile + lane] = R * marg_u<PK>(c, gam);
       }
+      double c = 0.0;
       for (int s = 0; s < S; ++s) {
-        double sum;
-        if constexpr (SC > 0) sum = pairwise_dot<SC>(Vw + lane, s_Pe + s * SC);
-        else sum = np_pairwise_sum<SMAX>(S, [&](int t) { return Vw[t * kTile + lane] * uniform_f64(s_Pe[s * S + t]); });
-        const double c = inv_marg<PK>(beta * sum, gam);
+        if (s == 0 || !iid) {
+          double sum;
+          if constexpr (SC > 0) sum = pairwise_dot<SC>(Vw + lane, s_Pe + s * SC);
+          else sum = np_pairwise_sum<SMAX>(S, [&](int t) { return Vw[t * kTile + lane] * uniform_f64(s_Pe[s * S + t]); });
+          c = inv_marg<PK>(beta * sum, gam);
+        }
         store_f64_agent(&dst_m[(size_t)s * n1 + j + 1], a + c);
         store_f64_agent(&dst_c[(size_t)s * n1 + j + 1], c);
         if (ring) store_f64_agent(&ring[(size_t)s * n_a + j], c);
@@ -229,16 +238,19 @@
     }
   };
   auto end = [&](int, int j, double a) {
+    double c = 0.0, m = 0.0;
 #pragma unroll
     for (int s = 0; s < NP; ++s) {
       if (s < S) {
         __builtin_amdgcn_sched_barrier(0);
-        double sum;
-        if constexpr (SC > 0) sum = pairwise_dot<SC>(Vw + lane, s_Pe + s * SC);
-        else sum = np_pairwise_sum<SMAX>(S, [&](int t) { return Vw[t * kTile + lane] * uniform_f64(s_Pe[s * S + t]); });
-        const double E = beta * sum;
-        const double c = inv_marg<PK>(E, gam);
-        const double m = a + c;
+        if (s == 0 || !iid) {
+          double sum;
+          if constexpr (SC > 0) sum = pairwise_dot<SC>(Vw + lane, s_Pe + s * SC);
+          else sum = np_pairwise_sum<SMAX>(S, [&](int t) { return Vw[t * kTile + lane] * uniform_f64(s_Pe[s * S + t]); });
+          const double E = beta * sum;
+          c = inv_marg<PK>(E, gam);
+          m = a + c;
+        }
         store_f64_agent(&dst_m[(size_t)s * n1 + j + 1], m);
         store_f64_agent(&dst_c[(size_t)s * n1 + j + 1], c);
         if (ring) store_f64_agent(&ring[(size_t)s * n_a + j], c);
@@ -273,9 +285,9 @@
 __device__ __forceinline__ double ge_egm_cycle_fn(int S, int n_a, int j0, int j1, const double* a_grid,
                                                const double* src_m, const double* src_c, double* dst_m,
                                                double* dst_c, bool track, double R, double beta, double gam,
-                                               double* dyn, double* ring) {
+                                               double* dyn, double* ring, bool iid) {
   return ge_egm_cycle<SMAX, SC, PK, NW>(S, n_a, j0, j1, a_grid, src_m, src_c, dst_m, dst_c, track, R, beta, gam,
-                                        ge_s_Wl, ge_s_Pe, ge_s_hint, dyn, dyn + (size_t)NW * SMAX * kTile, ring);
+                                        ge_s_Wl, ge_s_Pe, ge_s_hint, dyn, dyn + (size_t)NW * SMAX * kTile, ring, iid);
 }
 
 template <int SMAX, int NW>
@@ -329,6 +341,7 @@
   double beta, gam;
   size_t tab_sz;
   int j0, j1, w, G, S, n_a, cal, lc;
+  int iid;
   __device__ __forceinline__ double* tabm(int b) const { return tab + (size_t)b * 2 * tab_sz; }
   __device__ __forceinline__ double* tabc(int b) const { return tab + (size_t)b * 2 * tab_sz + tab_sz; }
 };
@@ -486,7 +499,7 @@
       const bool track = n >= 2;
       double* ring = aa && ge_ring_wanted(n, g.aa_period) ? ge_ring(cx, n) : nullptr;
       const double dl = ge_egm_cycle_fn<SMAX, SC, PK, NW>(cx.S, cx.n_a, cx.j0, cx.j1, cx.a_grid, sm, sc, cx.tabm(b_dst),
-                                                          cx.tabc(b_dst), track, R, cx.beta, cx.gam, dyn, ring);
+                                                          cx.tabc(b_dst), track, R, cx.beta, cx.gam, dyn, ring, cx.iid != 0);
       const int xp = g.extrap_period;
       const bool want_value = ext && n >= xp - 1 && ((n % xp) == xp - 1 || (n % xp) == 0);
       double dclu = 0.0;
@@ -552,7 +565,7 @@
   gptr<unsigned long long> gran;
   gptr<const double> a_grid, init_m, init_c;
   double beta, gam, R;
-  int j0, j1, w, G, S, n_a;
+  int j0, j1, w, G, S, n_a, iid;
   GeHhOpt opt;
   unsigned dyn_lds;
 };
@@ -574,6 +587,7 @@
   cx.S = SC > 0 ? SC : hk_uni(a.S);
   cx.n_a = hk_uni(a.n_a);
   cx.cal = cx.lc = 0;
+  cx.iid = hk_uni(a.iid);
   cx.tab_sz = (size_t)cx.S * (cx.n_a + 1);
   const GeHhOpt opt = {hk_uni(a.opt.max_cyc), hk_uni(a.opt.aa_period), hk_uni(a.opt.extrap_period)};
   unsigned nb = *nb_io, ne = *ne_io;
@@ -694,6 +708,13 @@
     st.nbc = 0u;
   }
   __syncthreads();
+  {
+    int iid = g.iid_on != 0 && S >= 2;
+    for (int q = S; q < S * S; ++q)
+      iid &= __double_as_longlong(ge_s_Pe[q]) == __double_as_longlong(ge_s_Pe[q % S]);
+    cx.iid = __builtin_amdgcn_readfirstlane(iid);
+  }
+  if (w == 0 && tid == 0) g.out_iid[cal] = (!PULL && cx.iid) ? 1 : 0;
 
   bool stopped = false;
   while ((!st.ev.rs.done && st.ev.steps < g.max_steps) || st.ev.final_ks) {
@@ -731,7 +752,7 @@
       ha.init_m = to_global((const double*)(secant ? cx.tabm(b_init) : (warm ? cx.tabm(b_cur) : nullptr)));
       ha.init_c = to_global((const double*)(secant ? cx.tabc(b_init) : (warm ? cx.tabc(b_cur) : nullptr)));
       ha.beta = cx.beta; ha.gam = cx.gam; ha.R = R;
-      ha.j0 = j0; ha.j1 = j1; ha.w = w; ha.G = G; ha.S = S; ha.n_a = n_a;
+      ha.j0 = j0; ha.j1 = j1; ha.w = w; ha.G = G; ha.S = S; ha.n_a = n_a; ha.iid = cx.iid;
       ha.opt = {g.max_cyc, g.aa_period, g.extrap_period};
       ha.dyn_lds = hk_lds_addr(ge_dyn);
       const int final_buf = pk == 1   ? ge_household_isolated<SMAX, SC, 1, TH>(ha, &nb, &ne)
@@ -781,6 +802,8 @@
       hk.lottery_fresh = true;
       hk.dyn_lds = hk_lds_addr(ge_dyn);
       if constexpr (PULL) mv = hk_solve_inlined<SMAX, KC, TH, true, false, SC>(hk, &nb, &ne);
+      else if (cx.iid)
+        mv = hk_solve_isolated<SMAX, KC, TH, false, (KC == 1 || kGeIidFuseAKc2) && kGeFuseA, SC, true>(hk, &nb, &ne);
       else mv = hk_solve_isolated<SMAX, KC, TH, false, (KC == 1 || kGeFuseAKc2) && kGeFuseA, SC>(hk, &nb, &ne);
     }
     if (mv == -1) return;
@@ -882,7 +905,7 @@
 
 struct GeScratch {
   double *tab, *mass, *pmass, *pg, *qb, *wlo, *slab, *outd, *prof, *evlog, *aah;
-  int *ainv, *lo, *span, *ids, *resume, *done, *outi;
+  int *ainv, *lo, *span, *ids, *resume, *done, *outi, *iid;
   unsigned *ctr, *err;
   unsigned long long* gran;
   GeState* saved;
@@ -911,6 +934,7 @@
   L.prof = c.take<double>((size_t)n_cal * kGeProf);
   L.evlog = c.take<double>((size_t)n_cal * kGeEvLog * kGeEvRec);
   L.aah = c.take<double>((size_t)n_cal * kGeAaHist * S * n_a);
+  L.iid = c.take<int>(n_cal);
   L.bytes = c.bytes();
   return L;
 }
@@ -918,6 +942,7 @@
 int32_t ge_stationary_resident(aiy_handle* h, const aiy_stationary_model* M, const aiy_ge_options* o, double* r_out,
                                double* K_out, double* Ks_out, int32_t* steps_out, int32_t* cyc_out,
                                int32_t* its_out, int32_t* status_out, hipStream_t st) {
+  h->ge_iid_cells = 0;
   if (!h->ge_resident || o->accel >= 0) return 0;
   const int n_cal = M->n_cal, S = M->S, n_a = M->n_a;
   GePlan p0;
@@ -950,6 +975,7 @@
   g.extrap_period = h->ge_extrap_period;
   g.aa_period = o->egm_extrapolate != 0 ? h->ge_anderson : 0;
   g.aah = L.aah;
+  g.iid_on = h->hist_iid; g.out_iid = L.iid;
   g.logsec = h->ge_logsec;
   g.tab = L.tab; g.mass = L.mass; g.pmass = L.pmass; g.pg = L.pg; g.qb = L.qb; g.ainv = L.ainv;
   g.loose_hist = std::pow(10.0, -(double)h->ge_loose_hist);
@@ -1017,7 +1043,8 @@
     active.swap(next);
   }
   std::vector<double> hd(3 * (size_t)n_cal);
-  std::vector<int> hi(4 * (size_t)n_cal);
+  std::vector<int> hi(4 * (size_t)n_cal), iid_h(n_cal, 0);
+  AIY_HIP(h, hipMemcpyAsync(iid_h.data(), L.iid, sizeof(int) * n_cal, hipMemcpyDeviceToHost, st));
   AIY_HIP(h, hipMemcpyAsync(hd.data(), outd, sizeof(double) * 3 * n_cal, hipMemcpyDeviceToHost, st));
   AIY_HIP(h, hipMemcpyAsync(hi.data(), outi, sizeof(int) * 4 * n_cal, hipMemcpyDeviceToHost, st));
   h->ge_prof.assign((size_t)n_cal * kGeProf, 0.0);
@@ -1030,6 +1057,7 @@
   long long cyc = 0, its = 0;
   int steps = 0;
   for (int c = 0; c < n_cal; ++c) {
+    h->ge_iid_cells += iid_h[c] != 0;
     r_out[c] = hd[c];
     K_out[c] = hd[n_cal + c];
     if (Ks_out) Ks_out[c] = hd[2 * n_cal + c];
@@ -1071,6 +1099,12 @@
   return AIY_OK;
 }
 
+extern "C" int32_t aiy_ge_last_iid_cells(aiy_handle* h, int32_t* cells) {
+  if (!h || !cells) return AIY_ERR_ARG;
+  *cells = h->ge_iid_cells;
+  return AIY_OK;
+}
+
 extern "C" int32_t aiy_ge_launch_stats(aiy_handle* h, double* ms_sum, int64_t* launches, double* point_matvecs,
                                        double* egm_cycles, int32_t reset) {
   if (!h) return AIY_ERR_ARG;
diff --git a/aiyagari_hark_amd/csrc/hist_bicg.h b/aiyagari_hark_amd/csrc/hist_bicg.h
--- a/aiyagari_hark_amd/csrc/hist_bicg.h
+++ b/aiyagari_hark_amd/csrc/hist_bicg.h
@@ -46,9 +46,20 @@
       tq = tn;                                                          \
     }                                                                   \
   } while (0)
+#define HK_PH_REPORT(mv)                                                                                           \
+  do {                                                                                                             \
+    if (tid == 0 && blockIdx.x >= AIY_DIAG_PHASES && blockIdx.x < AIY_DIAG_PHASES + 10 && (mv) > 0)                \
+      printf("[bicg phases] block %d G=%d nj=%d matvecs=%d us/matvec: push %.2f publish %.2f barrier %.2f "        \
+             "gather+mix %.2f reduce %.2f vector %.2f\n",                                                          \
+             (int)blockIdx.x, G, j1 - j0, (mv), ph[0] * 0.01 / (mv), ph[1] * 0.01 / (mv), ph[2] * 0.01 / (mv),     \
+             ph[3] * 0.01 / (mv), ph[4] * 0.01 / (mv), ph[5] * 0.01 / (mv));                                       \
+  } while (0)
 #else
 #define HK_PH(k) \
   do {           \
+  } while (0)
+#define HK_PH_REPORT(mv) \
+  do {                   \
   } while (0)
 #endif
 
@@ -105,10 +116,12 @@
   return a;
 }
 
-template <int SMAX, int KC, int TH, bool PULL = false, bool FUSEA = false, int SC = 0>
+template <int SMAX, int KC, int TH, bool PULL = false, bool FUSEA = false, int SC = 0, bool IID = false>
 __device__ __forceinline__ int hk_solve(const HkArgs& r, const HkShared<SMAX, KC, TH>& L, unsigned& nb,
                                         unsigned& ne) {
   constexpr bool kVlds = SMAX <= 8;
+  static_assert(!IID || (!PULL && SMAX <= 8), "the asset-grid solve: push form, S <= 8");
+  constexpr int NV = IID ? 1 : SMAX;
 #ifdef AIY_DIAG_PHASES
   unsigned long long ph[6] = {0, 0, 0, 0, 0, 0}, tq = 0;
 #endif
@@ -282,7 +295,7 @@
       s_cinfo[(k * SMAX + s) * TH + tid] = hk_cinfo(cf, cn, hi);
     }
   }
-  constexpr bool kLoReg = SMAX <= 8 && KC == 1 && TH <= 512;
+  constexpr bool kLoReg = SMAX <= 8 && (KC == 1 || IID) && TH <= 512;
   int dreg[KC][kLoReg ? SMAX : 1];
   double wreg[KC][kLoReg ? SMAX : 1];
   if constexpr (kLoReg) {
@@ -300,6 +313,11 @@
   const int v_base = lane < S ? s_base[lane] : 0;
   const int v_plo = lane < 2 * S ? s_pub[lane][0] : 0;
   const int v_phi = lane < 2 * S ? s_pub[lane][1] : 0;
+  double pi[IID ? SMAX : 1];
+  if constexpr (IID) {
+#pragma unroll
+    for (int s = 0; s < SMAX; ++s) pi[s] = hk_uni(s_P[s]);
+  }
   const int jbase = j0 + tid;
   auto col = [&]() {
     int c = jbase;
@@ -307,7 +325,7 @@
     return c;
   };
 
-  auto push = [&](const double (&q)[KC][SMAX]) {
+  auto push = [&](const double (&q)[KC][NV]) {
     constexpr int PR = SMAX <= 8 ? SMAX : 4;
     const int jc = col();
 #pragma unroll
@@ -342,8 +360,11 @@
             const int s = s0 + u;
             if (s < S) {
               const int d = dd[k][u];
-              const double vlo = ww[k][u] * q[k][s];
-              const double vhi = (1.0 - ww[k][u]) * q[k][s];
+              double qs;
+              if constexpr (IID) qs = pi[s] * q[k][0];
+              else qs = q[k][s];
+              const double vlo = ww[k][u] * qs;
+              const double vhi = (1.0 - ww[k][u]) * qs;
               const int ilo = __builtin_amdgcn_readlane(v_base, s) + d, ihi = ilo + 1;
               const int d0 = __builtin_amdgcn_readfirstlane(d);
               if (__all(act && d == d0)) {
@@ -374,7 +395,7 @@
     }
     asm volatile("s_waitcnt vmcnt(0)" ::: "memory");
   };
-  auto gather_mix = [&](int par, double (&out)[KC][SMAX]) {
+  auto gather_mix = [&](int par, double (&out)[KC][NV]) {
     constexpr int GR = 4;
     double T[KC][SMAX];
 #pragma unroll
@@ -496,6 +517,15 @@
         }
       }
     }
+    if constexpr (IID) {
+#pragma unroll
+      for (int k = 0; k < KC; ++k) {
+        double acc = T[k][0];
+#pragma unroll
+        for (int s = 1; s < SMAX; ++s) acc += T[k][s];
+        out[k][0] = acc;
+      }
+    } else {
 #pragma unroll
     for (int sp = 0; sp < SMAX; ++sp) {
       double pc[SMAX];
@@ -509,6 +539,7 @@
         for (int s = 0; s < SMAX; ++s) acc += pc[s] * T[k][s];
         out[k][sp] = acc;
       }
+    }
     }
   };
   auto stage_q = [&](const double (&q)[KC][SMAX]) {
@@ -608,7 +639,7 @@
       }
     }
   };
-  auto matvec = [&](const double (&q)[KC][SMAX], double (&out)[KC][SMAX]) -> bool {
+  auto matvec = [&](const double (&q)[KC][NV], double (&out)[KC][NV]) -> bool {
     if constexpr (PULL) {
       HK_PH(5);
       stage_q(q);
@@ -645,7 +676,7 @@
     HK_PH(4);
     return s_flag != 0;
   };
-  auto matvec_rp = [&](auto&& do_push, double (&out)[KC][SMAX], const double* vals, int nv, unsigned kmax) -> bool {
+  auto matvec_rp = [&](auto&& do_push, double (&out)[KC][NV], const double* vals, int nv, unsigned kmax) -> bool {
     HK_PH(5);
     hc_wave_parts(vals, nv, kmax, s_part);
     do_push();
@@ -665,8 +696,216 @@
     HK_PH(3);
     return *L.s_rok != 0;
   };
-  auto matvec_r = [&](const double (&q)[KC][SMAX], double (&out)[KC][SMAX], const double* vals, int nv,
+  auto matvec_r = [&](const double (&q)[KC][NV], double (&out)[KC][NV], const double* vals, int nv,
                       unsigned kmax) -> bool { return matvec_rp([&] { push(q); }, out, vals, nv, kmax); };
+  if constexpr (IID) {
+    int mv = 0;
+    auto col_act = [&](int jc, bool (&act)[KC]) {
+#pragma unroll
+      for (int k = 0; k < KC; ++k) act[k] = jc + k * TH < j1;
+    };
+    double pimax = 0.0;
+#pragma unroll
+    for (int s = 0; s < SMAX; ++s)
+      if (s < S) pimax = fmax(pimax, pi[s]);
+    const double tol = r.tol / pimax;
+    double xv[KC][1], rv[KC][1], pv[KC][1], tv[KC][1], vv[KC], uv[KC];
+    double part[kHcRed];
+    bool restart = true, first = true;
+    double rho = 0.0, total0 = 0.0;
+    bool act[KC];
+    double pu = 0.0;
+    unsigned seed = 0;
+    auto rh_at = [&](int jc, int k) { return hk_rhat((unsigned)(jc + k * TH) + seed * 0x5BD1E995u); };
+    double best = __builtin_inf();
+    int mv_best = 0;
+    auto store_x = [&](int jc, const double (&m)[KC]) {
+#pragma unroll
+      for (int k = 0; k < KC; ++k)
+        if (jc + k * TH < j1) {
+#pragma unroll
+          for (int s = 0; s < SMAX; ++s)
+            if (s < S) X[(size_t)s * n_a + jc + k * TH] = pi[s] * m[k];
+        }
+    };
+    {
+      const int jc = col();
+#pragma unroll
+      for (int k = 0; k < KC; ++k) {
+        double xs[SMAX];
+#pragma unroll
+        for (int s = 0; s < SMAX; ++s) xs[s] = X[min(s, S - 1) * n_a + min(jc + k * TH, n_a - 1)];
+        double acc = xs[0];
+#pragma unroll
+        for (int s = 1; s < SMAX; ++s)
+          if (s < S) acc += xs[s];
+        xv[k][0] = jc + k * TH < j1 ? acc : 0.0;
+      }
+    }
+    HK_PH(-1);
+    while (true) {
+      if (restart) {
+        if (!matvec(xv, tv)) return -1;
+        ++mv;
+        const int jc = col();
+        col_act(jc, act);
+        double rr = 0.0, rm = 0.0, xs = 0.0;
+#pragma unroll
+        for (int k = 0; k < KC; ++k) {
+          rv[k][0] = tv[k][0] - xv[k][0];
+          if (act[k]) {
+            rr += rh_at(jc, k) * rv[k][0];
+            rm = nan_max(rm, fabs(rv[k][0]));
+            xs += xv[k][0];
+          }
+        }
+        part[0] = rr;
+        part[1] = rm;
+        part[2] = xs;
+        if (!reduce(part, 3, 2u, [] {})) return -1;
+        rho = s_res[0];
+        if (mv == 1) total0 = s_res[2];
+        if (s_res[1] < tol || mv >= r.max_iter) {
+          const double scale = total0 / s_res[2];
+          double m[KC];
+#pragma unroll
+          for (int k = 0; k < KC; ++k) m[k] = mv == 1 ? tv[k][0] : tv[k][0] * scale;
+          store_x(jc, m);
+          break;
+        }
+        double pun = 0.0;
+#pragma unroll
+        for (int k = 0; k < KC; ++k) {
+          pv[k][0] = rv[k][0];
+          uv[k] = 0.0;
+          if constexpr (FUSEA) {
+            if (act[k]) {
+              double tr = 0.0;
+#pragma unroll
+              for (int s = 0; s < SMAX; ++s)
+                if (s < S) {
+                  const unsigned q = (unsigned)dreg[k][s] + seed * 0x5BD1E995u;
+                  tr += pi[s] * (wreg[k][s] * hk_rhat(q) + (1.0 - wreg[k][s]) * hk_rhat(q + 1u));
+                }
+              uv[k] = rh_at(jc, k) - tr;
+              pun += uv[k] * pv[k][0];
+            }
+          }
+        }
+        pu = pun;
+        restart = false;
+        first = true;
+      }
+      if (r.stop_ctr != nullptr && tid == 0 && ((mv >> 1) & 7) == 0)
+        s_stop = __hip_atomic_load((const unsigned*)r.stop_ctr, __ATOMIC_RELAXED, __HIP_MEMORY_SCOPE_AGENT) >= r.stop_at;
+      int jc = col();
+      col_act(jc, act);
+      if constexpr (FUSEA) {
+        double rm = 0.0;
+#pragma unroll
+        for (int k = 0; k < KC; ++k)
+          if (act[k]) rm = nan_max(rm, fabs(rv[k][0]));
+        part[0] = pu;
+        part[1] = (r.stop_ctr != nullptr && tid == 0 && s_stop) ? kHkStopSentinel : rm;
+        if (!matvec_r(pv, tv, part, 2, 2u)) return -1;
+        ++mv;
+#pragma unroll
+        for (int k = 0; k < KC; ++k) vv[k] = pv[k][0] - tv[k][0];
+      } else {
+        if (!matvec(pv, tv)) return -1;
+        ++mv;
+        jc = col();
+        col_act(jc, act);
+        double rvv = 0.0, rm = 0.0;
+#pragma unroll
+        for (int k = 0; k < KC; ++k) {
+          vv[k] = pv[k][0] - tv[k][0];
+          if (act[k]) {
+            rvv += rh_at(jc, k) * vv[k];
+            rm = nan_max(rm, fabs(rv[k][0]));
+          }
+        }
+        part[0] = rvv;
+        part[1] = (r.stop_ctr != nullptr && tid == 0 && s_stop) ? kHkStopSentinel : rm;
+        if (!reduce(part, 2, 2u, [] {})) return -1;
+      }
+      if (s_res[1] >= kHkStopSentinel) {
+        double m[KC];
+#pragma unroll
+        for (int k = 0; k < KC; ++k) m[k] = xv[k][0];
+        store_x(col(), m);
+        return -(2 + mv);
+      }
+      if ((!first && s_res[1] < tol) || mv >= r.max_iter) {
+        restart = true;
+        continue;
+      }
+      if (first || s_res[1] < 0.9 * best) {
+        best = first ? __builtin_inf() : s_res[1];
+        mv_best = mv;
+      } else if (mv - mv_best > kHkStall) {
+        ++seed;
+        best = __builtin_inf();
+        restart = true;
+        continue;
+      }
+      first = false;
+      const double alpha = rho / s_res[0];
+      if (!(fabs(alpha) < 1e300)) {
+        restart = true;
+        continue;
+      }
+#pragma unroll
+      for (int k = 0; k < KC; ++k) {
+        xv[k][0] += alpha * pv[k][0];
+        rv[k][0] -= alpha * vv[k];
+      }
+      if (!matvec(rv, tv)) return -1;
+      ++mv;
+      jc = col();
+      col_act(jc, act);
+      double ts = 0.0, tt = 0.0, rs = 0.0, rt = 0.0, sm = 0.0;
+#pragma unroll
+      for (int k = 0; k < KC; ++k) {
+        tv[k][0] = rv[k][0] - tv[k][0];
+        if (act[k]) {
+          const double h = rh_at(jc, k);
+          ts += tv[k][0] * rv[k][0];
+          tt += tv[k][0] * tv[k][0];
+          rs += h * rv[k][0];
+          rt += h * tv[k][0];
+          sm = nan_max(sm, fabs(rv[k][0]));
+        }
+      }
+      part[0] = ts;
+      part[1] = tt;
+      part[2] = rs;
+      part[3] = rt;
+      part[4] = sm;
+      if (!reduce(part, 5, 16u, [] {})) return -1;
+      double omega = (s_res[4] < tol) ? 0.0 : s_res[0] / s_res[1];
+      if (!(fabs(omega) < 1e300)) omega = 0.0;
+      if (omega == 0.0) {
+        restart = true;
+        continue;
+      }
+      const double rho2 = s_res[2] - omega * s_res[3];
+      const double beta = (rho2 / rho) * (alpha / omega);
+      rho = rho2;
+      double pun = 0.0;
+#pragma unroll
+      for (int k = 0; k < KC; ++k) {
+        xv[k][0] += omega * rv[k][0];
+        rv[k][0] = rv[k][0] - omega * tv[k][0];
+        pv[k][0] = rv[k][0] + beta * (pv[k][0] - omega * vv[k]);
+        if constexpr (FUSEA) pun += uv[k] * pv[k][0];
+      }
+      pu = pun;
+      if (!(fabs(beta) < 1e300) || rho == 0.0) restart = true;
+    }
+    HK_PH_REPORT(mv);
+    return mv;
+  } else {
   double rv[KC][SMAX], pv[KC][SMAX], tv[KC][SMAX];
   double* Vl = kVlds ? Tacc + cap : (double*)r.Vg;
   double* Pg = (double*)r.Pg;
@@ -971,14 +1210,9 @@
     pu = pun;
     if (!(fabs(beta) < 1e300) || rho == 0.0) restart = true;
   }
-#ifdef AIY_DIAG_PHASES
-  if (tid == 0 && blockIdx.x >= AIY_DIAG_PHASES && blockIdx.x < AIY_DIAG_PHASES + 10 && mv > 0)
-    printf("[bicg phases] block %d G=%d nj=%d matvecs=%d us/matvec: push %.2f publish %.2f barrier %.2f gather+mix "
-           "%.2f reduce %.2f vector %.2f\n",
-           (int)blockIdx.x, G, j1 - j0, mv, ph[0] * 0.01 / mv, ph[1] * 0.01 / mv, ph[2] * 0.01 / mv, ph[3] * 0.01 / mv,
-           ph[4] * 0.01 / mv, ph[5] * 0.01 / mv);
-#endif
+  HK_PH_REPORT(mv);
   return mv;
+  }
 }
 
 __device__ __forceinline__ int hk_uni(int x) { return __builtin_amdgcn_readfirstlane(x); }
@@ -1007,7 +1241,25 @@
   return u;
 }
 
-template <int SMAX, int KC, int TH, bool PULL = false, bool FUSEA = false, int SC = 0>
+template <int SMAX, int KC, int TH>
+struct HkIsoLds {
+  int s_base[SMAX];
+  int s_pub[2 * SMAX][2];
+  int s_tot;
+  HcCand s_cand[SMAX][kHcCand];
+  int s_ncand[SMAX];
+  unsigned short s_cinfo[KC * SMAX * TH];
+  double s_P[SMAX * SMAX];
+  double s_part[kHcRed][TH / kWave];
+  double s_res[kHcRed];
+  int s_flag, s_stop;
+  int s_ex[2 * SMAX];
+  int s_nheavy, s_heavy[kHkHeavy][4], s_rok, s_wcnt[TH / kWave];
+  double s_hval[kHkHeavy];
+};
+template <int SMAX, int KC, int TH>
+__shared__ HkIsoLds<SMAX, KC, TH> hk_iso_lds;
+template <int SMAX, int KC, int TH, bool PULL = false, bool FUSEA = false, int SC = 0, bool IID = false>
 __device__ __noinline__ int hk_solve_isolated(HkArgs a, unsigned* nb_io, unsigned* ne_io);
 template <int SMAX, int KC, int TH, bool PULL = false, bool FUSEA = false, int SC = 0>
 __device__ __forceinline__ int hk_solve_inlined(HkArgs a, unsigned* nb_io, unsigned* ne_io) {
@@ -1033,26 +1285,15 @@
   *ne_io = ne;
   return mv;
 }
-template <int SMAX, int KC, int TH, bool PULL, bool FUSEA, int SC>
+template <int SMAX, int KC, int TH, bool PULL, bool FUSEA, int SC, bool IID>
 __device__ __noinline__ int hk_solve_isolated(HkArgs a, unsigned* nb_io, unsigned* ne_io) {
   double* hk_dyn = (double*)(lptr<double>)(size_t)(unsigned)__builtin_amdgcn_readfirstlane((int)a.dyn_lds);
-  __shared__ int s_base[SMAX];
-  __shared__ int s_pub[2 * SMAX][2];
-  __shared__ int s_tot;
-  __shared__ HcCand s_cand[SMAX][kHcCand];
-  __shared__ int s_ncand[SMAX];
-  __shared__ unsigned short s_cinfo[KC * SMAX * TH];
-  __shared__ double s_P[SMAX * SMAX];
-  __shared__ double s_part[kHcRed][TH / kWave];
-  __shared__ double s_res[kHcRed];
-  __shared__ int s_flag, s_stop;
-  __shared__ int s_ex[2 * SMAX];
-  __shared__ int s_nheavy, s_heavy[kHkHeavy][4], s_rok, s_wcnt[TH / kWave];
-  __shared__ double s_hval[kHkHeavy];
-  HkShared<SMAX, KC, TH> L{hk_dyn, s_base, s_pub, &s_tot, s_cand, s_ncand, s_cinfo, s_P, s_part, s_res,
-                                 &s_flag, &s_stop, s_ex, &s_nheavy, s_wcnt, s_heavy, s_hval, &s_rok};
+  HkIsoLds<SMAX, KC, TH>& S_ = hk_iso_lds<SMAX, KC, TH>;
+  HkShared<SMAX, KC, TH> L{hk_dyn, S_.s_base, S_.s_pub, &S_.s_tot, S_.s_cand, S_.s_ncand, S_.s_cinfo, S_.s_P,
+                           S_.s_part, S_.s_res, &S_.s_flag, &S_.s_stop, S_.s_ex, &S_.s_nheavy, S_.s_wcnt,
+                           S_.s_heavy, S_.s_hval, &S_.s_rok};
   unsigned nb = *nb_io, ne = *ne_io;
-  const int mv = hk_solve<SMAX, KC, TH, PULL, FUSEA, SC>(hk_uniform_args(a), L, nb, ne);
+  const int mv = hk_solve<SMAX, KC, TH, PULL, FUSEA, SC, IID>(hk_uniform_args(a), L, nb, ne);
   *nb_io = nb;
   *ne_io = ne;
   return mv;
diff --git a/aiyagari_hark_amd/csrc/internal.h b/aiyagari_hark_amd/csrc/internal.h
--- a/aiyagari_hark_amd/csrc/internal.h
+++ b/aiyagari_hark_amd/csrc/internal.h
@@ -31,6 +31,7 @@
   int hist_krylov = 0;
   int res_shape_stream = 1;
   int hist_pull = 0;
+  int hist_iid = 1;
   int ge_loose_hist = 8;
   const double* egm_tolv = nullptr;
   const double* egm_tolh = nullptr;
@@ -43,6 +44,7 @@
   int ge_rebalance = 55;
   int ge_rounds = 0;
   int ge_mid_stops = 0;
+  int ge_iid_cells = 0;
   int ge_extrap_period = 32;
   int ge_anderson = 12;
   int ge_logsec = 2;
diff --git a/aiyagari_hark_amd/csrc/panel.hip b/aiyagari_hark_amd/csrc/panel.hip
--- a/aiyagari_hark_amd/csrc/panel.hip
+++ b/aiyagari_hark_amd/csrc/panel.hip
@@ -437,6 +437,7 @@
       return AIY_OK;
     case AIY_OPT_HIST_KRYLOV: h->hist_krylov = value != 0; return AIY_OK;
     case AIY_OPT_HIST_PULL: h->hist_pull = value != 0; return AIY_OK;
+    case AIY_OPT_HIST_IID: h->hist_iid = value != 0; return AIY_OK;
     case AIY_OPT_RESIDENT_SHAPE_STREAM:
       if (value < -1 || value > 2) return fail(h, AIY_ERR_ARG, "AIY_OPT_RESIDENT_SHAPE_STREAM must be -1, 0, 1 or 2");
       h->res_shape_stream = (int)value;
@@ -487,6 +488,7 @@
     case AIY_OPT_HIST_ACCEL: *value = h->hist_accel; return AIY_OK;
     case AIY_OPT_HIST_KRYLOV: *value = h->hist_krylov; return AIY_OK;
     case AIY_OPT_HIST_PULL: *value = h->hist_pull; return AIY_OK;
+    case AIY_OPT_HIST_IID: *value = h->hist_iid; return AIY_OK;
     case AIY_OPT_RESIDENT_SHAPE_STREAM: *value = h->res_shape_stream; return AIY_OK;
     case AIY_OPT_GE_LOOSE_HIST: *value = h->ge_loose_hist; return AIY_OK;
     case AIY_OPT_GE_RESIDENT: *value = h->ge_resident; return AIY_OK;
diff --git a/aiyagari_hark_amd/stationary.py b/aiyagari_hark_amd/stationary.py
--- a/aiyagari_hark_amd/stationary.py
+++ b/aiyagari_hark_amd/stationary.py
@@ -271,7 +271,8 @@
 
 _GROUP_CTX = {}
 _GROUP_CARRY_OPTIONS = (_lib.AIY_OPT_GE_LOGSEC, _lib.AIY_OPT_GE_REBALANCE, _lib.AIY_OPT_GE_EXTRAP_PERIOD,
-                        _lib.AIY_OPT_HIST_PULL, _lib.AIY_OPT_GE_LOOSE_HIST, _lib.AIY_OPT_GE_ANDERSON)
+                        _lib.AIY_OPT_HIST_PULL, _lib.AIY_OPT_GE_LOOSE_HIST, _lib.AIY_OPT_GE_ANDERSON,
+                        _lib.AIY_OPT_HIST_IID)
 
 
 def _close_groups():
diff --git a/include/aiyagari.h b/include/aiyagari.h
--- a/include/aiyagari.h
+++ b/include/aiyagari.h
@@ -167,6 +167,7 @@
 #define AIY_OPT_HIST_PULL 15
 #define AIY_OPT_GE_LOOSE_HIST 17
 #define AIY_OPT_RESIDENT_SHAPE_STREAM 18
+#define AIY_OPT_HIST_IID 24
 int32_t aiy_set_option(aiy_handle* h, int32_t option, int64_t value);
 int32_t aiy_get_option(aiy_handle* h, int32_t option, int64_t* value);
 
@@ -231,6 +232,7 @@
 int32_t aiy_ge_last_eval_log(aiy_handle* h, double* out, int32_t n_cal);
 
 int32_t aiy_ge_last_rounds(aiy_handle* h, int32_t* launches, int32_t* mid_solve_stops);
+int32_t aiy_ge_last_iid_cells(aiy_handle* h, int32_t* cells);
 
 int32_t aiy_hist_launch_stats(aiy_handle* h, double* ms_sum, int64_t* launches, int32_t reset);
 
```

Result: faster. 700.7 (median of 6 runs) (+10.6%).
